# MIT-SPARK/Khronos

Measured on NVIDIA B200. Metric: rgbd_frames_per_sec_integrated, higher is better.
Workload: dtype f32

## Files before the change

khronos_b200/build.py:

```python
from __future__ import annotations

import os
import subprocess
import sys

HERE = os.path.dirname(os.path.abspath(__file__))
ROOT = os.path.dirname(HERE)
CSRC = os.path.join(HERE, "csrc")
SOURCES = ["kb_kernels.cu", "kb_motion_device.cu", "kb_objects_device.cu", "kb_tracks_device.cu", "kb_rays.cu", "kb_peer.cu", "kb_mesh.cu", "kb_api.cu", "kb_motion_host.cpp"]
HEADERS = ["kb_device.cuh", "kb_kernels.cuh", "kb_motion_device.cuh", "kb_objects_device.cuh", "kb_tracks_device.cuh", "kb_unionfind.cuh", "kb_mesh.cuh", "kb_mc_tables.h", "kb_motion_host.h", os.path.join(ROOT, "include", "khronos_b200.h")]
LIB = os.path.join(CSRC, "libkhronos_b200.so")

NVCC_FLAGS = [
    "-gencode", "arch=compute_100a,code=sm_100a", "-O3", "-lineinfo", "-std=c++17",
    "-fmad=false", "-Xcompiler", "-fPIC,-ffp-contract=off,-fno-fast-math", "-shared",
]


def _stale(target, deps):
    if not os.path.exists(target):
        return True
    t = os.path.getmtime(target)
    return any(os.path.getmtime(d) > t for d in deps)


def build_product(force=False, verbose=False):
    srcs = [os.path.join(CSRC, s) for s in SOURCES]
    deps = srcs + [h if os.path.isabs(h) else os.path.join(CSRC, h) for h in HEADERS]
    if not force and not _stale(LIB, deps):
        return LIB
    extra = [f"-DKB_FUSE_MIN_BLOCKS={os.environ['KB_FUSE_MIN_BLOCKS']}"] if os.environ.get("KB_FUSE_MIN_BLOCKS") else []
    cmd = ["nvcc"] + NVCC_FLAGS + extra + (["-Xptxas", "-v"] if verbose else []) + ["-o", LIB] + srcs
    print(" ".join(cmd), file=sys.stderr)
    subprocess.check_call(cmd, cwd=CSRC)
    return LIB


VARIANTS = {"mb12": ["-DKB_FUSE_MIN_BLOCKS=12"], "mb8": ["-DKB_FUSE_MIN_BLOCKS=8"]}


def build_variant(name):
    srcs = [os.path.join(CSRC, s) for s in SOURCES]
    out = os.path.join(CSRC, f"libkhronos_b200_{name}.so")
    cmd = ["nvcc"] + NVCC_FLAGS + VARIANTS[name] + ["-o", out] + srcs
    print(" ".join(cmd), file=sys.stderr)
    subprocess.check_call(cmd, cwd=CSRC)
    return out


def build_oracle():
    subprocess.check_call(["make", "-C", os.path.join(ROOT, "oracle")])
    return os.path.join(ROOT, "oracle", "liboracle.so")


if __name__ == "__main__":
    build_product(force="--force" in sys.argv, verbose="-v" in sys.argv)
    build_oracle()
    for v in VARIANTS:
        if ("--variant=" + v) in sys.argv:
            build_variant(v)
```

khronos_b200/csrc/kb_api.cu:

```cuda
#include <algorithm>
#include <climits>
#include <cmath>
#include <cstdio>
#include <cstdlib>
#include <cstring>
#include <string>
#include <thread>
#include <type_traits>
#include <vector>

#include "../../include/khronos_b200.h"
#include "kb_kernels.cuh"
#include "kb_mesh.cuh"
#include "kb_motion_device.cuh"
#include "kb_objects_device.cuh"
#include "kb_tracks_device.cuh"
#include "kb_motion_host.h"

using namespace kb;

struct kb_handle {
  kb_map_config map{};
  kb_integrator_config integ{};
  kb_tracking_config trk{};
  kb_motion_config mot{};
  kb_camera cam{};
  bool has_trk = false, has_mot = false, has_cam = false;
  int device = 0;
  cudaStream_t stream = nullptr;
  bool own_stream = false;
  int rank = 0, nranks = 1;
  DeviceMap dm{};
  int L = 0;
  float block_size = 0, mle_diag = 0, mle_off = 0, mle_init = 0;
  unsigned long long blocked_mask = 0;
  std::vector<uint64_t> stamps;
  float* stg_depth = nullptr;
  int* stg_label = nullptr;
  int* stg_mask = nullptr;
  int* stg_object = nullptr;
  uint16_t* stg_depth16 = nullptr;
  uint8_t* stg_label8 = nullptr;
  uint8_t* stg_color = nullptr;
  size_t stg_color_pixels = 0;
  uint16_t* mot_depth16 = nullptr;
  float* stg_vertex = nullptr;
  float* mot_depth = nullptr;
  size_t stg_pixels = 0, mot_pixels = 0;
  int stg_set = 0;
  cudaStream_t copy_stream = nullptr;
  cudaEvent_t stg_ready[2] = {nullptr, nullptr}, stg_consumed[2] = {nullptr, nullptr};
  BatchParams batch{};
  float* tile_max = nullptr;
  size_t tile_stride = 0;
  int* work_slots = nullptr;
  uint32_t* work_masks = nullptr;
  uint32_t* work_upd = nullptr;
  uint32_t* item_fmask = nullptr;
  int* item_list = nullptr;
  int item_list_cap = 0;
  bool use_item_list = true;
  bool pipelined = true;
  cudaStream_t pre_stream = nullptr;
  cudaEvent_t pre_done[2] = {nullptr, nullptr}, fuse_done[2] = {nullptr, nullptr}, main_front = nullptr;
  bool main_dirty = true;
  int* work_slots2 = nullptr;
  uint32_t* work_masks2 = nullptr;
  uint32_t* work_upd2 = nullptr;
  uint32_t* item_fmask2 = nullptr;
  bool narrow_labels = false;
  int narrow_threads = 8;
  uint8_t* pin_label8 = nullptr;
  size_t pin_label8_pixels = 0;
  int fuse_coop = 0;
  int mlp_group = 0;
  int cull_grid = 0;
  int parity = 0;
  TrackEval pass{};
  float trk_cfg_thr = 0.f;
  uint64_t last_pass_stamp = 0;
  int* pending = nullptr;
  int everfree_grid = 0;
  bool cull = true;
  bool cull_forced = false;
  int fuse_grid = 0;
  bool hwm_dirty = true;
  size_t tombstones_ub = 0;
  size_t rehash_threshold = 0;
  int hwm_cached = 0;
  int* h_ctr = nullptr;
  int prev_ctr[kNumCounters] = {0};
  bool ctr_dirty = false;
  int3* d_pixel_gidx = nullptr;
  uint8_t* d_pixel_seed = nullptr;
  std::vector<int32_t> h_pixel_gidx;
  std::vector<uint8_t> h_pixel_seed;
  std::vector<float> h_depth;
  MotionResult motion;
  MotionTable mt{};
  int32_t* d_dynamic = nullptr;
  int* h_mscal = nullptr;
  bool motion_stale = false;
  MotionHostParams motion_hp{};
  bool motion_have_image = false;
  bool everfree_v2 = true;
  bool motion_sparse = true;
  bool mt_dirty = false;
  int3* d_removed = nullptr;
  int max_removed = 0;
  float* obj_depth = nullptr;
  int* obj_label = nullptr;
  int32_t* d_object = nullptr;
  int* h_oscal = nullptr;
  size_t obj_pixels = 0;
  std::vector<int32_t> obj_image_host, obj_label_host;
  bool obj_have = false;
  int32_t* trk_ids = nullptr;
  unsigned long long* trk_export = nullptr;
  size_t trk_pixels = 0;
  int* trk_counts = nullptr;
  unsigned long long* trk_sums = nullptr;
  int* trk_present = nullptr;
  int* trk_idlist = nullptr;
  unsigned long long* trk_keys = nullptr;
  int* trk_of = nullptr;
  size_t trk_voxel_cap = 0;
  int* trk_inter = nullptr;
  size_t trk_inter_cap = 0;
  std::vector<int32_t> trk_counts_host;
  bool trk_have = false;
  ShardExchange xch{};
  int cap_pending = 1024, cap_halo = 2048;
  uint8_t* d_flags_local = nullptr;
  size_t flags_local_pixels = 0;
  TrackingParams open_pass{};
  uint64_t open_pass_stamp = 0;
  int open_pass_state = 0;
  std::vector<uint8_t> shard_table_host;
  uint8_t* shard_table_dev = nullptr;
  int* inst_counts = nullptr;
  unsigned int* inst_bbox = nullptr;
  uint8_t* inst_background = nullptr;
  uint8_t* inst_keep = nullptr;
  int* inst_bad = nullptr;
  size_t inst_pixels = 0;
  struct InstCluster { int id, count; float bbox[6]; };
  std::vector<InstCluster> inst_clusters;
  std::vector<uint8_t> inst_keep_host;
  bool inst_have = false;
  int* mesh_slots = nullptr;
  unsigned char* mesh_cases = nullptr;
  int* mesh_tri_count = nullptr;
  long long* mesh_tri_base = nullptr;
  size_t mesh_block_cap = 0;
  float* mesh_points = nullptr;
  unsigned char* mesh_colors = nullptr;
  unsigned int* mesh_labels = nullptr;
  size_t mesh_tri_cap = 0;
// ... 264 lines not shown
    return KB_ERR_INVALID;
  if (integ->semantic_mode == KB_SEMANTICS_MLE && (integ->num_labels < 2 || integ->num_labels > KB_MAX_LABELS))
    return KB_ERR_INVALID;
  if (trk && (trk->neighbor_connectivity != 6 && trk->neighbor_connectivity != 18 && trk->neighbor_connectivity != 26))
    return KB_ERR_INVALID;
  if (trk && (!(trk->temporal_buffer > 0.f) || !(trk->temporal_window > 0.f) || trk->tsdf_occupancy_threshold == 0.f))
    return KB_ERR_INVALID;
  if (mot && (mot->neighbor_connectivity != 6 && mot->neighbor_connectivity != 18 && mot->neighbor_connectivity != 26))
    return KB_ERR_INVALID;
  if (mot && (mot->max_cluster_size < mot->min_cluster_size || !(mot->max_range > 0.f)))
    return KB_ERR_INVALID;

  auto* h = new kb_handle();
  h->map = *map;
  h->integ = *integ;
  if (trk) { h->trk = *trk; h->has_trk = true; }
  {
    const float cfg = trk ? trk->tsdf_occupancy_threshold : -1.5f;
    h->trk_cfg_thr = cfg < 0 ? cfg * -map->voxel_size : cfg;
  }
  if (mot) { h->mot = *mot; h->has_mot = true; }
  h->device = device;
  h->stamps.push_back(0);
  h->block_size = map->voxel_size * static_cast<float>(map->voxels_per_side);
  h->L = !map->with_semantics ? 0
         : integ->semantic_mode == KB_SEMANTICS_MLE ? integ->num_labels
         : integ->semantic_mode == KB_SEMANTICS_BINARY ? 2 : 0;
  if (integ->semantic_mode == KB_SEMANTICS_MLE) {
    const double c = static_cast<double>(integ->label_confidence), N = static_cast<double>(integ->num_labels);
    h->mle_diag = static_cast<float>(std::log(c));
    h->mle_off = static_cast<float>(std::log((1.0 - c) / (N - 1.0)));
    h->mle_init = static_cast<float>(std::log(1.0 / N));
    for (int i = 0; i < KB_MAX_LABELS; ++i)
      if (integ->label_blocked[i]) h->blocked_mask |= 1ull << i;
  }

  DeviceMap& m = h->dm;
  m.vps = map->voxels_per_side;
  m.V = m.vps * m.vps * m.vps;
  m.max_blocks = map->max_blocks;
  m.max_sem = h->L > 0 ? (map->max_semantic_blocks > 0 ? map->max_semantic_blocks : map->max_blocks) : 0;
  m.Lp = h->L == 0 ? 0 : (integ->semantic_mode == KB_SEMANTICS_BINARY ? 2 : ((h->L + 3) / 4) * 4);
  uint32_t cap = 1024;
  while (cap < static_cast<uint32_t>(m.max_blocks) * 2u) cap <<= 1;
  m.hash_mask = cap - 1;

  int st = KB_OK;
  auto run = [&]() -> int {
    KB_CUDA(h, cudaSetDevice(device));
    KB_CUDA(h, cudaStreamCreateWithFlags(&h->stream, cudaStreamNonBlocking));
    h->own_stream = true;
    const size_t S = m.max_blocks, V = m.V;
    KB_CUDA(h, devAlloc(&m.hash_keys, cap, 0xFF));
    KB_CUDA(h, devAlloc(&m.hash_vals, cap, 0xFF));
    KB_CUDA(h, devAlloc(&m.counters, kCounterInts, 0));
    KB_CUDA(h, devAlloc(&m.free_list, S, 0));
    KB_CUDA(h, devAlloc(&m.block_index, S, 0));
    KB_CUDA(h, devAlloc(&m.block_flags, S, 0));
    KB_CUDA(h, devAlloc(&m.block_sem, S, 0xFF));
    KB_CUDA(h, devAlloc(&m.tsdf, S * V, 0));
    if (map->with_tracking) {
      KB_CUDA(h, devAlloc(&m.last_obs, S * V, 0));
      KB_CUDA(h, devAlloc(&m.last_occ, S * V, 0));
      KB_CUDA(h, devAlloc(&m.vflags, S * V, 0));
      KB_CUDA(h, devAlloc(&m.born_frame, S, 0));
      m.frame_capacity = 1 << 20;
      KB_CUDA(h, devAlloc(&m.next_pass, static_cast<size_t>(m.frame_capacity), 0));
      KB_CUDA(h, devAlloc(&m.act_min, static_cast<size_t>(m.frame_capacity), 0));
      KB_CUDA(h, devAlloc(&h->pending, S, 0));
    }
    if (h->L > 0) {
      const size_t Q = m.max_sem;
      KB_CUDA(h, devAlloc(&m.sem_free_list, Q, 0));
      KB_CUDA(h, devAlloc(&m.sem_label, Q * V, 0xFF));
      KB_CUDA(h, devAlloc(&m.sem_lik, Q * V * m.Lp, 0));
    }
    KB_CUDA(h, cudaMallocHost(reinterpret_cast<void**>(&h->h_ctr), sizeof(int) * kCounterInts));
    std::memset(h->h_ctr, 0, sizeof(int) * kCounterInts);
    KB_CUDA(h, cudaStreamCreateWithFlags(&h->copy_stream, cudaStreamNonBlocking));
    for (int i = 0; i < 2; ++i) {
      KB_CUDA(h, cudaEventCreateWithFlags(&h->stg_ready[i], cudaEventDisableTiming));
      KB_CUDA(h, cudaEventCreateWithFlags(&h->stg_consumed[i], cudaEventDisableTiming));
    }
    KB_CUDA(h, devAlloc(&h->work_slots, S, 0));
    KB_CUDA(h, devAlloc(&h->work_masks, S, 0));
    KB_CUDA(h, devAlloc(&h->work_upd, S, 0));
    h->batch.items_per_block = m.V / 128;
    KB_CUDA(h, devAlloc(&h->item_fmask, S * h->batch.items_per_block, 0));
    if (const char* e = std::getenv("KB_FUSE_ITEM_LIST")) h->use_item_list = e[0] == '1';
    h->rehash_threshold = (static_cast<size_t>(cap)) / 4;
    if (const char* e = std::getenv("KB_REHASH_TOMBSTONES")) h->rehash_threshold = static_cast<size_t>(std::max(1, std::atoi(e)));
    if (const char* e = std::getenv("KB_EVERFREE_V2")) h->everfree_v2 = e[0] == '1';
    if (const char* e = std::getenv("KB_MOTION_SPARSE")) h->motion_sparse = e[0] == '1';
    if (const char* e = std::getenv("KB_H2D_NARROW_LABELS")) h->narrow_labels = e[0] == '1';
    if (const char* e = std::getenv("KB_H2D_THREADS")) h->narrow_threads = std::max(1, std::atoi(e));
    if (const char* e = std::getenv("KB_PIPELINE")) h->pipelined = e[0] == '1';
    if (h->pipelined) {
      KB_CUDA(h, cudaStreamCreateWithFlags(&h->pre_stream, cudaStreamNonBlocking));
      for (int i = 0; i < 2; ++i) {
        KB_CUDA(h, cudaEventCreateWithFlags(&h->pre_done[i], cudaEventDisableTiming));
        KB_CUDA(h, cudaEventCreateWithFlags(&h->fuse_done[i], cudaEventDisableTiming));
      }
      KB_CUDA(h, cudaEventCreateWithFlags(&h->main_front, cudaEventDisableTiming));
      KB_CUDA(h, devAlloc(&h->work_slots2, S, 0));
      KB_CUDA(h, devAlloc(&h->work_masks2, S, 0));
      KB_CUDA(h, devAlloc(&h->work_upd2, S, 0));
      KB_CUDA(h, devAlloc(&h->item_fmask2, S * h->batch.items_per_block, 0));
    }
    if (const char* e = std::getenv("KB_FUSE_COOP")) h->fuse_coop = e[0] == '1' ? 1 : 0;
    if (const char* e = std::getenv("KB_FUSE_MLP")) h->mlp_group = e[0] == '2' ? 2 : (e[0] == '4' ? 4 : 0);
    if (h->use_item_list) {
      h->item_list_cap = static_cast<int>(std::min<size_t>(S * h->batch.items_per_block, size_t(1) << 28));
      KB_CUDA(h, devAlloc(&h->item_list, static_cast<size_t>(2 * kItemClasses) * h->item_list_cap, 0));
    }
    {
      cudaDeviceProp prop{};
      KB_CUDA(h, cudaGetDeviceProperties(&prop, device));
      h->everfree_grid = prop.multiProcessorCount * 4;
      h->cull_grid = prop.multiProcessorCount * 8;
      h->fuse_grid = prop.multiProcessorCount * fuseBlocksPerSm(m.vps, m.Lp);
      if (const char* e = std::getenv("KB_FUSE_CTAS_PER_SM")) {
        const int n = std::atoi(e);
        if (n > 0) h->fuse_grid = prop.multiProcessorCount * n;
      }
    }
    h->max_removed = m.max_blocks;
    KB_CUDA(h, devAlloc(&h->d_removed, static_cast<size_t>(h->max_removed), 0));
    KB_CUDA(h, cudaDeviceSynchronize());
    return KB_OK;
  };
  st = run();
  if (st != KB_OK) {
    std::fprintf(stderr, "kb_create: %s\n", h->err.c_str());
    kb_destroy(h);
    return st;
  }
  *out = h;
  return KB_OK;
}

int kb_destroy(kb_handle* h) {
  if (!h) return KB_OK;
  cudaSetDevice(h->device);
  if (h->stream) cudaStreamSynchronize(h->stream);
  DeviceMap& m = h->dm;
  cudaFree(m.hash_keys); cudaFree(m.hash_vals); cudaFree(m.counters); cudaFree(m.free_list);
  cudaFree(m.sem_free_list); cudaFree(m.block_index); cudaFree(m.block_flags); cudaFree(m.block_sem);
  cudaFree(m.tsdf); cudaFree(m.last_obs); cudaFree(m.last_occ); cudaFree(m.vflags);
  cudaFree(m.born_frame); cudaFree(m.next_pass); cudaFree(m.act_min); cudaFree(h->pending);
  cudaFree(m.sem_label); cudaFree(m.sem_lik); cudaFree(m.color); cudaFree(h->stg_color);
  cudaFree(h->xch.halo_mark); cudaFree(h->xch.publish); cudaFree(h->xch.ghost_keys); cudaFree(h->xch.ghost_vals);
  cudaFree(h->obj_depth); cudaFree(h->obj_label); cudaFree(h->d_object); cudaFree(h->d_flags_local);
  if (h->h_oscal) cudaFreeHost(h->h_oscal);
  cudaFree(h->trk_ids); cudaFree(h->trk_export); cudaFree(h->trk_counts); cudaFree(h->trk_sums); cudaFree(h->trk_present); cudaFree(h->trk_idlist);
  cudaFree(h->trk_keys); cudaFree(h->trk_of); cudaFree(h->trk_inter);
  cudaFree(h->stg_depth); cudaFree(h->stg_label); cudaFree(h->stg_mask); cudaFree(h->stg_object);
  cudaFree(h->stg_vertex); cudaFree(h->d_pixel_gidx); cudaFree(h->d_pixel_seed); cudaFree(h->d_removed);
  cudaFree(h->d_dynamic);
  { MotionTable& t = h->mt; cudaFree(t.keys); cudaFree(t.count); cudaFree(t.flags); cudaFree(t.deg); cudaFree(t.parent);
    cudaFree(t.pix_total); cudaFree(t.min_seed); cudaFree(t.cluster_id); cudaFree(t.roots); cudaFree(t.scalars); cudaFree(t.pix_slot); cudaFree(t.occupied); }
  if (h->h_mscal) cudaFreeHost(h->h_mscal);
  cudaFree(h->stg_depth16); cudaFree(h->stg_label8); cudaFree(h->mot_depth16);
  cudaFree(h->mot_depth); cudaFree(h->tile_max); cudaFree(h->work_slots); cudaFree(h->work_masks); cudaFree(h->work_upd); cudaFree(h->item_fmask); cudaFree(h->item_list);
  for (int i = 0; i < 2; ++i) {
    if (h->stg_ready[i]) cudaEventDestroy(h->stg_ready[i]);
    if (h->stg_consumed[i]) cudaEventDestroy(h->stg_consumed[i]);
  }
  if (h->copy_stream) { cudaStreamSynchronize(h->copy_stream); cudaStreamDestroy(h->copy_stream); }
  if (h->pin_label8) cudaFreeHost(h->pin_label8);
  if (h->pre_stream) { cudaStreamSynchronize(h->pre_stream); cudaStreamDestroy(h->pre_stream); }
  for (int i = 0; i < 2; ++i) {
    if (h->pre_done[i]) cudaEventDestroy(h->pre_done[i]);
    if (h->fuse_done[i]) cudaEventDestroy(h->fuse_done[i]);
  }
  if (h->main_front) cudaEventDestroy(h->main_front);
  cudaFree(h->work_slots2); cudaFree(h->work_masks2); cudaFree(h->work_upd2); cudaFree(h->item_fmask2);
  cudaFree(h->shard_table_dev);
  cudaFree(h->inst_counts); cudaFree(h->inst_bbox); cudaFree(h->inst_background); cudaFree(h->inst_keep); cudaFree(h->inst_bad);
  cudaFree(h->mesh_slots); cudaFree(h->mesh_cases); cudaFree(h->mesh_tri_count); cudaFree(h->mesh_tri_base);
  cudaFree(h->mesh_points); cudaFree(h->mesh_colors); cudaFree(h->mesh_labels);
  if (h->h_ctr) cudaFreeHost(h->h_ctr);
  if (h->own_stream && h->stream) cudaStreamDestroy(h->stream);
  delete h;
  return KB_OK;
}

int kb_set_stream(kb_handle* h, void* cuda_stream) {
  if (h) h->main_dirty = true;
  if (!h) return KB_ERR_INVALID;
  KB_CUDA(h, cudaSetDevice(h->device));
  KB_CUDA(h, cudaStreamSynchronize(h->stream));
  if (h->own_stream) cudaStreamDestroy(h->stream);
  h->stream = static_cast<cudaStream_t>(cuda_stream);
  h->own_stream = false;
  return KB_OK;
}

int kb_synchronize(kb_handle* h) {
  if (!h) return KB_ERR_INVALID;
  KB_CUDA(h, cudaStreamSynchronize(h->copy_stream));
  KB_CUDA(h, cudaStreamSynchronize(h->stream));
  return KB_OK;
}

int kb_set_camera(kb_handle* h, const kb_camera* cam) {
  if (!h || !cam || cam->width <= 1 || cam->height <= 1 || !(cam->fx > 0.f) || !(cam->fy > 0.f))
    return fail(h, KB_ERR_INVALID, "invalid camera");
  KB_CUDA(h, cudaSetDevice(h->device));
  const bool same = h->has_cam && std::memcmp(&h->cam, cam, sizeof(kb_camera)) == 0;
  h->cam = *cam;
  h->has_cam = true;
  if (same) return KB_OK;
  const kb_camera& c = h->cam;
  BatchParams& p = h->batch;
  p.W = c.width; p.H = c.height;
  p.fx = c.fx; p.fy = c.fy; p.cx = c.cx; p.cy = c.cy;
  p.min_range = c.min_range; p.max_range = c.max_range;
  {
    const float xl = (0.f - c.cx) / c.fx, xr = (static_cast<float>(c.width - 1) - c.cx) / c.fx;
    const float yt = (0.f - c.cy) / c.fy, yb = (static_cast<float>(c.height - 1) - c.cy) / c.fy;
    const float il = 1.f / std::sqrt(1.f + xl * xl), ir = 1.f / std::sqrt(1.f + xr * xr);
    const float it = 1.f / std::sqrt(1.f + yt * yt), ib = 1.f / std::sqrt(1.f + yb * yb);
    p.pl[0][0] = il;  p.pl[0][1] = -xl * il;
    p.pl[1][0] = -ir; p.pl[1][1] = xr * ir;
    p.pl[2][0] = it;  p.pl[2][1] = -yt * it;
    p.pl[3][0] = -ib; p.pl[3][1] = yb * ib;
  }
  p.voxel_size = h->map.voxel_size;
  p.block_size = h->block_size;
  p.trunc = h->map.truncation_distance;
  p.infl = h->block_size * 0.8660254f;
  p.use_dropoff = h->integ.use_weight_dropoff;
  p.dropoff_eps = h->integ.weight_dropoff_epsilon > 0.f ? h->integ.weight_dropoff_epsilon
                                                       : h->integ.weight_dropoff_epsilon * -h->map.voxel_size;
  p.constant_weight = h->integ.use_constant_weight;
  p.max_weight = h->integ.max_weight;
  p.interp = h->integ.interpolation_method;
  p.adaptive_thr = h->integ.adaptive_max_depth_difference;
  p.sem_mode = h->L > 0 ? h->integ.semantic_mode : KB_SEMANTICS_NONE;
  p.L = h->L;
  p.mle_diag = h->mle_diag; p.mle_off = h->mle_off; p.mle_init = h->mle_init;
  p.blocked_mask = h->blocked_mask;
  p.with_tracking = h->map.with_tracking;
  p.occ_thr = h->trk_cfg_thr;
  h->tile_stride = 0;
  for (int l = 0; l < kTileLevels; ++l) {
    p.lvl_tx[l] = l == 0 ? (c.width + 7) / 8 : (p.lvl_tx[l - 1] + 1) / 2;
    p.lvl_ty[l] = l == 0 ? (c.height + 7) / 8 : (p.lvl_ty[l - 1] + 1) / 2;
    p.lvl_off[l] = static_cast<int>(h->tile_stride);
    h->tile_stride += static_cast<size_t>(p.lvl_tx[l]) * p.lvl_ty[l];
  }
  p.work_slots = h->work_slots;
  p.work_masks = h->work_masks;
  p.work_upd = h->work_upd;
  p.item_fmask = h->item_fmask;
  p.max_work = h->dm.max_blocks;
  cudaFree(h->tile_max);
  h->tile_max = nullptr;
  KB_CUDA(h, devAlloc(&h->tile_max, h->tile_stride * kMaxBatch * 2, 0));
  return ensureMotionBuffers(h, static_cast<size_t>(c.width) * c.height);
}

int kb_get_debug_counters(kb_handle* h, int32_t* out, int32_t n) {
  if (!h || !out) return KB_ERR_INVALID;
  KB_CUDA(h, cudaSetDevice(h->device));
  int st = readCounters(h);
  if (st != KB_OK) return st;
  for (int i = 0; i < std::min<int>(n, kNumCounters); ++i) out[i] = h->h_ctr[i];
  return KB_OK;
}

int kb_set_culling(kb_handle* h, int enabled) {
  if (!h) return KB_ERR_INVALID;
  h->cull = enabled != 0;
  h->cull_forced = enabled == 2;
  return KB_OK;
}

int kb_set_shard(kb_handle* h, int rank, int nranks) {
  if (h) h->main_dirty = true;
  if (!h || nranks < 1 || rank < 0 || rank >= nranks) return fail(h, KB_ERR_INVALID, "invalid shard");
  h->rank = rank;
  h->nranks = nranks;
  h->dm.shard_cell = 0;
  h->dm.shard_gx = h->dm.shard_gy = 1;
  h->dm.shard_table = nullptr;
  h->shard_table_host.clear();
  return KB_OK;
}

int kb_set_shard_cells(kb_handle* h, int rank, int nranks, int cell_blocks, int grid_x, int grid_y) {
  if (h) h->main_dirty = true;
  if (!h || nranks < 1 || rank < 0 || rank >= nranks || cell_blocks < 0 || (cell_blocks > 0 && (grid_x < 1 || grid_y < 1)))
    return fail(h, KB_ERR_INVALID, "invalid cell shard layout");
  h->rank = rank;
  h->nranks = nranks;
  h->dm.shard_cell = cell_blocks;
  h->dm.shard_gx = cell_blocks > 0 ? grid_x : 1;
  h->dm.shard_gy = cell_blocks > 0 ? grid_y : 1;
  h->dm.shard_table = nullptr;
  h->shard_table_host.clear();
  return KB_OK;
}

int kb_set_shard_table(kb_handle* h, int rank, int nranks, int cell_blocks, int32_t origin_cx, int32_t origin_cy, int32_t width,
                       int32_t height, const uint8_t* owners) {
  if (h) h->main_dirty = true;
  if (!h || nranks < 1 || nranks > 255 || rank < 0 || rank >= nranks || cell_blocks < 1 || width < 1 || height < 1 || !owners ||
      static_cast<long long>(width) * height > (1 << 24))
    return fail(h, KB_ERR_INVALID, "invalid cell table");
  KB_CUDA(h, cudaSetDevice(h->device));
  const size_t n = static_cast<size_t>(width) * height;
  for (size_t i = 0; i < n; ++i)
    if (owners[i] >= nranks) return fail(h, KB_ERR_INVALID, "cell table entry >= nranks");
  KB_CUDA(h, cudaStreamSynchronize(h->stream));
  cudaFree(h->shard_table_dev);
  h->shard_table_dev = nullptr;
  KB_CUDA(h, cudaMalloc(reinterpret_cast<void**>(&h->shard_table_dev), n));
  KB_CUDA(h, cudaMemcpy(h->shard_table_dev, owners, n, cudaMemcpyHostToDevice));
  h->shard_table_host.assign(owners, owners + n);
  h->rank = rank;
  h->nranks = nranks;
  h->dm.shard_cell = cell_blocks;
  int gy = static_cast<int>(std::floor(std::sqrt(static_cast<double>(nranks))));
  while (nranks % gy) --gy;
  h->dm.shard_gx = nranks / gy;
  h->dm.shard_gy = gy;
  h->dm.shard_table = h->shard_table_dev;
  h->dm.tab_ox = origin_cx; h->dm.tab_oy = origin_cy; h->dm.tab_w = width; h->dm.tab_h = height;
  return KB_OK;
}

int kb_cell_owner(int32_t bx, int32_t by, int cell_blocks, int grid_x, int grid_y, int nranks) {
  if (nranks <= 1 || cell_blocks < 1 || grid_x < 1 || grid_y < 1) return 0;
  return cellOwner(bx, by, cell_blocks, grid_x, grid_y, nranks);
}

namespace {
struct HostFrustum { float pl[4][2]; float infl, min_range, max_range, block_size; };
struct HostLayout { int nranks, cell, gx, gy; const uint8_t* table; int ox, oy, w, h; };

void hostFrustum(const kb_camera& c, float block_size, HostFrustum* f) {
// ... 67 lines not shown
      for (int by = lo[1]; by <= hi[1] && mask != all; ++by)
        for (int bx = lo[0]; bx <= hi[0]; ++bx) {
          const int owner = layoutOwner(L, bx, by, bz);
          if ((mask >> owner) & 1u) continue;
          if (!candidateSelected(f, infl, R, t, bx, by, bz)) continue;
          mask |= 1u << owner;
          if (mask == all) break;
        }
    owner_mask[i] = mask;
  }
  return KB_OK;
}

int frameCellsImpl(const HostFrustum& f, const kb_frame* frames, int32_t n_frames, int cell_blocks, int32_t origin_cx, int32_t origin_cy,
                   int32_t width, int32_t height, uint8_t* touched) {
  const float infl = f.infl + 1e-3f;
  const size_t cells = static_cast<size_t>(width) * height;
  std::memset(touched, 0, cells * static_cast<size_t>(n_frames));
  for (int i = 0; i < n_frames; ++i) {
    float R[9], t[3];
    int lo[3], hi[3];
    if (!frameBox(f, infl, frames[i], R, t, lo, hi)) return KB_ERR_INVALID;
    uint8_t* row = touched + cells * static_cast<size_t>(i);
    for (int by = lo[1]; by <= hi[1]; ++by) {
      const int cy = floorDiv(by, cell_blocks) - origin_cy;
      if (cy < 0 || cy >= height) continue;
      for (int bx = lo[0]; bx <= hi[0]; ++bx) {
        const int cx = floorDiv(bx, cell_blocks) - origin_cx;
        if (cx < 0 || cx >= width || row[cy * width + cx]) continue;
        for (int bz = lo[2]; bz <= hi[2]; ++bz)
          if (candidateSelected(f, infl, R, t, bx, by, bz)) { row[cy * width + cx] = 1; break; }
      }
    }
  }
  return KB_OK;
}

HostLayout handleLayout(const kb_handle* h) {
  const DeviceMap& m = h->dm;
  return HostLayout{h->nranks, m.shard_cell, m.shard_gx, m.shard_gy, h->shard_table_host.empty() ? nullptr : h->shard_table_host.data(),
                    m.tab_ox, m.tab_oy, m.tab_w, m.tab_h};
}
}

int kb_frame_owners(kb_handle* h, const kb_frame* frames, int32_t n_frames, uint32_t* owner_mask) {
  if (!h || !frames || !owner_mask || n_frames < 0) return fail(h, KB_ERR_INVALID, "null argument");
  if (!h->has_cam) return fail(h, KB_ERR_STATE, "kb_set_camera must be called first");
  if (h->nranks > 32) return fail(h, KB_ERR_INVALID, "kb_frame_owners supports at most 32 ranks");
  HostFrustum f;
  handleFrustum(h, &f);
  const int st = frameOwnersImpl(f, handleLayout(h), frames, n_frames, owner_mask);
  return st == KB_OK ? KB_OK : fail(h, st, "non-finite sensor pose");
}

int kb_frame_cells(kb_handle* h, const kb_frame* frames, int32_t n_frames, int cell_blocks, int32_t origin_cx, int32_t origin_cy,
                   int32_t width, int32_t height, uint8_t* touched) {
  if (!h || !frames || !touched || n_frames < 0 || cell_blocks < 1 || width < 1 || height < 1) return fail(h, KB_ERR_INVALID, "invalid argument");
  if (!h->has_cam) return fail(h, KB_ERR_STATE, "kb_set_camera must be called first");
  HostFrustum f;
  handleFrustum(h, &f);
  const int st = frameCellsImpl(f, frames, n_frames, cell_blocks, origin_cx, origin_cy, width, height, touched);
  return st == KB_OK ? KB_OK : fail(h, st, "non-finite sensor pose");
}

int kb_frame_owners_host(const kb_camera* camera, float voxel_size, int32_t voxels_per_side, const kb_shard_layout* layout,
                         const kb_frame* frames, int32_t n_frames, uint32_t* owner_mask) {
  if (!camera || !layout || !frames || !owner_mask || n_frames < 0 || !(voxel_size > 0.f) || voxels_per_side < 1 || layout->nranks < 1 ||
      layout->nranks > 32 || layout->cell_blocks < 0 || (layout->cell_blocks > 0 && (layout->grid_x < 1 || layout->grid_y < 1)))
    return KB_ERR_INVALID;
  HostFrustum f;
  hostFrustum(*camera, voxel_size * static_cast<float>(voxels_per_side), &f);
  const HostLayout L{layout->nranks, layout->cell_blocks, layout->grid_x, layout->grid_y, layout->table, layout->table_origin_cx,
                     layout->table_origin_cy, layout->table_width, layout->table_height};
  return frameOwnersImpl(f, L, frames, n_frames, owner_mask);
}

int kb_frame_cells_host(const kb_camera* camera, float voxel_size, int32_t voxels_per_side, const kb_frame* frames, int32_t n_frames,
                        int cell_blocks, int32_t origin_cx, int32_t origin_cy, int32_t width, int32_t height, uint8_t* touched) {
  if (!camera || !frames || !touched || n_frames < 0 || !(voxel_size > 0.f) || voxels_per_side < 1 || cell_blocks < 1 || width < 1 || height < 1)
    return KB_ERR_INVALID;
  HostFrustum f;
  hostFrustum(*camera, voxel_size * static_cast<float>(voxels_per_side), &f);
  return frameCellsImpl(f, frames, n_frames, cell_blocks, origin_cx, origin_cy, width, height, touched);
}

static int integrateBatch(kb_handle* h, const kb_frame* frames, int n, int allocate_blocks) {
  const kb_camera& c = h->cam;
  const size_t px = static_cast<size_t>(c.width) * c.height;
  BatchParams& p = h->batch;
  if (allocate_blocks && n > 1) {
    const double reach = static_cast<double>(c.max_range) + static_cast<double>(h->block_size) * 0.8660254;
    const double inv = 1.0 / static_cast<double>(h->block_size);
    double lo[3] = {1e300, 1e300, 1e300}, hi[3] = {-1e300, -1e300, -1e300};
    for (int b = 0; b < n; ++b)
      for (int a = 0; a < 3; ++a) {
        const double t = frames[b].world_T_sensor[a * 4 + 3];
        lo[a] = std::min(lo[a], std::floor((t - reach) * inv));
        hi[a] = std::max(hi[a], std::floor((t + reach) * inv));
      }
    const double single = std::pow(2.0 * reach * inv + 2.0, 3.0);
    const double cells = (hi[0] - lo[0] + 1.0) * (hi[1] - lo[1] + 1.0) * (hi[2] - lo[2] + 1.0);
    if (!(cells <= 8.0 * single)) {
      int st = integrateBatch(h, frames, n / 2, allocate_blocks);
      if (st != KB_OK) return st;
      return integrateBatch(h, frames + n / 2, n - n / 2, allocate_blocks);
    }
  }
  p.n_frames = n;
  p.allocate = allocate_blocks ? 1 : 0;
  p.rank = h->rank;
  p.nranks = h->nranks;
  p.parity = h->parity;
  h->parity ^= 1;
  const int par = p.parity;
  const bool pipe = h->pipelined && n >= 4;
  if (!pipe) h->main_dirty = true;
  p.pipelined = pipe ? 1 : 0;
  p.fetch_ctr = (pipe && par) ? kCtrFetchB : kCtrFetch;
  p.items_ctr = (pipe && par) ? kCtrItemsB0 : kCtrItems0;
  p.work_slots = (pipe && par) ? h->work_slots2 : h->work_slots;
  p.work_masks = (pipe && par) ? h->work_masks2 : h->work_masks;
  p.work_upd = (pipe && par) ? h->work_upd2 : h->work_upd;
  p.item_fmask = (pipe && par) ? h->item_fmask2 : h->item_fmask;
  const size_t tile_set = (pipe && par) ? h->tile_stride * kMaxBatch : 0;
  p.cull = (h->cull && (n >= 4 || h->cull_forced)) ? 1 : 0;
  p.layers_per_item = n >= 8 ? 1 : 4;
  p.trk = h->pass;

  bool any_host = false, any_compact = false, any_color = false, any_host_color = false;
  for (int b = 0; b < n; ++b) {
    any_host |= frames[b].memory != KB_MEM_DEVICE;
    any_compact |= frames[b].depth_u16 != nullptr || frames[b].label_u8 != nullptr;
    any_color |= frames[b].color != nullptr;
    any_host_color |= frames[b].color != nullptr && frames[b].memory != KB_MEM_DEVICE;
  }
  p.has_color = any_color ? 1 : 0;
  p.item_list = (h->use_item_list && p.cull && n >= 8 && !any_color)
                    ? h->item_list + ((pipe && par) ? static_cast<size_t>(kItemClasses) * h->item_list_cap : 0) : nullptr;
  p.item_list_cap = h->item_list_cap;
  p.mlp_group = h->mlp_group;
  p.coop = h->fuse_coop;
  if (any_color) {
    int st = ensureColorLayer(h);
    if (st == KB_OK && any_host_color) st = ensureColorStaging(h, px);
    if (st != KB_OK) return st;
  }
  const int set = h->stg_set;
  const bool use_staging = any_host || any_compact;
  if (use_staging) {
    int st = ensureStaging(h, px);
    if (st != KB_OK) return st;
    h->stg_set ^= 1;
    KB_CUDA(h, cudaStreamWaitEvent(h->copy_stream, h->stg_consumed[set], 0));
  }
  bool narrowed[kMaxBatch] = {false};
  bool any_narrowed = false;
  if (h->narrow_labels && any_host) {
    int cand[kMaxBatch], nc = 0;
    for (int b = 0; b < n; ++b)
      if (frames[b].memory != KB_MEM_DEVICE && frames[b].label && !frames[b].label_u8) cand[nc++] = b;
    if (nc > 0) {
      if (h->pin_label8_pixels < px) {
        KB_CUDA(h, cudaStreamSynchronize(h->copy_stream));
        if (h->pin_label8) cudaFreeHost(h->pin_label8);
        h->pin_label8 = nullptr;
        KB_CUDA(h, cudaMallocHost(reinterpret_cast<void**>(&h->pin_label8), px * kMaxBatch * 2));
        h->pin_label8_pixels = px;
      }
      KB_CUDA(h, cudaEventSynchronize(h->stg_ready[set]));
      uint8_t* base8 = h->pin_label8 + static_cast<size_t>(set) * kMaxBatch * px;
      auto work = [&](int t, int T) {
        for (int k = t; k < nc; k += T) {
          const int b = cand[k];
          const int32_t* __restrict__ src = frames[b].label;
          uint8_t* __restrict__ dst = base8 + static_cast<size_t>(b) * px;
          int32_t acc = 0;
          for (size_t i = 0; i < px; ++i) { acc |= src[i]; dst[i] = static_cast<uint8_t>(src[i]); }
          narrowed[b] = (acc & ~0xFF) == 0;
        }
      };
      const int T = std::max(1, std::min(h->narrow_threads, nc));
      if (T == 1) {
        work(0, 1);
      } else {
        std::vector<std::thread> pool;
        for (int t = 0; t < T; ++t) pool.emplace_back(work, t, T);
        for (auto& th : pool) th.join();
      }
      for (int b = 0; b < n; ++b) any_narrowed |= narrowed[b];
    }
  }
  int lo[3] = {INT32_MAX, INT32_MAX, INT32_MAX}, hi[3] = {INT32_MIN, INT32_MIN, INT32_MIN};
  for (int b = 0; b < n; ++b) {
    const kb_frame& f = frames[b];
    FrameView& v = p.f[b];
    float Rw[9], tw[3];
    poseToFloat(f.world_T_sensor, v.R, v.t, Rw, tw);
    if (h->map.with_tracking && f.stamp_ns <= h->last_pass_stamp)
      return fail(h, KB_ERR_STATE, "frames must be newer than the last kb_update_tracking stamp");
    uint32_t fidx = 0;
    int st = frameIndex(h, f.stamp_ns, &fidx);
    if (st != KB_OK) return st;
    v.frame_idx = fidx;
    v.target_id = f.object_target_id;
    const size_t off = (static_cast<size_t>(set) * kMaxBatch + b) * px;
    if (f.memory == KB_MEM_DEVICE) {
      v.depth = f.depth; v.label = f.label; v.mask = f.mask; v.object_image = f.object_image;
      v.depth16 = f.depth_u16; v.label8 = f.label_u8;
      v.color = f.color;
    } else {
      v.color = f.color ? h->stg_color + off * 3 : nullptr;
      v.depth = f.depth ? h->stg_depth + off : nullptr;
      v.label = f.label ? h->stg_label + off : nullptr;
      v.mask = f.mask ? h->stg_mask + off : nullptr;
      v.object_image = f.object_image ? h->stg_object + off : nullptr;
      v.depth16 = f.depth_u16 ? h->stg_depth16 + off : nullptr;
      v.label8 = (f.label_u8 || narrowed[b]) ? h->stg_label8 + off : nullptr;
    }
    v.depth_scale = f.depth_u16_scale;
    if (v.depth16) v.depth = h->stg_depth + off;
    if (v.label8) v.label = h->stg_label + off;
    if (!v.depth) return fail(h, KB_ERR_INVALID, "frame without depth image");
    if (f.mask == KB_MASK_LAST_DETECTION)
      v.mask = h->motion_have_image ? h->d_dynamic : nullptr;
    v.tiles = h->tile_max + tile_set + static_cast<size_t>(b) * h->tile_stride;
    if (allocate_blocks) {
      const float reach = c.max_range + p.infl;
      const float inv = 1.f / h->block_size;
      for (int a = 0; a < 3; ++a) {
        lo[a] = std::min(lo[a], static_cast<int>(std::floor((tw[a] - reach) * inv)));
        hi[a] = std::max(hi[a], static_cast<int>(std::floor((tw[a] + reach) * inv)));
      }
    }
  }
  if (any_host) {
    auto copyKind = [&](auto member, auto* staging, size_t per = 1) -> int {
      using T = std::remove_pointer_t<decltype(staging)>;
      const size_t img = px * per;
      int b = 0;
      while (b < n) {
        const T* src = (frames[b].memory == KB_MEM_DEVICE) ? nullptr : static_cast<const T*>(frames[b].*member);
        if (!src || static_cast<const void*>(src) == static_cast<const void*>(KB_MASK_LAST_DETECTION)) { ++b; continue; }
        int e = b + 1;
        while (e < n && frames[e].memory != KB_MEM_DEVICE && static_cast<const T*>(frames[e].*member) == src + static_cast<size_t>(e - b) * img) ++e;
        T* dst = staging + (static_cast<size_t>(set) * kMaxBatch + b) * img;
        KB_CUDA(h, cudaMemcpyAsync(dst, src, static_cast<size_t>(e - b) * img * sizeof(T), cudaMemcpyHostToDevice, h->copy_stream));
        b = e;
      }
      return KB_OK;
    };
    int cst;
    if ((cst = copyKind(&kb_frame::depth, h->stg_depth)) != KB_OK) return cst;
    if (!any_narrowed) {
      if ((cst = copyKind(&kb_frame::label, h->stg_label)) != KB_OK) return cst;
    } else {
      for (int b = 0; b < n;) {
        if (narrowed[b]) {
          int e = b + 1;
          while (e < n && narrowed[e]) ++e;
          const size_t o = (static_cast<size_t>(set) * kMaxBatch + b) * px;
          KB_CUDA(h, cudaMemcpyAsync(h->stg_label8 + o, h->pin_label8 + o, static_cast<size_t>(e - b) * px, cudaMemcpyHostToDevice, h->copy_stream));
          b = e;
        } else {
          if (frames[b].memory != KB_MEM_DEVICE && frames[b].label) {
            const size_t o = (static_cast<size_t>(set) * kMaxBatch + b) * px;
            KB_CUDA(h, cudaMemcpyAsync(h->stg_label + o, frames[b].label, px * sizeof(int32_t), cudaMemcpyHostToDevice, h->copy_stream));
          }
          ++b;
        }
      }
    }
    if ((cst = copyKind(&kb_frame::mask, h->stg_mask)) != KB_OK) return cst;
    if ((cst = copyKind(&kb_frame::object_image, h->stg_object)) != KB_OK) return cst;
    if ((cst = copyKind(&kb_frame::depth_u16, h->stg_depth16)) != KB_OK) return cst;
    if ((cst = copyKind(&kb_frame::label_u8, h->stg_label8)) != KB_OK) return cst;
    if (any_host_color && (cst = copyKind(&kb_frame::color, h->stg_color, 3)) != KB_OK) return cst;
    KB_CUDA(h, cudaEventRecord(h->stg_ready[set], h->copy_stream));
    KB_CUDA(h, cudaStreamWaitEvent(h->stream, h->stg_ready[set], 0));
  }
  if (allocate_blocks) {
    for (int a = 0; a < 3; ++a) { p.lo[a] = lo[a]; p.dims[a] = hi[a] - lo[a] + 1; }
    h->hwm_dirty = true;
  } else {
    if (h->hwm_dirty) {
      int st, nslots = 0;
      if ((st = slotHwm(h, &nslots)) != KB_OK) return st;
      h->hwm_cached = nslots;
      h->hwm_dirty = false;
    }
    p.n_slots = h->hwm_cached;
  }
  any_compact = any_compact || any_narrowed;
  bool all_compact = any_compact;
  for (int b = 0; b < n; ++b) all_compact = all_compact && frames[b].depth_u16 != nullptr && frames[b].label == nullptr;
  p.compact_taps = all_compact ? 1 : 0;
  cudaStream_t ps = h->stream;
  if (pipe) {
    ps = h->pre_stream;
    if (any_host) KB_CUDA(h, cudaStreamWaitEvent(ps, h->stg_ready[set], 0));
    KB_CUDA(h, cudaStreamWaitEvent(ps, h->fuse_done[par], 0));
    if (h->main_dirty) {
      KB_CUDA(h, cudaEventRecord(h->main_front, h->stream));
      KB_CUDA(h, cudaStreamWaitEvent(ps, h->main_front, 0));
      h->main_dirty = false;
    }
    KB_CUDA(h, cudaMemsetAsync(h->dm.counters + kCtrWork0 + par, 0, sizeof(int), ps));
    KB_CUDA(h, cudaMemsetAsync(h->dm.counters + p.fetch_ctr, 0, sizeof(int), ps));
  }
  if (!pipe && h->pipelined) {
    KB_CUDA(h, cudaMemsetAsync(h->dm.counters + kCtrWork0 + par, 0, sizeof(int), ps));
  }
  if (any_compact && !all_compact) launchExpandFrames(p, ps);
  if (p.cull) launchTileMax(p, ps);
  launchSelectBlocks(h->dm, p, h->cull_grid, ps);
  if (pipe) {
    KB_CUDA(h, cudaEventRecord(h->pre_done[par], ps));
    KB_CUDA(h, cudaStreamWaitEvent(h->stream, h->pre_done[par], 0));
  }
  launchFuse(h->dm, p, h->fuse_grid, h->stream);
  if (pipe) KB_CUDA(h, cudaEventRecord(h->fuse_done[par], h->stream));
  KB_CUDA(h, cudaGetLastError());
  if (use_staging) KB_CUDA(h, cudaEventRecord(h->stg_consumed[set], h->stream));
  if (any_host) {
    bool must_wait = false;
    for (int b = 0; b < n; ++b) must_wait |= frames[b].memory == KB_MEM_HOST;
    if (must_wait) KB_CUDA(h, cudaStreamSynchronize(h->copy_stream));
  }
  h->ctr_dirty = true;
  return KB_OK;
}

int kb_integrate_frames(kb_handle* h, const kb_frame* frames, int32_t n_frames, int allocate_blocks,
                        kb_frame_stats* stats) {
  if (!h || !frames || n_frames < 0) return fail(h, KB_ERR_INVALID, "null frames");
  if (!h->has_cam) return fail(h, KB_ERR_STATE, "kb_set_camera must be called first");
  for (int i = 0; i < n_frames; ++i) {
    if (!frames[i].depth && !frames[i].depth_u16) return fail(h, KB_ERR_INVALID, "frame without depth image");
    for (int k = 0; k < 16; ++k)
      if (!std::isfinite(frames[i].world_T_sensor[k])) return fail(h, KB_ERR_INVALID, "non-finite sensor pose");
  }
  KB_CUDA(h, cudaSetDevice(h->device));
  int st;
  if (stats && h->ctr_dirty) {
    if ((st = readCounters(h)) != KB_OK) return st;
    std::memcpy(h->prev_ctr, h->h_ctr, sizeof(h->prev_ctr));
    h->ctr_dirty = false;
  }
  if (!h->own_stream) h->main_dirty = true;
  for (int i = 0; i < n_frames; i += kMaxBatch) {
    if ((st = integrateBatch(h, frames + i, std::min(kMaxBatch, n_frames - i), allocate_blocks)) != KB_OK) return st;
  }
  if (stats) {
    if ((st = readCounters(h)) != KB_OK) return st;
    const int* c1 = h->h_ctr;
    const int* c0 = h->prev_ctr;
    auto d = [&](int k) { return static_cast<int32_t>(static_cast<uint32_t>(c1[k]) - static_cast<uint32_t>(c0[k])); };
    stats->blocks_in_frustum = d(kCtrFrustum);
    stats->blocks_allocated = d(kCtrAllocated);
    stats->blocks_updated = d(kCtrBlocksUpdated);
    stats->voxels_updated = d(kCtrVoxelsUpdated);
    stats->voxels_in_band = d(kCtrVoxelsBand);
    stats->voxels_semantic = d(kCtrVoxelsSemantic);
    stats->total_blocks = c1[kCtrLiveBlocks];
    stats->capacity_exceeded = c1[kCtrCapacityExceeded];
    std::memcpy(h->prev_ctr, h->h_ctr, sizeof(h->prev_ctr));
    h->ctr_dirty = false;
    if (c1[kCtrCapacityExceeded]) return fail(h, KB_ERR_CAPACITY, "block / semantic pool exhausted");
  }
  return KB_OK;
}

int kb_integrate_frame(kb_handle* h, const kb_frame* f, int allocate_blocks, kb_frame_stats* stats) {
  return kb_integrate_frames(h, f, f ? 1 : 0, allocate_blocks, stats);
}

int kb_get_totals(kb_handle* h, kb_frame_stats* t) {
  if (!h || !t) return KB_ERR_INVALID;
  KB_CUDA(h, cudaSetDevice(h->device));
  int st = readCounters(h);
  if (st != KB_OK) return st;
  const int* c = h->h_ctr;
  t->blocks_in_frustum = c[kCtrFrustum];
  t->blocks_allocated = c[kCtrAllocated];
  t->blocks_updated = c[kCtrBlocksUpdated];
  t->voxels_updated = c[kCtrVoxelsUpdated];
  t->voxels_in_band = c[kCtrVoxelsBand];
  t->voxels_semantic = c[kCtrVoxelsSemantic];
  t->total_blocks = c[kCtrLiveBlocks];
  t->capacity_exceeded = c[kCtrCapacityExceeded];
  return KB_OK;
}

int kb_get_totals64(kb_handle* h, kb_totals64* t) {
  if (!h || !t) return KB_ERR_INVALID;
  KB_CUDA(h, cudaSetDevice(h->device));
  int st = readCounters(h);
  if (st != KB_OK) return st;
  const unsigned long long* c = totals64(h->h_ctr);
  t->blocks_in_frustum = c[kTotFrustum];
  t->blocks_allocated = c[kTotAllocated];
  t->blocks_updated = c[kTotBlocksUpdated];
  t->voxels_updated = c[kTotVoxelsUpdated];
  t->voxels_in_band = c[kTotVoxelsBand];
  t->voxels_semantic = c[kTotVoxelsSemantic];
  t->block_frame_pairs = c[kTotPairs];
  t->total_blocks = static_cast<uint64_t>(std::max(h->h_ctr[kCtrLiveBlocks], 0));
  t->capacity_exceeded = static_cast<uint64_t>(h->h_ctr[kCtrCapacityExceeded]);
  t->frames = static_cast<uint64_t>(h->stamps.size() - 1);
  return KB_OK;
}

int kb_map_checksum(kb_handle* h, uint64_t out[4]) {
  if (!h || !out) return KB_ERR_INVALID;
  KB_CUDA(h, cudaSetDevice(h->device));
  int st, n = 0;
  if ((st = slotHwm(h, &n)) != KB_OK) return st;
  unsigned long long *d_stamps = nullptr, *d_out = nullptr;
  auto body = [&]() -> int {
    KB_CUDA(h, cudaMalloc(&d_stamps, sizeof(uint64_t) * h->stamps.size()));
    KB_CUDA(h, cudaMalloc(&d_out, sizeof(uint64_t) * 4));
    KB_CUDA(h, cudaMemcpyAsync(d_stamps, h->stamps.data(), sizeof(uint64_t) * h->stamps.size(), cudaMemcpyHostToDevice, h->stream));
    KB_CUDA(h, cudaMemsetAsync(d_out, 0, sizeof(uint64_t) * 4, h->stream));
    launchChecksum(h->dm, n, d_stamps, d_out, h->stream);
    KB_CUDA(h, cudaGetLastError());
    KB_CUDA(h, cudaMemcpyAsync(out, d_out, sizeof(uint64_t) * 4, cudaMemcpyDeviceToHost, h->stream));
    KB_CUDA(h, cudaStreamSynchronize(h->stream));
    return KB_OK;
  };
  st = body();
  cudaFree(d_stamps);
  cudaFree(d_out);
  h->main_dirty = true;
  return st;
}
// ... 1144 lines not shown
```

khronos_b200/csrc/kb_device.cuh:

```cuda
#pragma once

#include <cuda_runtime.h>
#include <stdint.h>

namespace kb {

constexpr unsigned long long kEmptyKey = ~0ull;
constexpr unsigned long long kTombKey = ~0ull - 1ull;
constexpr uint32_t kFlagAllocated = 1u << 8;
constexpr uint32_t kFlagEverFreePending = 1u << 9;
constexpr uint32_t kPublicFlagMask = 0x1Fu;
constexpr uint16_t kSemEmpty = 0xFFFFu;
constexpr uint8_t kVoxEverFree = 1, kVoxActive = 2, kVoxToRemove = 4;
constexpr uint8_t kVoxNotOccupied = 8;
constexpr uint32_t kFlagInactiveOverride = 1u << 10;

struct DeviceMap {
  unsigned long long* hash_keys;
  int* hash_vals;
  uint32_t hash_mask;
  int max_blocks, max_sem;
  int vps, V, Lp;
  int* counters;
  int* free_list;
  int* sem_free_list;
  int3* block_index;
  uint32_t* block_flags;
  int* block_sem;
  float2* tsdf;
  uint32_t* last_obs;
  uint32_t* last_occ;
  uint8_t* vflags;
  uint32_t* born_frame;
  uint32_t* next_pass;
  uint32_t* act_min;
  int frame_capacity;
  uint16_t* sem_label;
  float* sem_lik;
  uchar4* color;
  int shard_cell, shard_gx, shard_gy;
  const uint8_t* shard_table;
  int tab_ox, tab_oy, tab_w, tab_h;
};

enum Counter {
  kCtrPoolHwm = 0,
  kCtrFreeCount = 1,
  kCtrSemHwm = 2,
  kCtrSemFreeCount = 3,
  kCtrLiveBlocks = 4,
  kCtrCapacityExceeded = 5,
  kCtrFrustum = 6,
  kCtrAllocated = 7,
  kCtrBlocksUpdated = 8,
  kCtrVoxelsUpdated = 9,
  kCtrVoxelsBand = 10,
  kCtrVoxelsSemantic = 11,
  kCtrSeeds = 12,
  kCtrRemoved = 13,
  kCtrErased = 14,
  kCtrWork0 = 15,
  kCtrWork1 = 16,
  kCtrPairs = 17,
  kCtrPending = 18,
  kCtrFetch = 19,
  kCtrHalo = 20,
  kCtrFetchB = 24,
  kCtrRehash = 28,
  kCtrItems0 = 32,
  kCtrItemsB0 = 40,
  kNumCounters = 48
};
constexpr int kItemClasses = 8;

enum Total64 {
  kTotVoxelsUpdated = 0,
  kTotVoxelsBand = 1,
  kTotVoxelsSemantic = 2,
  kTotFrustum = 3,
  kTotPairs = 4,
  kTotBlocksUpdated = 5,
  kTotAllocated = 6,
  kNumTotals = 8
};
constexpr int kCounterInts = kNumCounters + 2 * kNumTotals;
__host__ __device__ inline unsigned long long* totals64(int* counters) {
  return reinterpret_cast<unsigned long long*>(counters + kNumCounters);
}

__host__ __device__ inline unsigned long long packKey(int x, int y, int z) {
  const unsigned long long o = 1ull << 20, m = (1ull << 21) - 1ull;
  return ((static_cast<unsigned long long>(x + static_cast<long long>(o)) & m)) |
         ((static_cast<unsigned long long>(y + static_cast<long long>(o)) & m) << 21) |
         ((static_cast<unsigned long long>(z + static_cast<long long>(o)) & m) << 42);
}

__host__ __device__ inline unsigned long long mix64(unsigned long long k) {
  k ^= k >> 33;
  k *= 0xff51afd7ed558ccdull;
  k ^= k >> 33;
  k *= 0xc4ceb9fe1a85ec53ull;
  k ^= k >> 33;
  return k;
}

__host__ __device__ inline int blockOwner(int x, int y, int z, int nranks) {
  return static_cast<int>((mix64(packKey(x, y, z)) >> 40) % static_cast<unsigned long long>(nranks));
}

__host__ __device__ inline int cellOwner(int x, int y, int cell, int gx, int gy, int nranks) {
  const int cx = (x >= 0 ? x : x - cell + 1) / cell, cy = (y >= 0 ? y : y - cell + 1) / cell;
  const int mx = ((cx % gx) + gx) % gx, my = ((cy % gy) + gy) % gy;
  return (mx + gx * my) % nranks;
}
__host__ __device__ inline int floorDiv(int a, int b) { return (a >= 0 ? a : a - b + 1) / b; }
__host__ __device__ inline int tableOwner(const uint8_t* table, int ox, int oy, int w, int h, int cell, int gx, int gy, int x, int y,
                                          int nranks) {
  const int cx = floorDiv(x, cell) - ox, cy = floorDiv(y, cell) - oy;
  if (cx >= 0 && cx < w && cy >= 0 && cy < h) return table[cy * w + cx] % nranks;
  return cellOwner(x, y, cell, gx, gy, nranks);
}
__device__ inline int mapOwner(const DeviceMap& m, int x, int y, int z, int nranks) {
  if (m.shard_cell <= 0) return blockOwner(x, y, z, nranks);
  if (m.shard_table) return tableOwner(m.shard_table, m.tab_ox, m.tab_oy, m.tab_w, m.tab_h, m.shard_cell, m.shard_gx, m.shard_gy, x, y, nranks);
  return cellOwner(x, y, m.shard_cell, m.shard_gx, m.shard_gy, nranks);
}

#ifdef __CUDACC__
__device__ inline int hashLookup(const DeviceMap& m, int x, int y, int z) {
  const unsigned long long key = packKey(x, y, z);
  uint32_t h = static_cast<uint32_t>(mix64(key)) & m.hash_mask;
  for (uint32_t probe = 0; probe <= m.hash_mask; ++probe) {
    const unsigned long long k = m.hash_keys[h];
    if (k == key) return m.hash_vals[h];
    if (k == kEmptyKey) return -1;
    h = (h + 1) & m.hash_mask;
  }
  return -1;
}

__device__ inline int allocSlot(int* counters, int ctr_hwm, int ctr_free, const int* free_list, int cap) {
  int nfree = atomicSub(&counters[ctr_free], 1);
  if (nfree > 0) return free_list[nfree - 1];
  atomicAdd(&counters[ctr_free], 1);
  const int s = atomicAdd(&counters[ctr_hwm], 1);
  if (s >= cap) {
    atomicSub(&counters[ctr_hwm], 1);
    atomicExch(&counters[kCtrCapacityExceeded], 1);
    return -1;
  }
  return s;
}

__device__ inline int hashFindOrInsert(const DeviceMap& m, int x, int y, int z, uint32_t born, int* created) {
  const unsigned long long key = packKey(x, y, z);
  uint32_t h = static_cast<uint32_t>(mix64(key)) & m.hash_mask;
// ... 76 lines not shown
```

khronos_b200/csrc/kb_kernels.cu:

```cuda
#include <limits.h>

#include <algorithm>

#include "../../include/khronos_b200.h"
#include "kb_kernels.cuh"

namespace kb {

namespace {

constexpr int kThreads = 256;
constexpr int kFuseThreads = 128;
#ifndef KB_FUSE_MIN_BLOCKS
#define KB_FUSE_MIN_BLOCKS 10
#endif
#ifndef KB_FUSE_COLOR_MIN_BLOCKS
#define KB_FUSE_COLOR_MIN_BLOCKS 8
#endif

__device__ __forceinline__ void xform(const float* R, const float* t, float x, float y, float z,
                                      float& ox, float& oy, float& oz) {
  ox = ((R[0] * x + R[1] * y) + R[2] * z) + t[0];
  oy = ((R[3] * x + R[4] * y) + R[5] * z) + t[1];
  oz = ((R[6] * x + R[7] * y) + R[8] * z) + t[2];
}

__device__ __forceinline__ bool inFrustum(const BatchParams& p, float x, float y, float z) {
  const float infl = p.infl;
  if (z < -infl) return false;
  const float r = sqrtf((x * x + y * y) + z * z);
  if (r < p.min_range - infl || r > p.max_range + infl) return false;
  if (p.pl[0][0] * x + p.pl[0][1] * z < -infl) return false;
  if (p.pl[1][0] * x + p.pl[1][1] * z < -infl) return false;
  if (p.pl[2][0] * y + p.pl[2][1] * z < -infl) return false;
  if (p.pl[3][0] * y + p.pl[3][1] * z < -infl) return false;
  return true;
}

template <bool COMPACT>
__device__ __forceinline__ float depthAt(const FrameView& f, int i) {
  if (COMPACT) return static_cast<float>(__ldg(&f.depth16[i])) * f.depth_scale;
  return __ldg(&f.depth[i]);
}
template <bool COMPACT>
__device__ __forceinline__ int labelAt(const FrameView& f, int i) {
  if (COMPACT) return static_cast<int>(__ldg(&f.label8[i]));
  return __ldg(&f.label[i]);
}

struct Taps {
  bool valid, bilinear;
  int u, v;
  float w0, w1, w2, w3;
};

template <bool COMPACT>
__device__ __forceinline__ Taps nearestTaps(const BatchParams& p, const FrameView& f, float u, float v) {
  Taps t;
  t.bilinear = false;
  t.u = static_cast<int>(roundf(u));
  t.v = static_cast<int>(roundf(v));
  t.w0 = t.w1 = t.w2 = t.w3 = 0.f;
  t.valid = t.u >= 0 && t.u < p.W && t.v >= 0 && t.v < p.H && depthAt<COMPACT>(f, t.v * p.W + t.u) > 0.f;
  return t;
}

template <bool COMPACT>
__device__ __forceinline__ Taps computeTaps(const BatchParams& p, const FrameView& f, float u, float v, float& range) {
  Taps t;
  t.valid = false;
  if (p.interp == KB_INTERP_NEAREST) {
    t = nearestTaps<COMPACT>(p, f, u, v);
    if (t.valid) range = depthAt<COMPACT>(f, t.v * p.W + t.u);
    return t;
  }
  const int u0 = static_cast<int>(floorf(u)), v0 = static_cast<int>(floorf(v));
  const bool inside = u0 >= 0 && v0 >= 0 && u0 + 1 < p.W && v0 + 1 < p.H;
  bool use_nearest = !inside;
  float r0 = 0.f, r1 = 0.f, r2 = 0.f, r3 = 0.f;
  if (inside) {
    const int i0 = v0 * p.W + u0;
    r0 = depthAt<COMPACT>(f, i0);
    r2 = depthAt<COMPACT>(f, i0 + 1);
    r1 = depthAt<COMPACT>(f, i0 + p.W);
    r3 = depthAt<COMPACT>(f, i0 + p.W + 1);
    const bool all_valid = r0 > 0.f && r1 > 0.f && r2 > 0.f && r3 > 0.f;
    if (p.interp == KB_INTERP_ADAPTIVE) {
      const float mx = fmaxf(fmaxf(r0, r1), fmaxf(r2, r3));
      const float mn = fminf(fminf(r0, r1), fminf(r2, r3));
      use_nearest = !all_valid || !(mx - mn < p.adaptive_thr);
    } else if (!all_valid) {
      return t;
    }
  } else if (p.interp != KB_INTERP_ADAPTIVE) {
    return t;
  }
  if (use_nearest) {
    t = nearestTaps<COMPACT>(p, f, u, v);
    if (t.valid) range = depthAt<COMPACT>(f, t.v * p.W + t.u);
    return t;
  }
  const float du = u - static_cast<float>(u0), dv = v - static_cast<float>(v0);
  t.valid = true;
  t.bilinear = true;
  t.u = u0;
  t.v = v0;
  t.w0 = (1.f - du) * (1.f - dv);
  t.w1 = (1.f - du) * dv;
  t.w2 = du * (1.f - dv);
  t.w3 = du * dv;
  range = ((t.w0 * r0 + t.w1 * r1) + t.w2 * r2) + t.w3 * r3;
  return t;
}

__device__ __forceinline__ int tapIndex(const BatchParams& p, const Taps& t) {
  int du = 0, dv = 0;
  if (t.bilinear) {
    int best = 0;
    float bw = t.w0;
    if (t.w1 > bw) { best = 1; bw = t.w1; }
    if (t.w2 > bw) { best = 2; bw = t.w2; }
    if (t.w3 > bw) { best = 3; }
    du = best >> 1;
    dv = best & 1;
  }
  return (t.v + dv) * p.W + t.u + du;
}

__device__ __forceinline__ float measurementWeight(const BatchParams& p, float depth, float sdf) {
  float w = (p.fx * p.fy) * (p.voxel_size * p.voxel_size) / (depth * depth);
  if (!p.constant_weight) w = w / (depth * depth);
  if (p.use_dropoff && sdf < -p.dropoff_eps) {
    w = w * ((p.trunc + sdf) / (p.trunc - p.dropoff_eps));
    w = fmaxf(w, 0.f);
  }
  return w;
}

__device__ __forceinline__ uchar3 measuredColor(const BatchParams& p, const FrameView& f, const Taps& t) {
  const uint8_t* __restrict__ p0 = f.color + (static_cast<size_t>(t.v) * p.W + t.u) * 3;
  if (!t.bilinear) return make_uchar3(__ldg(p0), __ldg(p0 + 1), __ldg(p0 + 2));
  const uint8_t* __restrict__ p1 = p0 + static_cast<size_t>(p.W) * 3;
  uint8_t o[3];
#pragma unroll
  for (int ch = 0; ch < 3; ++ch) {
    const float s = ((t.w0 * static_cast<float>(__ldg(p0 + ch)) + t.w1 * static_cast<float>(__ldg(p1 + ch))) +
                     t.w2 * static_cast<float>(__ldg(p0 + 3 + ch))) + t.w3 * static_cast<float>(__ldg(p1 + 3 + ch));
    o[ch] = static_cast<uint8_t>(static_cast<int>(s));
  }
  return make_uchar3(o[0], o[1], o[2]);
}

__device__ __forceinline__ uint8_t mergeChannel(uint8_t c, uint8_t cm, float ratio) {
  return static_cast<uint8_t>(static_cast<int>(static_cast<float>(c) * (1.f - ratio) + static_cast<float>(cm) * ratio));
}

__device__ __forceinline__ int warpSum(int v) {
#pragma unroll
  for (int o = 16; o > 0; o >>= 1) v += __shfl_xor_sync(0xffffffffu, v, o);
  return v;
}

__global__ void __launch_bounds__(256) expandFramesKernel(const __grid_constant__ BatchParams p) {
  const FrameView& f = p.f[blockIdx.y];
  const int n = p.W * p.H;
  for (int i = blockIdx.x * blockDim.x + threadIdx.x; i < n; i += gridDim.x * blockDim.x) {
    if (f.depth16) const_cast<float*>(f.depth)[i] = static_cast<float>(__ldg(&f.depth16[i])) * f.depth_scale;
    if (f.label8) const_cast<int*>(f.label)[i] = static_cast<int>(__ldg(&f.label8[i]));
  }
}

__global__ void expandDepthKernel(const uint16_t* __restrict__ src, float scale, float* __restrict__ dst, int n) {
  const int i = blockIdx.x * blockDim.x + threadIdx.x;
  if (i < n) dst[i] = static_cast<float>(src[i]) * scale;
}

__global__ void __launch_bounds__(256) tileMaxKernel(const __grid_constant__ BatchParams p) {
  const int b = blockIdx.y;
  const int warps_x = (p.W + 31) / 32;
  const int warp = blockIdx.x * 8 + (threadIdx.x >> 5);
  const int lane = threadIdx.x & 31;
  if (warp >= warps_x * p.lvl_ty[1]) return;
  const int ty16 = warp / warps_x, wx = warp % warps_x;
  const int u = wx * 32 + lane;
  const FrameView& f = p.f[b];
  float d[2] = {0.f, 0.f};
#pragma unroll
  for (int r = 0; r < 16; ++r) {
    const int v = ty16 * 16 + r;
    if (u < p.W && v < p.H)
      d[r >> 3] = fmaxf(d[r >> 3], p.compact_taps ? depthAt<true>(f, v * p.W + u) : depthAt<false>(f, v * p.W + u));
  }
#pragma unroll
  for (int h = 0; h < 2; ++h) {
    d[h] = fmaxf(d[h], __shfl_xor_sync(0xffffffffu, d[h], 1));
    d[h] = fmaxf(d[h], __shfl_xor_sync(0xffffffffu, d[h], 2));
    d[h] = fmaxf(d[h], __shfl_xor_sync(0xffffffffu, d[h], 4));
    const int tx = wx * 4 + (lane >> 3), ty = ty16 * 2 + h;
    if ((lane & 7) == 0 && tx < p.lvl_tx[0] && ty < p.lvl_ty[0]) p.f[b].tiles[p.lvl_off[0] + ty * p.lvl_tx[0] + tx] = d[h];
  }
  float m16 = fmaxf(d[0], d[1]);
  m16 = fmaxf(m16, __shfl_xor_sync(0xffffffffu, m16, 8));
  const int tx16 = wx * 2 + (lane >> 4);
  if ((lane & 15) == 0 && tx16 < p.lvl_tx[1]) p.f[b].tiles[p.lvl_off[1] + ty16 * p.lvl_tx[1] + tx16] = m16;
}

__global__ void __launch_bounds__(256) tileMaxVec4Kernel(const __grid_constant__ BatchParams p) {
  const int b = blockIdx.y;
  const int strips_x = (p.W + 127) / 128;
  const int warp = blockIdx.x * 8 + (threadIdx.x >> 5);
  const int lane = threadIdx.x & 31;
  if (warp >= strips_x * p.lvl_ty[1]) return;
  const int ty16 = warp / strips_x, sx = warp % strips_x;
  const int u = sx * 128 + lane * 4;
  const FrameView& f = p.f[b];
  float d[2] = {0.f, 0.f};
  if (u < p.W) {
    const float4* __restrict__ base = reinterpret_cast<const float4*>(f.depth + u);
    const int w4 = p.W >> 2;
    float4 v[16];
#pragma unroll
    for (int r = 0; r < 16; ++r) {
// ... 79 lines not shown
__device__ __forceinline__ bool boxCulledLane(const BatchParams& p, const FrameView& f, float lox, float loy, float loz,
                                              float hix, float hiy, float hiz) {
  return boxCulledPose(p, f.R, f.t, f.tiles, lox, loy, loz, hix, hiy, hiz);
}

template <bool PIPE>
__global__ void __launch_bounds__(128) selectBlocksKernel(const DeviceMap m, const __grid_constant__ BatchParams p) {
  const int c0 = (blockIdx.x * blockDim.x + threadIdx.x) >> 5;
  const int lane = threadIdx.x & 31;
  __shared__ float s_pose[12][kMaxBatch];
  __shared__ const float* s_tiles[kMaxBatch];
  for (int i = threadIdx.x; i < 12 * kMaxBatch; i += blockDim.x) {
    const int b = i % kMaxBatch, k = i / kMaxBatch;
    s_pose[k][b] = b < p.n_frames ? (k < 9 ? p.f[b].R[k] : p.f[b].t[k - 9]) : 0.f;
  }
  if (threadIdx.x < kMaxBatch) s_tiles[threadIdx.x] = threadIdx.x < p.n_frames ? p.f[threadIdx.x].tiles : nullptr;
  __syncthreads();
  float Rl[9], tl[3];
#pragma unroll
  for (int k = 0; k < 9; ++k) Rl[k] = s_pose[k][lane];
#pragma unroll
  for (int k = 0; k < 3; ++k) tl[k] = s_pose[9 + k][lane];
  if (!PIPE && c0 == 0 && lane == 0) {
    m.counters[kCtrWork0 + (p.parity ^ 1)] = 0;
    m.counters[kCtrFetch] = 0;
  }
  int slot = -1, bx = 0, by = 0, bz = 0;
  uint32_t mask = 0;
  int created = 0;
  if (p.allocate) {
    if (c0 >= p.dims[0] * p.dims[1] * p.dims[2]) return;
    int c = c0;
    bx = p.lo[0] + c % p.dims[0];
    c /= p.dims[0];
    by = p.lo[1] + c % p.dims[1];
    bz = p.lo[2] + c / p.dims[1];
    const float cx = (static_cast<float>(bx) + 0.5f) * p.block_size;
    const float cy = (static_cast<float>(by) + 0.5f) * p.block_size;
    const float cz = (static_cast<float>(bz) + 0.5f) * p.block_size;
    if (p.nranks > 1 && mapOwner(m, bx, by, bz, p.nranks) != p.rank) return;
    bool in = false;
    if (lane < p.n_frames) {
      float x, y, z;
      xform(Rl, tl, cx, cy, cz, x, y, z);
      in = inFrustum(p, x, y, z);
    }
    mask = __ballot_sync(0xffffffffu, in);
    if (!mask) return;
    if (lane == 0) slot = hashFindOrInsert(m, bx, by, bz, p.f[__ffs(mask) - 1].frame_idx, &created);
    slot = __shfl_sync(0xffffffffu, slot, 0);
    if (slot < 0) return;
  } else {
    if (c0 >= p.n_slots || !(m.block_flags[c0] & kFlagAllocated)) return;
    slot = c0;
    const int3 bi = m.block_index[slot];
    bx = bi.x; by = bi.y; bz = bi.z;
    mask = p.n_frames >= 32 ? 0xffffffffu : ((1u << p.n_frames) - 1u);
  }
  if (lane == 0) {
    atomicAdd(&m.counters[kCtrFrustum], __popc(mask));
    atomicAdd(&totals64(m.counters)[kTotFrustum], static_cast<unsigned long long>(__popc(mask)));
    if (created) {
      atomicAdd(&m.counters[kCtrAllocated], 1);
      atomicAdd(&totals64(m.counters)[kTotAllocated], 1ull);
    }
  }
  if (p.cull) {
    const float ox = static_cast<float>(bx) * p.block_size, oy = static_cast<float>(by) * p.block_size,
                oz = static_cast<float>(bz) * p.block_size;
    const float lo = 0.5f * p.voxel_size, hi = p.block_size - 0.5f * p.voxel_size;
    bool keep = false;
    if ((mask >> lane) & 1u)
      keep = !boxCulledPose(p, Rl, tl, s_tiles[lane], ox + lo, oy + lo, oz + lo, ox + hi, oy + hi, oz + hi);
    mask = __ballot_sync(0xffffffffu, keep);
    if (!mask) return;
  }
  int i = 0;
  if (lane == 0) {
    if (p.L > 0 && m.block_sem[slot] < 0) {
      m.block_sem[slot] = allocSlot(m.counters, kCtrSemHwm, kCtrSemFreeCount, m.sem_free_list, m.max_sem);
    }
    atomicAdd(&m.counters[kCtrPairs], __popc(mask));
    atomicAdd(&totals64(m.counters)[kTotPairs], static_cast<unsigned long long>(__popc(mask)));
    i = atomicAdd(&m.counters[kCtrWork0 + p.parity], 1);
    if (i < p.max_work) {
      p.work_slots[i] = slot;
      p.work_masks[i] = mask;
      p.work_upd[i] = 0;
    } else {
      atomicExch(&m.counters[kCtrCapacityExceeded], 1);
    }
  }
  i = __shfl_sync(0xffffffffu, i, 0);
  if (i < p.max_work && lane < p.items_per_block) p.item_fmask[static_cast<size_t>(i) * p.items_per_block + lane] = p.cull ? 0u : mask;
}

constexpr int kCullChunk = 1;
template <int VPS>
__global__ void __launch_bounds__(128) itemCullKernel(const DeviceMap m, const __grid_constant__ BatchParams p) {
  constexpr int ITEMS = (VPS / 4) * (VPS / 8) * (VPS / 4);
  const int lane = threadIdx.x & 31;
  const int warp = (blockIdx.x * blockDim.x + threadIdx.x) >> 5;
  const int n_warps = (gridDim.x * blockDim.x) >> 5;
  const int chunks = (p.n_frames + kCullChunk - 1) / kCullChunk;
  const int n = min(m.counters[kCtrWork0 + p.parity], p.max_work) * chunks;
  for (int w = warp; w < n; w += n_warps) {
    const int wi = w / chunks, ch = w % chunks;
    const uint32_t bmask = p.work_masks[wi] & (((kCullChunk >= 32 ? 0u : (1u << kCullChunk)) - 1u) << (ch * kCullChunk));
    if (!bmask || lane >= ITEMS) continue;
    const int3 bi = m.block_index[p.work_slots[wi]];
    int x0, y0, z0;
    itemOrigin<VPS>(lane, x0, y0, z0);
    const float ox = static_cast<float>(bi.x) * p.block_size, oy = static_cast<float>(bi.y) * p.block_size,
                oz = static_cast<float>(bi.z) * p.block_size;
    const float lx = ox + (static_cast<float>(x0) + 0.5f) * p.voxel_size, hx = ox + (static_cast<float>(x0 + 3) + 0.5f) * p.voxel_size;
    const float ly = oy + (static_cast<float>(y0) + 0.5f) * p.voxel_size, hy = oy + (static_cast<float>(y0 + 7) + 0.5f) * p.voxel_size;
    const float lz = oz + (static_cast<float>(z0) + 0.5f) * p.voxel_size, hz = oz + (static_cast<float>(z0 + 3) + 0.5f) * p.voxel_size;
    uint32_t keep = 0, rem = bmask;
    while (rem) {
      const int b = __ffs(rem) - 1;
      rem &= rem - 1;
      if (!boxCulledLane(p, p.f[b], lx, ly, lz, hx, hy, hz)) keep |= 1u << b;
    }
    if (keep) atomicOr(&p.item_fmask[static_cast<size_t>(wi) * ITEMS + lane], keep);
  }
}

template <int VPS, bool PB>
__global__ void __launch_bounds__(256) itemCompactKernel(const DeviceMap m, const __grid_constant__ BatchParams p) {
  constexpr int kItems = PB ? kCtrItemsB0 : kCtrItems0;
  constexpr int BOXES = (VPS / 4) * (VPS / 8) * (VPS / 4);
  const int n = min(m.counters[kCtrWork0 + p.parity], p.max_work) * BOXES;
  const int lane = threadIdx.x & 31;
  for (int base = (blockIdx.x * blockDim.x + threadIdx.x) - lane; base < n; base += gridDim.x * blockDim.x) {
    const int i = base + lane;
    const uint32_t fm = i < n ? p.item_fmask[i] : 0u;
    const int cls = fm ? (32 - __popc(fm)) >> 2 : -1;
    const unsigned peers = __match_any_sync(0xffffffffu, cls);
    if (cls < 0) continue;
    const int leader = __ffs(peers) - 1;
    int start = 0;
    if (lane == leader) start = atomicAdd(&m.counters[kItems + cls], __popc(peers));
    start = __shfl_sync(peers, start, leader);
    const int idx = start + __popc(peers & ((1u << lane) - 1u));
    if (idx < p.item_list_cap) p.item_list[static_cast<size_t>(cls) * p.item_list_cap + idx] = i;
  }
}

template <bool PB>
__device__ __forceinline__ int listedBox(const BatchParams& p, const int (&n_cls)[kItemClasses], int j) {
  int k = 0;
#pragma unroll
  for (int c = 0; c < kItemClasses - 1; ++c) {
    if (k == c && j >= n_cls[c]) { j -= n_cls[c]; k = c + 1; }
  }
  return p.item_list[static_cast<size_t>(k) * p.item_list_cap + j];
}

__device__ __noinline__ uint32_t trackingFold(const DeviceMap m, const TrackEval t, uint32_t born, size_t gi) {
  const uint8_t fl = m.vflags[gi];
  const uint32_t c_stored = m.last_occ[gi];
  uint32_t c_true;
  bool act, rem;
  evalTracking(m, t, born, m.last_obs[gi], c_stored, fl, &c_true, &act, &rem);
  if (c_true != c_stored) m.last_occ[gi] = c_true;
  return (fl & kVoxEverFree) | (act ? kVoxActive : 0) | (rem ? kVoxToRemove : 0);
}

template <int VPS, int LPI, bool COMPACT, bool COLOR, bool LIST = false, bool PB = false>
__global__ void __launch_bounds__(kFuseThreads, COLOR ? KB_FUSE_COLOR_MIN_BLOCKS : KB_FUSE_MIN_BLOCKS) fuseKernel(const DeviceMap m, const __grid_constant__ BatchParams p) {
  constexpr int kFetch = PB ? kCtrFetchB : kCtrFetch;
  [[maybe_unused]] constexpr int kItems = PB ? kCtrItemsB0 : kCtrItems0;
  constexpr int V = VPS * VPS * VPS;
  constexpr int NK = 4;
  constexpr int BOXES = (VPS / 4) * (VPS / 8) * (VPS / NK);
  extern __shared__ float s_rows[];
  const int lane = threadIdx.x & 31;
  constexpr int lpi = LPI, ipb = NK / LPI;
  int n_cls[kItemClasses] = {0};
  int n_items;
  if constexpr (LIST) {
    n_items = 0;
#pragma unroll
    for (int c = 0; c < kItemClasses; ++c) {
      n_cls[c] = min(m.counters[kItems + c], p.item_list_cap);
      n_items += n_cls[c];
    }
    n_items *= ipb;
  } else {
    n_items = min(m.counters[kCtrWork0 + p.parity], p.max_work) * BOXES * ipb;
  }
  const bool binary = p.sem_mode == KB_SEMANTICS_BINARY;
  const int L = p.L;
  int n_valid = 0, n_band = 0, n_sem = 0;

  int pending = 0;
  if (lane == 0) pending = atomicAdd(&m.counters[kFetch], 1);
  for (;;) {
    const int w = __shfl_sync(0xffffffffu, pending, 0);
    if (w >= n_items) break;
    if (lane == 0) pending = atomicAdd(&m.counters[kFetch], 1);
    int box = w / ipb;
    if constexpr (LIST) {
      box = listedBox<PB>(p, n_cls, box);
    }
    const uint32_t fmask = p.item_fmask[box];
    if (!fmask) continue;
    const int wi = box / BOXES, it = box % BOXES;
    const int slot = p.work_slots[wi];
    const int3 bi = m.block_index[slot];
    const int sem = L > 0 ? m.block_sem[slot] : -1;
    int x0, y0, z0;
    itemOrigin<VPS>(it, x0, y0, z0);
    uint32_t upd_all = 0;
    bool any_have = false;
#pragma unroll 1
    for (int k = (w % ipb) * lpi; k < (w % ipb) * lpi + lpi; ++k) {
    const int vx = x0 + (lane & 3), vy = y0 + (lane >> 2), vz = z0 + k;
    const int lin = vx + VPS * (vy + VPS * vz);
    const size_t gi = static_cast<size_t>(slot) * V + lin;
    const float wx = static_cast<float>(bi.x) * p.block_size + (static_cast<float>(vx) + 0.5f) * p.voxel_size;
    const float wy = static_cast<float>(bi.y) * p.block_size + (static_cast<float>(vy) + 0.5f) * p.voxel_size;
    const float wz = static_cast<float>(bi.z) * p.block_size + (static_cast<float>(vz) + 0.5f) * p.voxel_size;
    float2 st = make_float2(0.f, 0.f);
    uint32_t lobs = 0, vfl = 0, upd_frames = 0;
    bool have = false, row_resident = false;
    int best_label = 0;
    uchar4 col = make_uchar4(0, 0, 0, 0);
    bool col_dirty = false;

    uint32_t rem = fmask;
    while (rem) {
      const int b = __ffs(rem) - 1;
      rem &= rem - 1;
      const FrameView& f = p.f[b];
      const bool has_label_img = L > 0 && (binary ? f.object_image != nullptr : (COMPACT ? f.label8 != nullptr : f.label != nullptr));
      float x, y, z;
      xform(f.R, f.t, wx, wy, wz, x, y, z);
      if (z <= 0.f) continue;
      const float u = p.fx * x / z + p.cx;
      const float v = p.fy * y / z + p.cy;
      if (u < 0.f || u > static_cast<float>(p.W - 1) || v < 0.f || v > static_cast<float>(p.H - 1)) continue;
      float range = 0.f;
      const Taps taps = computeTaps<COMPACT>(p, f, u, v, range);
      if (!taps.valid) continue;
      const float sdf = range - z;
      if (sdf < -p.trunc) continue;
      const bool in_band = fabsf(sdf) < p.trunc;
      uint32_t label = 0;
      if (in_band) {
        const int ti = tapIndex(p, taps);
        if (f.mask != nullptr && __ldg(&f.mask[ti]) != 0) continue;
        if (has_label_img) {
          if (binary) {
            label = __ldg(&f.object_image[ti]) == f.target_id ? 1u : 0u;
          } else {
            label = static_cast<uint32_t>(labelAt<COMPACT>(f, ti));
            if (label < static_cast<uint32_t>(KB_MAX_LABELS) && ((p.blocked_mask >> label) & 1ull)) continue;
          }
        }
      }
      const float wm = measurementWeight(p, z, sdf);
      if (!have) {
        st = m.tsdf[gi];
        have = true;
        if (p.with_tracking) vfl = trackingFold(m, p.trk, m.born_frame[slot], gi);
        if constexpr (COLOR) col = m.color[gi];
      }
      const float sdf_c = fminf(fmaxf(sdf, -p.trunc), p.trunc);
      const float2 old = st;
      st.x = (old.x * old.y + sdf_c * wm) / (old.y + wm);
      st.y = fminf(old.y + wm, p.max_weight);
      lobs = f.frame_idx;
      upd_frames |= 1u << b;
      ++n_valid;
      if (!in_band) continue;
      ++n_band;
      if constexpr (COLOR) {
        if (f.color != nullptr) {
          const uchar3 cm = measuredColor(p, f, taps);
          const float tot = old.y + wm;
          const float ratio = tot > 0.f ? wm / tot : 0.f;
          col.x = mergeChannel(col.x, cm.x, ratio);
          col.y = mergeChannel(col.y, cm.y, ratio);
          col.z = mergeChannel(col.z, cm.z, ratio);
          col_dirty = true;
        }
      }
      if (sem >= 0 && has_label_img && label < static_cast<uint32_t>(L)) {
        const size_t si = static_cast<size_t>(sem) * V + lin;
        if (!row_resident) {
          row_resident = true;
          const bool empty = m.sem_label[si] == kSemEmpty;
          if (binary) {
            const float2 c = empty ? make_float2(0.f, 0.f) : *reinterpret_cast<const float2*>(m.sem_lik + si * 2);
            s_rows[threadIdx.x] = c.x;
            s_rows[kFuseThreads + threadIdx.x] = c.y;
          } else {
            const float4* __restrict__ lk = reinterpret_cast<const float4*>(m.sem_lik + si * m.Lp);
            for (int k4 = 0; k4 < m.Lp; k4 += 4) {
              const float4 c = empty ? make_float4(p.mle_init, p.mle_init, p.mle_init, p.mle_init) : lk[k4 >> 2];
              s_rows[(k4 + 0) * kFuseThreads + threadIdx.x] = c.x;
              s_rows[(k4 + 1) * kFuseThreads + threadIdx.x] = c.y;
              s_rows[(k4 + 2) * kFuseThreads + threadIdx.x] = c.z;
              s_rows[(k4 + 3) * kFuseThreads + threadIdx.x] = c.w;
            }
          }
        }
        if (binary) {
          const float c = s_rows[label * kFuseThreads + threadIdx.x] + 1.f;
          s_rows[label * kFuseThreads + threadIdx.x] = c;
          best_label = s_rows[kFuseThreads + threadIdx.x] > s_rows[threadIdx.x] ? 1 : 0;
        } else {
          for (int k2 = 0; k2 < m.Lp; k2 += 2) {
            float c0 = s_rows[(k2 + 0) * kFuseThreads + threadIdx.x], c1 = s_rows[(k2 + 1) * kFuseThreads + threadIdx.x];
            c0 += static_cast<uint32_t>(k2 + 0) == label ? p.mle_diag : p.mle_off;
            c1 += static_cast<uint32_t>(k2 + 1) == label ? p.mle_diag : p.mle_off;
            s_rows[(k2 + 0) * kFuseThreads + threadIdx.x] = c0;
            s_rows[(k2 + 1) * kFuseThreads + threadIdx.x] = c1;
          }
        }
        ++n_sem;
      }
    }

    if (have) {
      m.tsdf[gi] = st;
      if constexpr (COLOR) {
        if (col_dirty) m.color[gi] = col;
      }
      if (p.with_tracking) {
        m.last_obs[gi] = lobs;
        m.vflags[gi] = static_cast<uint8_t>(vfl | (st.x < p.occ_thr ? 0 : kVoxNotOccupied));
      }
      if (row_resident) {
        const size_t si = static_cast<size_t>(sem) * V + lin;
        if (binary) {
          *reinterpret_cast<float2*>(m.sem_lik + si * 2) = make_float2(s_rows[threadIdx.x], s_rows[kFuseThreads + threadIdx.x]);
        } else {
          float4* __restrict__ lk = reinterpret_cast<float4*>(m.sem_lik + si * m.Lp);
          for (int k4 = 0; k4 < m.Lp; k4 += 4)
            lk[k4 >> 2] = make_float4(s_rows[(k4 + 0) * kFuseThreads + threadIdx.x], s_rows[(k4 + 1) * kFuseThreads + threadIdx.x],
                                      s_rows[(k4 + 2) * kFuseThreads + threadIdx.x], s_rows[(k4 + 3) * kFuseThreads + threadIdx.x]);
        }
        if (!binary) {
          float bestv = s_rows[threadIdx.x];
          best_label = 0;
          for (int kk = 1; kk < L; ++kk) {
            const float c = s_rows[kk * kFuseThreads + threadIdx.x];
            if (c > bestv) { bestv = c; best_label = kk; }
          }
        }
        m.sem_label[si] = static_cast<uint16_t>(best_label);
      }
    }
    upd_all |= upd_frames;
    any_have |= have;
    }
    if (__any_sync(0xffffffffu, any_have)) {
      uint32_t upd_frames = upd_all;
#pragma unroll
      for (int o = 16; o > 0; o >>= 1) upd_frames |= __shfl_xor_sync(0xffffffffu, upd_frames, o);
      if (lane == 0) {
        const uint32_t all = KB_FLAG_UPDATED | KB_FLAG_MESH_UPDATED | KB_FLAG_ESDF_UPDATED | KB_FLAG_TRACKING_UPDATED;
        if ((m.block_flags[slot] & all) != all) atomicOr(&m.block_flags[slot], all);
        if ((p.work_upd[wi] & upd_frames) != upd_frames) {
          const uint32_t prev = atomicOr(&p.work_upd[wi], upd_frames);
          const int fresh = __popc(upd_frames & ~prev);
          if (fresh) {
            atomicAdd(&m.counters[kCtrBlocksUpdated], fresh);
            atomicAdd(&totals64(m.counters)[kTotBlocksUpdated], static_cast<unsigned long long>(fresh));
          }
        }
      }
    }
  }
  n_valid = warpSum(n_valid);
  if (n_valid) {
    n_band = warpSum(n_band);
    n_sem = warpSum(n_sem);
    if (lane == 0) {
      unsigned long long* t64 = totals64(m.counters);
      atomicAdd(&m.counters[kCtrVoxelsUpdated], n_valid);
      atomicAdd(&t64[kTotVoxelsUpdated], static_cast<unsigned long long>(n_valid));
      if (n_band) {
        atomicAdd(&m.counters[kCtrVoxelsBand], n_band);
        atomicAdd(&t64[kTotVoxelsBand], static_cast<unsigned long long>(n_band));
      }
      if (n_sem) {
        atomicAdd(&m.counters[kCtrVoxelsSemantic], n_sem);
        atomicAdd(&t64[kTotVoxelsSemantic], static_cast<unsigned long long>(n_sem));
      }
    }
  }
}

template <int VPS, bool COMPACT, bool PB>
__global__ void __launch_bounds__(kFuseThreads, KB_FUSE_MIN_BLOCKS) fuseKernelCoop(const DeviceMap m, const __grid_constant__ BatchParams p) {
  constexpr int kFetch = PB ? kCtrFetchB : kCtrFetch;
  constexpr int kItems = PB ? kCtrItemsB0 : kCtrItems0;
  constexpr int V = VPS * VPS * VPS;
  constexpr int NK = 4;
  constexpr int BOXES = (VPS / 4) * (VPS / 8) * (VPS / NK);
  constexpr uint8_t kInvalid = 0xFE, kNoSem = 0xFF;
  extern __shared__ float s_dyn[];
  const int rows_floats = max(m.Lp, 2) * 32;
  float* __restrict__ s_rows = s_dyn;
  float* __restrict__ s_w = s_dyn + rows_floats;
  float* __restrict__ s_s = s_w + 32 * 32;
  uint8_t* __restrict__ s_l = reinterpret_cast<uint8_t*>(s_s + 32 * 32);
  __shared__ int s_item;
  const int warp = threadIdx.x >> 5, lane = threadIdx.x & 31;
  int n_cls[kItemClasses];
  int n_items = 0;
#pragma unroll
  for (int c = 0; c < kItemClasses; ++c) {
    n_cls[c] = min(m.counters[kItems + c], p.item_list_cap);
    n_items += n_cls[c];
  }
  n_items *= NK;
  const bool binary = p.sem_mode == KB_SEMANTICS_BINARY;
  const int L = p.L;
  int n_valid = 0, n_band = 0, n_sem = 0;
  int pending = 0;
  if (threadIdx.x == 0) pending = atomicAdd(&m.counters[kFetch], 1);
  for (;;) {
    if (threadIdx.x == 0) s_item = pending;
    __syncthreads();
    const int w = s_item;
    if (w >= n_items) break;
    if (threadIdx.x == 0) pending = atomicAdd(&m.counters[kFetch], 1);
    const int box = listedBox<PB>(p, n_cls, w / NK);
    const uint32_t fmask = p.item_fmask[box];
    const int wi = box / BOXES, it = box % BOXES;
    const int slot = p.work_slots[wi];
    const int3 bi = m.block_index[slot];
    const int sem = L > 0 ? m.block_sem[slot] : -1;
    int x0, y0, z0;
    itemOrigin<VPS>(it, x0, y0, z0);
    const int vx = x0 + (lane & 3), vy = y0 + (lane >> 2), vz = z0 + (w % NK);
    const int lin = vx + VPS * (vy + VPS * vz);
    const size_t gi = static_cast<size_t>(slot) * V + lin;
    const float wx = static_cast<float>(bi.x) * p.block_size + (static_cast<float>(vx) + 0.5f) * p.voxel_size;
    const float wy = static_cast<float>(bi.y) * p.block_size + (static_cast<float>(vy) + 0.5f) * p.voxel_size;
    const float wz = static_cast<float>(bi.z) * p.block_size + (static_cast<float>(vz) + 0.5f) * p.voxel_size;
    const int nf = __popc(fmask);
    for (int r = warp; r < nf; r += 4) {
      const int b = __fns(fmask, 0, r + 1);
      const FrameView& f = p.f[b];
      const bool has_label_img = L > 0 && (binary ? f.object_image != nullptr : (COMPACT ? f.label8 != nullptr : f.label != nullptr));
      uint8_t tag = kInvalid;
      float sdf = 0.f, wm = 0.f;
      float x, y, z;
      xform(f.R, f.t, wx, wy, wz, x, y, z);
      if (z > 0.f) {
        const float u = p.fx * x / z + p.cx;
        const float v = p.fy * y / z + p.cy;
        if (!(u < 0.f || u > static_cast<float>(p.W - 1) || v < 0.f || v > static_cast<float>(p.H - 1))) {
          float range = 0.f;
          const Taps taps = computeTaps<COMPACT>(p, f, u, v, range);
          if (taps.valid) {
            sdf = range - z;
            if (!(sdf < -p.trunc)) {
              bool ok = true;
              uint32_t label = 0;
              const bool in_band = fabsf(sdf) < p.trunc;
              if (in_band) {
                const int ti = tapIndex(p, taps);
                if (f.mask != nullptr && __ldg(&f.mask[ti]) != 0) ok = false;
                if (ok && has_label_img) {
                  if (binary) {
                    label = __ldg(&f.object_image[ti]) == f.target_id ? 1u : 0u;
                  } else {
                    label = static_cast<uint32_t>(labelAt<COMPACT>(f, ti));
                    if (label < static_cast<uint32_t>(KB_MAX_LABELS) && ((p.blocked_mask >> label) & 1ull)) ok = false;
                  }
                }
              }
              if (ok) {
                wm = measurementWeight(p, z, sdf);
                tag = (in_band && sem >= 0 && has_label_img && label < static_cast<uint32_t>(L)) ? static_cast<uint8_t>(label) : kNoSem;
              }
            }
          }
        }
      }
      s_w[r * 32 + lane] = wm;
      s_s[r * 32 + lane] = sdf;
      s_l[r * 32 + lane] = tag;
    }
    __syncthreads();
    if (warp == 0) {
      float2 st = make_float2(0.f, 0.f);
      uint32_t lobs = 0, vfl = 0, upd_frames = 0;
      bool have = false, row_resident = false;
      int best_label = 0;
      uint32_t rem = fmask;
      int r = 0;
      while (rem) {
        const int b = __ffs(rem) - 1;
        rem &= rem - 1;
        const uint8_t tag = s_l[r * 32 + lane];
        const float wm = s_w[r * 32 + lane], sdf = s_s[r * 32 + lane];
        ++r;
        if (tag == kInvalid) continue;
        if (!have) {
          st = m.tsdf[gi];
          have = true;
          if (p.with_tracking) vfl = trackingFold(m, p.trk, m.born_frame[slot], gi);
        }
        const float sdf_c = fminf(fmaxf(sdf, -p.trunc), p.trunc);
        const float2 old = st;
        st.x = (old.x * old.y + sdf_c * wm) / (old.y + wm);
        st.y = fminf(old.y + wm, p.max_weight);
        lobs = p.f[b].frame_idx;
        upd_frames |= 1u << b;
        ++n_valid;
        if (!(fabsf(sdf) < p.trunc)) continue;
        ++n_band;
        if (tag == kNoSem) continue;
        const uint32_t label = tag;
        const size_t si = static_cast<size_t>(sem) * V + lin;
        if (!row_resident) {
          row_resident = true;
          const bool empty = m.sem_label[si] == kSemEmpty;
          if (binary) {
            const float2 c = empty ? make_float2(0.f, 0.f) : *reinterpret_cast<const float2*>(m.sem_lik + si * 2);
            s_rows[lane] = c.x;
            s_rows[32 + lane] = c.y;
          } else {
            const float4* __restrict__ lk = reinterpret_cast<const float4*>(m.sem_lik + si * m.Lp);
            for (int k4 = 0; k4 < m.Lp; k4 += 4) {
              const float4 c = empty ? make_float4(p.mle_init, p.mle_init, p.mle_init, p.mle_init) : lk[k4 >> 2];
              s_rows[(k4 + 0) * 32 + lane] = c.x;
              s_rows[(k4 + 1) * 32 + lane] = c.y;
              s_rows[(k4 + 2) * 32 + lane] = c.z;
              s_rows[(k4 + 3) * 32 + lane] = c.w;
            }
          }
        }
        if (binary) {
          s_rows[label * 32 + lane] = s_rows[label * 32 + lane] + 1.f;
          best_label = s_rows[32 + lane] > s_rows[lane] ? 1 : 0;
        } else {
          for (int k2 = 0; k2 < m.Lp; k2 += 2) {
            float c0 = s_rows[(k2 + 0) * 32 + lane], c1 = s_rows[(k2 + 1) * 32 + lane];
            c0 += static_cast<uint32_t>(k2 + 0) == label ? p.mle_diag : p.mle_off;
            c1 += static_cast<uint32_t>(k2 + 1) == label ? p.mle_diag : p.mle_off;
            s_rows[(k2 + 0) * 32 + lane] = c0;
            s_rows[(k2 + 1) * 32 + lane] = c1;
          }
        }
        ++n_sem;
      }
      if (have) {
        m.tsdf[gi] = st;
        if (p.with_tracking) {
          m.last_obs[gi] = lobs;
          m.vflags[gi] = static_cast<uint8_t>(vfl | (st.x < p.occ_thr ? 0 : kVoxNotOccupied));
        }
        if (row_resident) {
          const size_t si = static_cast<size_t>(sem) * V + lin;
          if (binary) {
            *reinterpret_cast<float2*>(m.sem_lik + si * 2) = make_float2(s_rows[lane], s_rows[32 + lane]);
          } else {
            float4* __restrict__ lk = reinterpret_cast<float4*>(m.sem_lik + si * m.Lp);
            for (int k4 = 0; k4 < m.Lp; k4 += 4)
              lk[k4 >> 2] = make_float4(s_rows[(k4 + 0) * 32 + lane], s_rows[(k4 + 1) * 32 + lane], s_rows[(k4 + 2) * 32 + lane],
                                        s_rows[(k4 + 3) * 32 + lane]);
            float bestv = s_rows[lane];
            best_label = 0;
            for (int kk = 1; kk < L; ++kk) {
              const float c = s_rows[kk * 32 + lane];
              if (c > bestv) { bestv = c; best_label = kk; }
            }
          }
          m.sem_label[si] = static_cast<uint16_t>(best_label);
        }
      }
      if (__any_sync(0xffffffffu, have)) {
#pragma unroll
        for (int o = 16; o > 0; o >>= 1) upd_frames |= __shfl_xor_sync(0xffffffffu, upd_frames, o);
        if (lane == 0) {
          const uint32_t all = KB_FLAG_UPDATED | KB_FLAG_MESH_UPDATED | KB_FLAG_ESDF_UPDATED | KB_FLAG_TRACKING_UPDATED;
          if ((m.block_flags[slot] & all) != all) atomicOr(&m.block_flags[slot], all);
          if ((p.work_upd[wi] & upd_frames) != upd_frames) {
            const uint32_t prev = atomicOr(&p.work_upd[wi], upd_frames);
            const int fresh = __popc(upd_frames & ~prev);
            if (fresh) {
              atomicAdd(&m.counters[kCtrBlocksUpdated], fresh);
              atomicAdd(&totals64(m.counters)[kTotBlocksUpdated], static_cast<unsigned long long>(fresh));
            }
          }
        }
      }
    }
  }
  if (warp == 0) {
    n_valid = warpSum(n_valid);
    if (n_valid) {
      n_band = warpSum(n_band);
      n_sem = warpSum(n_sem);
      if (lane == 0) {
        unsigned long long* t64 = totals64(m.counters);
        atomicAdd(&m.counters[kCtrVoxelsUpdated], n_valid);
        atomicAdd(&t64[kTotVoxelsUpdated], static_cast<unsigned long long>(n_valid));
        if (n_band) {
          atomicAdd(&m.counters[kCtrVoxelsBand], n_band);
          atomicAdd(&t64[kTotVoxelsBand], static_cast<unsigned long long>(n_band));
        }
        if (n_sem) {
          atomicAdd(&m.counters[kCtrVoxelsSemantic], n_sem);
          atomicAdd(&t64[kTotVoxelsSemantic], static_cast<unsigned long long>(n_sem));
        }
      }
    }
  }
}

#ifndef KB_FUSE_MLP_MIN_BLOCKS
#define KB_FUSE_MLP_MIN_BLOCKS 5
#endif
template <int VPS, int LPI, bool COMPACT, int G, bool LIST, bool PB = false>
__global__ void __launch_bounds__(kFuseThreads, KB_FUSE_MLP_MIN_BLOCKS) fuseKernelMlp(const DeviceMap m, const __grid_constant__ BatchParams p) {
  constexpr int kFetch = PB ? kCtrFetchB : kCtrFetch;
  [[maybe_unused]] constexpr int kItems = PB ? kCtrItemsB0 : kCtrItems0;
  constexpr int V = VPS * VPS * VPS;
  constexpr int NK = 4;
  constexpr int BOXES = (VPS / 4) * (VPS / 8) * (VPS / NK);
  extern __shared__ float s_rows[];
  const int lane = threadIdx.x & 31;
  constexpr int lpi = LPI, ipb = NK / LPI;
  int n_cls[kItemClasses] = {0};
  int n_items;
  if constexpr (LIST) {
    n_items = 0;
#pragma unroll
    for (int c = 0; c < kItemClasses; ++c) {
      n_cls[c] = min(m.counters[kItems + c], p.item_list_cap);
      n_items += n_cls[c];
    }
    n_items *= ipb;
  } else {
    n_items = min(m.counters[kCtrWork0 + p.parity], p.max_work) * BOXES * ipb;
  }
  const bool binary = p.sem_mode == KB_SEMANTICS_BINARY;
  const int L = p.L;
  const int W = p.W, H = p.H;
  int n_valid = 0, n_band = 0, n_sem = 0;

  int pending = 0;
  if (lane == 0) pending = atomicAdd(&m.counters[kFetch], 1);
  for (;;) {
    const int w = __shfl_sync(0xffffffffu, pending, 0);
    if (w >= n_items) break;
    if (lane == 0) pending = atomicAdd(&m.counters[kFetch], 1);
    int box = w / ipb;
    if constexpr (LIST) {
      box = listedBox<PB>(p, n_cls, box);
    }
    const uint32_t fmask = p.item_fmask[box];
    if (!fmask) continue;
    const int wi = box / BOXES, it = box % BOXES;
    const int slot = p.work_slots[wi];
    const int3 bi = m.block_index[slot];
    const int sem = L > 0 ? m.block_sem[slot] : -1;
    int x0, y0, z0;
    itemOrigin<VPS>(it, x0, y0, z0);
    uint32_t upd_all = 0;
    bool any_have = false;
#pragma unroll 1
    for (int k = (w % ipb) * lpi; k < (w % ipb) * lpi + lpi; ++k) {
      const int vx = x0 + (lane & 3), vy = y0 + (lane >> 2), vz = z0 + k;
      const int lin = vx + VPS * (vy + VPS * vz);
      const size_t gi = static_cast<size_t>(slot) * V + lin;
      const float wx = static_cast<float>(bi.x) * p.block_size + (static_cast<float>(vx) + 0.5f) * p.voxel_size;
      const float wy = static_cast<float>(bi.y) * p.block_size + (static_cast<float>(vy) + 0.5f) * p.voxel_size;
      const float wz = static_cast<float>(bi.z) * p.block_size + (static_cast<float>(vz) + 0.5f) * p.voxel_size;
      float2 st = make_float2(0.f, 0.f);
      uint32_t lobs = 0, vfl = 0, upd_frames = 0;
      bool have = false, row_resident = false;
      int best_label = 0;

      uint32_t rem = fmask;
#pragma unroll 1
      while (rem) {
        int fb[G];
        bool ok[G], inside[G];
        int u0[G], v0[G];
        float fz[G], du[G], dv[G], r0[G], r1[G], r2[G], r3[G];
#pragma unroll
        for (int g = 0; g < G; ++g) {
          ok[g] = false;
          fb[g] = 0;
          if (rem) {
            const int b = __ffs(rem) - 1;
            rem &= rem - 1;
            fb[g] = b;
            const FrameView& f = p.f[b];
            float x, y, z;
            xform(f.R, f.t, wx, wy, wz, x, y, z);
            const float zs = z > 0.f ? z : 1.f;
            const float u = p.fx * x / zs + p.cx;
            const float v = p.fy * y / zs + p.cy;
            const bool o = z > 0.f && !(u < 0.f || u > static_cast<float>(W - 1) || v < 0.f || v > static_cast<float>(H - 1));
            const int iu = o ? static_cast<int>(floorf(u)) : 0, iv = o ? static_cast<int>(floorf(v)) : 0;
            ok[g] = o;
            fz[g] = z;
            u0[g] = iu;
            v0[g] = iv;
            du[g] = u - static_cast<float>(iu);
            dv[g] = v - static_cast<float>(iv);
            inside[g] = iu + 1 < W && iv + 1 < H;
            const int iu1 = min(iu + 1, W - 1), iv1 = min(iv + 1, H - 1);
            r0[g] = depthAt<COMPACT>(f, iv * W + iu);
            r2[g] = depthAt<COMPACT>(f, iv * W + iu1);
            r1[g] = depthAt<COMPACT>(f, iv1 * W + iu);
            r3[g] = depthAt<COMPACT>(f, iv1 * W + iu1);
          }
        }
        bool valid[G], band[G];
        float sdfc[G], wm[G];
        uint32_t lab[G];
        int maskv[G];
#pragma unroll
        for (int g = 0; g < G; ++g) {
          valid[g] = false;
          band[g] = false;
          sdfc[g] = 0.f;
          wm[g] = 0.f;
          lab[g] = 0;
          maskv[g] = 0;
          if (!ok[g]) continue;
          const FrameView& f = p.f[fb[g]];
          const bool ru = du[g] >= 0.5f, rv = dv[g] >= 0.5f;
          const float rn = ru ? (rv ? r3[g] : r2[g]) : (rv ? r1[g] : r0[g]);
          bool tv = false, bil = false;
          float range = 0.f, w0 = 0.f, w1 = 0.f, w2 = 0.f, w3 = 0.f;
          if (p.interp == KB_INTERP_NEAREST) {
            tv = rn > 0.f;
            range = rn;
          } else {
            bool use_nearest = !inside[g], reject = false;
            if (inside[g]) {
              const bool all_valid = r0[g] > 0.f && r1[g] > 0.f && r2[g] > 0.f && r3[g] > 0.f;
              if (p.interp == KB_INTERP_ADAPTIVE) {
                const float mx = fmaxf(fmaxf(r0[g], r1[g]), fmaxf(r2[g], r3[g]));
                const float mn = fminf(fminf(r0[g], r1[g]), fminf(r2[g], r3[g]));
                use_nearest = !all_valid || !(mx - mn < p.adaptive_thr);
              } else if (!all_valid) {
                reject = true;
              }
            } else if (p.interp != KB_INTERP_ADAPTIVE) {
              reject = true;
            }
            if (!reject) {
              if (use_nearest) {
                tv = rn > 0.f;
                range = rn;
              } else {
                tv = true;
                bil = true;
                w0 = (1.f - du[g]) * (1.f - dv[g]);
                w1 = (1.f - du[g]) * dv[g];
                w2 = du[g] * (1.f - dv[g]);
                w3 = du[g] * dv[g];
                range = ((w0 * r0[g] + w1 * r1[g]) + w2 * r2[g]) + w3 * r3[g];
              }
            }
          }
          if (!tv) continue;
          const float sdf = range - fz[g];
          if (sdf < -p.trunc) continue;
          valid[g] = true;
          band[g] = fabsf(sdf) < p.trunc;
          sdfc[g] = fminf(fmaxf(sdf, -p.trunc), p.trunc);
          wm[g] = measurementWeight(p, fz[g], sdf);
          if (band[g]) {
            int tu = u0[g] + (ru ? 1 : 0), tvv = v0[g] + (rv ? 1 : 0);
            if (bil) {
              int best = 0;
              float bw = w0;
              if (w1 > bw) { best = 1; bw = w1; }
              if (w2 > bw) { best = 2; bw = w2; }
              if (w3 > bw) { best = 3; }
              tu = u0[g] + (best >> 1);
              tvv = v0[g] + (best & 1);
            }
            const int ti = tvv * W + tu;
            if (f.mask != nullptr) maskv[g] = __ldg(&f.mask[ti]);
            const bool has_label_img = L > 0 && (binary ? f.object_image != nullptr : (COMPACT ? f.label8 != nullptr : f.label != nullptr));
            if (has_label_img) {
              if (binary) lab[g] = __ldg(&f.object_image[ti]) == f.target_id ? 1u : 0u;
              else lab[g] = static_cast<uint32_t>(labelAt<COMPACT>(f, ti));
            }
          }
        }
#pragma unroll
        for (int g = 0; g < G; ++g) {
          if (!valid[g]) continue;
          const int b = fb[g];
          const FrameView& f = p.f[b];
          const bool has_label_img = L > 0 && (binary ? f.object_image != nullptr : (COMPACT ? f.label8 != nullptr : f.label != nullptr));
          const uint32_t label = lab[g];
          if (band[g]) {
            if (maskv[g] != 0) continue;
            if (has_label_img && !binary && label < static_cast<uint32_t>(KB_MAX_LABELS) && ((p.blocked_mask >> label) & 1ull)) continue;
          }
          if (!have) {
            st = m.tsdf[gi];
            have = true;
            if (p.with_tracking) vfl = trackingFold(m, p.trk, m.born_frame[slot], gi);
          }
          const float2 old = st;
          st.x = (old.x * old.y + sdfc[g] * wm[g]) / (old.y + wm[g]);
          st.y = fminf(old.y + wm[g], p.max_weight);
          lobs = f.frame_idx;
          upd_frames |= 1u << b;
          ++n_valid;
          if (!band[g]) continue;
          ++n_band;
          if (sem >= 0 && has_label_img && label < static_cast<uint32_t>(L)) {
            const size_t si = static_cast<size_t>(sem) * V + lin;
            if (!row_resident) {
              row_resident = true;
              const bool empty = m.sem_label[si] == kSemEmpty;
              if (binary) {
                const float2 c = empty ? make_float2(0.f, 0.f) : *reinterpret_cast<const float2*>(m.sem_lik + si * 2);
                s_rows[threadIdx.x] = c.x;
                s_rows[kFuseThreads + threadIdx.x] = c.y;
              } else {
                const float4* __restrict__ lk = reinterpret_cast<const float4*>(m.sem_lik + si * m.Lp);
                for (int k4 = 0; k4 < m.Lp; k4 += 4) {
                  const float4 c = empty ? make_float4(p.mle_init, p.mle_init, p.mle_init, p.mle_init) : lk[k4 >> 2];
                  s_rows[(k4 + 0) * kFuseThreads + threadIdx.x] = c.x;
                  s_rows[(k4 + 1) * kFuseThreads + threadIdx.x] = c.y;
                  s_rows[(k4 + 2) * kFuseThreads + threadIdx.x] = c.z;
                  s_rows[(k4 + 3) * kFuseThreads + threadIdx.x] = c.w;
                }
              }
            }
            if (binary) {
              const float c = s_rows[label * kFuseThreads + threadIdx.x] + 1.f;
              s_rows[label * kFuseThreads + threadIdx.x] = c;
              best_label = s_rows[kFuseThreads + threadIdx.x] > s_rows[threadIdx.x] ? 1 : 0;
            } else {
              for (int k2 = 0; k2 < m.Lp; k2 += 2) {
                float c0 = s_rows[(k2 + 0) * kFuseThreads + threadIdx.x], c1 = s_rows[(k2 + 1) * kFuseThreads + threadIdx.x];
                c0 += static_cast<uint32_t>(k2 + 0) == label ? p.mle_diag : p.mle_off;
                c1 += static_cast<uint32_t>(k2 + 1) == label ? p.mle_diag : p.mle_off;
                s_rows[(k2 + 0) * kFuseThreads + threadIdx.x] = c0;
                s_rows[(k2 + 1) * kFuseThreads + threadIdx.x] = c1;
              }
            }
            ++n_sem;
          }
        }
      }

      if (have) {
        m.tsdf[gi] = st;
        if (p.with_tracking) {
          m.last_obs[gi] = lobs;
          m.vflags[gi] = static_cast<uint8_t>(vfl | (st.x < p.occ_thr ? 0 : kVoxNotOccupied));
        }
        if (row_resident) {
          const size_t si = static_cast<size_t>(sem) * V + lin;
          if (binary) {
            *reinterpret_cast<float2*>(m.sem_lik + si * 2) = make_float2(s_rows[threadIdx.x], s_rows[kFuseThreads + threadIdx.x]);
          } else {
            float4* __restrict__ lk = reinterpret_cast<float4*>(m.sem_lik + si * m.Lp);
            for (int k4 = 0; k4 < m.Lp; k4 += 4)
              lk[k4 >> 2] = make_float4(s_rows[(k4 + 0) * kFuseThreads + threadIdx.x], s_rows[(k4 + 1) * kFuseThreads + threadIdx.x],
                                        s_rows[(k4 + 2) * kFuseThreads + threadIdx.x], s_rows[(k4 + 3) * kFuseThreads + threadIdx.x]);
          }
          if (!binary) {
            float bestv = s_rows[threadIdx.x];
            best_label = 0;
            for (int kk = 1; kk < L; ++kk) {
              const float c = s_rows[kk * kFuseThreads + threadIdx.x];
              if (c > bestv) { bestv = c; best_label = kk; }
            }
          }
          m.sem_label[si] = static_cast<uint16_t>(best_label);
        }
      }
      upd_all |= upd_frames;
      any_have |= have;
    }
    if (__any_sync(0xffffffffu, any_have)) {
      uint32_t upd_frames = upd_all;
#pragma unroll
      for (int o = 16; o > 0; o >>= 1) upd_frames |= __shfl_xor_sync(0xffffffffu, upd_frames, o);
      if (lane == 0) {
        const uint32_t all = KB_FLAG_UPDATED | KB_FLAG_MESH_UPDATED | KB_FLAG_ESDF_UPDATED | KB_FLAG_TRACKING_UPDATED;
        if ((m.block_flags[slot] & all) != all) atomicOr(&m.block_flags[slot], all);
        if ((p.work_upd[wi] & upd_frames) != upd_frames) {
          const uint32_t prev = atomicOr(&p.work_upd[wi], upd_frames);
          const int fresh = __popc(upd_frames & ~prev);
          if (fresh) {
            atomicAdd(&m.counters[kCtrBlocksUpdated], fresh);
            atomicAdd(&totals64(m.counters)[kTotBlocksUpdated], static_cast<unsigned long long>(fresh));
          }
        }
      }
    }
  }
  n_valid = warpSum(n_valid);
  if (n_valid) {
    n_band = warpSum(n_band);
    n_sem = warpSum(n_sem);
    if (lane == 0) {
      unsigned long long* t64 = totals64(m.counters);
      atomicAdd(&m.counters[kCtrVoxelsUpdated], n_valid);
      atomicAdd(&t64[kTotVoxelsUpdated], static_cast<unsigned long long>(n_valid));
      if (n_band) {
        atomicAdd(&m.counters[kCtrVoxelsBand], n_band);
        atomicAdd(&t64[kTotVoxelsBand], static_cast<unsigned long long>(n_band));
      }
      if (n_sem) {
        atomicAdd(&m.counters[kCtrVoxelsSemantic], n_sem);
        atomicAdd(&t64[kTotVoxelsSemantic], static_cast<unsigned long long>(n_sem));
      }
    }
  }
}

__global__ void trackingPassKernel(const DeviceMap m, const TrackingParams p) {
  const int slot = blockIdx.x * blockDim.x + threadIdx.x;
  if (slot == 0) {
    for (uint32_t i = p.prev_pass + 1; i <= p.ev.k_last; ++i) m.next_pass[i] = p.ev.k_last;
    m.act_min[p.ev.k_last] = p.ev.act_min;
  }
  if (slot >= p.n_slots) return;
  const uint32_t flags = m.block_flags[slot];
  if (!(flags & kFlagAllocated)) return;
  uint32_t f = flags & ~(static_cast<uint32_t>(KB_FLAG_TRACKING_UPDATED) | kFlagInactiveOverride);
  if (flags & KB_FLAG_TRACKING_UPDATED) p.pending[atomicAdd(&m.counters[kCtrPending], 1)] = slot;
  if (f != flags) m.block_flags[slot] = f;
}

__device__ __forceinline__ bool voxelFreeNow(const DeviceMap& m, const TrackEval& t, size_t idx, uint8_t f) {
  if (f & kVoxEverFree) return true;
  if (!(f & kVoxNotOccupied)) return false;
  const uint32_t oc = m.last_occ[idx];
  return oc == 0 ? (t.zero_free != 0) : (oc < t.free_max);
}

__device__ __forceinline__ int ghostLookup(const TrackingParams& p, int x, int y, int z) {
  const unsigned long long key = packKey(x, y, z);
  uint32_t h = static_cast<uint32_t>(mix64(key)) & p.ghost_mask;
  for (uint32_t probe = 0; probe <= p.ghost_mask; ++probe) {
    const unsigned long long k = p.ghost_keys[h];
    if (k == key) return p.ghost_vals[h];
    if (k == kEmptyKey) return -1;
    h = (h + 1) & p.ghost_mask;
  }
  return -1;
}

template <bool SHARD>
__global__ void __launch_bounds__(kThreads) everFreeKernel(const DeviceMap m, const TrackingParams p) {
  __shared__ int s_nbr[27];
  __shared__ uint8_t s_free[18 * 18 * 18];
  const int n = m.counters[kCtrPending];
  const int vps = m.vps, V = m.V, hs = vps + 2;
  for (int w = blockIdx.x; w < n; w += gridDim.x) {
    const int slot = p.pending[w];
    __syncthreads();
    if (threadIdx.x < 27) {
      const int3 bi = m.block_index[slot];
      const int dx = threadIdx.x % 3 - 1, dy = (threadIdx.x / 3) % 3 - 1, dz = threadIdx.x / 9 - 1;
      int ns = (dx == 0 && dy == 0 && dz == 0) ? slot : hashLookup(m, bi.x + dx, bi.y + dy, bi.z + dz);
      if (SHARD && ns < 0 && mapOwner(m, bi.x + dx, bi.y + dy, bi.z + dz, p.nranks) != p.rank) {
        const int off = ghostLookup(p, bi.x + dx, bi.y + dy, bi.z + dz);
        if (off >= 0) ns = -(2 + off);
      }
      s_nbr[threadIdx.x] = ns;
    }
    __syncthreads();
    for (int i = threadIdx.x; i < hs * hs * hs; i += kThreads) {
      int x = i % hs - 1, y = (i / hs) % hs - 1, z = i / (hs * hs) - 1;
      int bx = 1, by = 1, bz = 1;
      if (x < 0) { x += vps; bx = 0; } else if (x >= vps) { x -= vps; bx = 2; }
      if (y < 0) { y += vps; by = 0; } else if (y >= vps) { y -= vps; by = 2; }
      if (z < 0) { z += vps; bz = 0; } else if (z >= vps) { z -= vps; bz = 2; }
      const int ns = s_nbr[bx + 3 * by + 9 * bz];
      uint8_t v = 0;
      if (ns >= 0) {
        const size_t idx = static_cast<size_t>(ns) * V + (x + vps * (y + vps * z));
        const uint8_t f = m.vflags[idx];
        v = (voxelFreeNow(m, p.ev, idx, f) ? 1 : 0) | ((f & kVoxEverFree) ? 2 : 0);
      } else if (SHARD && ns <= -2) {
        const int lin = x + vps * (y + vps * z);
        v = (static_cast<uint32_t>(__ldg(&p.ghost_bits[(-ns - 2) + (lin >> 5)])) >> (lin & 31)) & 1u;
      }
      s_free[i] = v;
    }
    __syncthreads();
    const size_t base = static_cast<size_t>(slot) * V;
    for (int lin = threadIdx.x; lin < V; lin += kThreads) {
      const int vx = lin % vps, vy = (lin / vps) % vps, vz = lin / (vps * vps);
      const int c = (vx + 1) + hs * ((vy + 1) + hs * (vz + 1));
      if (s_free[c] != 1) continue;
      bool blocked = false;
      for (int dz = -1; dz <= 1 && !blocked; ++dz)
        for (int dy = -1; dy <= 1 && !blocked; ++dy)
          for (int dx = -1; dx <= 1; ++dx) {
// ... 435 lines not shown
                                     const unsigned long long* stamps, unsigned long long* last_obs,
                                     unsigned long long* last_occ, uint8_t* ever_free, uint8_t* active,
                                     uint8_t* to_remove, uint8_t* block_active) {
  const int V = m.V, slot = slots[blockIdx.x];
  const uint32_t born = m.born_frame[slot];
  int any_active = 0;
  for (int lin = threadIdx.x; lin < V; lin += blockDim.x) {
    const size_t src = static_cast<size_t>(slot) * V + lin, dst = static_cast<size_t>(blockIdx.x) * V + lin;
    const uint8_t f = m.vflags[src];
    const uint32_t o = m.last_obs[src];
    uint32_t c;
    bool act, rem;
    evalTracking(m, ev, born, o, m.last_occ[src], f, &c, &act, &rem);
    last_obs[dst] = stamps[o];
    last_occ[dst] = stamps[c];
    ever_free[dst] = (f & kVoxEverFree) ? 1 : 0;
    active[dst] = act ? 1 : 0;
    to_remove[dst] = rem ? 1 : 0;
    any_active |= act ? 1 : 0;
  }
  any_active = __syncthreads_or(any_active);
  if (threadIdx.x == 0) {
    const bool seen = ev.k_last != 0 && ev.k_last >= born;
    block_active[blockIdx.x] = (seen && any_active && !(m.block_flags[slot] & kFlagInactiveOverride)) ? 1 : 0;
  }
}

__global__ void gatherColorKernel(const DeviceMap m, const int* slots, uint8_t* rgb) {
  const int V = m.V, slot = slots[blockIdx.x];
  for (int lin = threadIdx.x; lin < V; lin += blockDim.x) {
    const uchar4 c = m.color[static_cast<size_t>(slot) * V + lin];
    uint8_t* o = rgb + (static_cast<size_t>(blockIdx.x) * V + lin) * 3;
    o[0] = c.x; o[1] = c.y; o[2] = c.z;
  }
}

__global__ void gatherSemanticKernel(const DeviceMap m, const int* slots, int L, uint32_t* label,
                                     uint8_t* empty, float* lik) {
  const int V = m.V, slot = slots[blockIdx.x];
  const int sem = m.block_sem[slot];
  for (int lin = threadIdx.x; lin < V; lin += blockDim.x) {
    const size_t dst = static_cast<size_t>(blockIdx.x) * V + lin;
    uint16_t lb = kSemEmpty;
    if (sem >= 0) lb = m.sem_label[static_cast<size_t>(sem) * V + lin];
    const bool is_empty = lb == kSemEmpty;
    label[dst] = is_empty ? 0u : lb;
    empty[dst] = is_empty ? 1 : 0;
    if (lik) {
      for (int k = 0; k < L; ++k)
        lik[dst * L + k] = is_empty ? 0.f : m.sem_lik[(static_cast<size_t>(sem) * V + lin) * m.Lp + k];
    }
  }
}

}

void launchExpandFrames(const BatchParams& p, cudaStream_t s) {
  expandFramesKernel<<<dim3(148, p.n_frames), 256, 0, s>>>(p);
}
void launchExpandDepth(const uint16_t* src, float scale, float* dst, int n, cudaStream_t s) {
  expandDepthKernel<<<(n + 255) / 256, 256, 0, s>>>(src, scale, dst, n);
}
void launchTileMax(const BatchParams& p, cudaStream_t s) {
  bool vec4 = !p.compact_taps && (p.W % 4) == 0;
  for (int b = 0; b < p.n_frames && vec4; ++b) vec4 = (reinterpret_cast<uintptr_t>(p.f[b].depth) & 15u) == 0;
  if (vec4) {
    const int warps = ((p.W + 127) / 128) * p.lvl_ty[1];
    tileMaxVec4Kernel<<<dim3((warps + 7) / 8, p.n_frames), 256, 0, s>>>(p);
  } else {
    const int warps = ((p.W + 31) / 32) * p.lvl_ty[1];
    tileMaxKernel<<<dim3((warps + 7) / 8, p.n_frames), 256, 0, s>>>(p);
  }
  tilePyramidKernel<<<p.n_frames, 256, 0, s>>>(p);
}
void launchSelectBlocks(const DeviceMap& m, const BatchParams& p, int cull_grid, cudaStream_t s) {
  const int n = p.allocate ? p.dims[0] * p.dims[1] * p.dims[2] : p.n_slots;
  if (p.pipelined) selectBlocksKernel<true><<<(std::max(n, 1) + 3) / 4, 128, 0, s>>>(m, p);
  else selectBlocksKernel<false><<<(std::max(n, 1) + 3) / 4, 128, 0, s>>>(m, p);
  if (p.cull) {
    if (m.vps == 16) itemCullKernel<16><<<cull_grid, 128, 0, s>>>(m, p);
    else itemCullKernel<8><<<cull_grid, 128, 0, s>>>(m, p);
  }
  if (p.item_list) {
    const bool pb = p.fetch_ctr == kCtrFetchB;
    cudaMemsetAsync(m.counters + (pb ? kCtrItemsB0 : kCtrItems0), 0, kItemClasses * sizeof(int), s);
    if (m.vps == 16) { if (pb) itemCompactKernel<16, true><<<cull_grid, 256, 0, s>>>(m, p); else itemCompactKernel<16, false><<<cull_grid, 256, 0, s>>>(m, p); }
    else { if (pb) itemCompactKernel<8, true><<<cull_grid, 256, 0, s>>>(m, p); else itemCompactKernel<8, false><<<cull_grid, 256, 0, s>>>(m, p); }
  }
}
static size_t fuseSmemBytes(int Lp) { return static_cast<size_t>(std::max(Lp, 2)) * kFuseThreads * sizeof(float); }
int fuseBlocksPerSm(int vps, int Lp) {
  int n = 0;
  if (vps == 16) cudaOccupancyMaxActiveBlocksPerMultiprocessor(&n, fuseKernel<16, 1, false, false>, kFuseThreads, fuseSmemBytes(Lp));
  else cudaOccupancyMaxActiveBlocksPerMultiprocessor(&n, fuseKernel<8, 1, false, false>, kFuseThreads, fuseSmemBytes(Lp));
  return n > 0 ? n : 4;
}
void launchFuse(const DeviceMap& m, const BatchParams& p, int grid, cudaStream_t s) {
  if (grid <= 0) return;
  const size_t smem = fuseSmemBytes(m.Lp);
  const bool one = p.layers_per_item == 1, c = p.compact_taps != 0, col = p.has_color != 0 && m.color != nullptr;
  const bool pb = p.fetch_ctr == kCtrFetchB;
#define KB_FUSE(V, LP, C)                                                                        \
  do {                                                                                           \
    if (pb) {                                                                                    \
      if (col) fuseKernel<V, LP, C, true, false, true><<<grid, kFuseThreads, smem, s>>>(m, p);   \
      else if (p.item_list) fuseKernel<V, LP, C, false, true, true><<<grid, kFuseThreads, smem, s>>>(m, p); \
      else fuseKernel<V, LP, C, false, false, true><<<grid, kFuseThreads, smem, s>>>(m, p);      \
    } else {                                                                                     \
      if (col) fuseKernel<V, LP, C, true><<<grid, kFuseThreads, smem, s>>>(m, p);                \
      else if (p.item_list) fuseKernel<V, LP, C, false, true><<<grid, kFuseThreads, smem, s>>>(m, p); \
      else fuseKernel<V, LP, C, false><<<grid, kFuseThreads, smem, s>>>(m, p);                   \
    }                                                                                            \
  } while (0)
#define KB_FUSE_MLP_G(V, LP, C, GG)                                                                                  \
  do {                                                                                                               \
    if (pb) {                                                                                                        \
      if (p.item_list) fuseKernelMlp<V, LP, C, GG, true, true><<<grid, kFuseThreads, smem, s>>>(m, p);               \
      else fuseKernelMlp<V, LP, C, GG, false, true><<<grid, kFuseThreads, smem, s>>>(m, p);                          \
    } else {                                                                                                         \
      if (p.item_list) fuseKernelMlp<V, LP, C, GG, true><<<grid, kFuseThreads, smem, s>>>(m, p);                     \
      else fuseKernelMlp<V, LP, C, GG, false><<<grid, kFuseThreads, smem, s>>>(m, p);                                \
    }                                                                                                                \
  } while (0)
#define KB_FUSE_MLP(V, LP, C)                                                                                        \
  do {                                                                                                               \
    if (p.mlp_group == 2) KB_FUSE_MLP_G(V, LP, C, 2);                                                                \
    else KB_FUSE_MLP_G(V, LP, C, 4);                                                                                 \
  } while (0)
  if (p.coop && p.item_list && one && !col && p.mlp_group == 0) {
    const size_t csmem = static_cast<size_t>(std::max(m.Lp, 2)) * 32 * sizeof(float) + 2 * 32 * 32 * sizeof(float) + 32 * 32;
#define KB_COOP(V, C)                                                                   \
  do {                                                                                  \
    if (pb) fuseKernelCoop<V, C, true><<<grid, kFuseThreads, csmem, s>>>(m, p);         \
    else fuseKernelCoop<V, C, false><<<grid, kFuseThreads, csmem, s>>>(m, p);           \
  } while (0)
    if (m.vps == 16) { if (c) KB_COOP(16, true); else KB_COOP(16, false); }
    else { if (c) KB_COOP(8, true); else KB_COOP(8, false); }
#undef KB_COOP
    return;
  }
  if (p.mlp_group != 0 && !col) {
    if (m.vps == 16) {
      if (one) { if (c) KB_FUSE_MLP(16, 1, true); else KB_FUSE_MLP(16, 1, false); }
      else { if (c) KB_FUSE_MLP(16, 4, true); else KB_FUSE_MLP(16, 4, false); }
    } else {
      if (one) { if (c) KB_FUSE_MLP(8, 1, true); else KB_FUSE_MLP(8, 1, false); }
      else { if (c) KB_FUSE_MLP(8, 4, true); else KB_FUSE_MLP(8, 4, false); }
    }
    return;
  }
  if (m.vps == 16) {
    if (one) { if (c) KB_FUSE(16, 1, true); else KB_FUSE(16, 1, false); }
    else { if (c) KB_FUSE(16, 4, true); else KB_FUSE(16, 4, false); }
  } else {
    if (one) { if (c) KB_FUSE(8, 1, true); else KB_FUSE(8, 1, false); }
    else { if (c) KB_FUSE(8, 4, true); else KB_FUSE(8, 4, false); }
  }
#undef KB_FUSE
#undef KB_FUSE_MLP
#undef KB_FUSE_MLP_G
}
void launchTrackingPass(const DeviceMap& m, const TrackingParams& p, int everfree_grid, cudaStream_t s) {
  trackingPassKernel<<<(std::max(p.n_slots, 1) + 255) / 256, 256, 0, s>>>(m, p);
  if (p.everfree_v2) everFreeKernelV2<false><<<everfree_grid, kThreads, 0, s>>>(m, p);
  else everFreeKernel<false><<<everfree_grid, kThreads, 0, s>>>(m, p);
  resetPendingKernel<<<1, 1, 0, s>>>(m);
}
void launchTrackingBegin(const DeviceMap& m, const TrackingParams& p, const ShardExchange& x, int32_t* pending_out, cudaStream_t s) {
  trackingPassKernel<<<(std::max(p.n_slots, 1) + 255) / 256, 256, 0, s>>>(m, p);
  exportPendingKernel<<<(x.cap_pending + 255) / 256, 256, 0, s>>>(m, p.pending, pending_out, x.cap_pending);
}
void launchHaloPack(const DeviceMap& m, const TrackingParams& p, const ShardExchange& x, const int32_t* all_pending,
                    int32_t* halo_out, cudaStream_t s) {
  const int n = x.nranks * x.cap_pending * 27;
  haloMarkKernel<<<(n + 255) / 256, 256, 0, s>>>(m, x, all_pending);
  haloPackKernel<<<148 * 4, kThreads, 0, s>>>(m, p, x, halo_out);
  haloUnmarkKernel<<<(m.max_blocks + 255) / 256, 256, 0, s>>>(m, x, m.max_blocks);
}
void launchTrackingBeginPeers(const DeviceMap& m, const TrackingParams& p, const ShardExchange& x, const PeerBuffers& peers, cudaStream_t s) {
  trackingPassKernel<<<(std::max(p.n_slots, 1) + 255) / 256, 256, 0, s>>>(m, p);
  exportPendingPeersKernel<<<(x.cap_pending + 255) / 256, 256, 0, s>>>(m, p.pending, peers, x.rank, x.pending_stride(), x.cap_pending);
}
void launchHaloPackPeers(const DeviceMap& m, const TrackingParams& p, const ShardExchange& x, const int32_t* all_pending,
                         const PeerBuffers& peers, cudaStream_t s) {
  const int n = x.nranks * x.cap_pending * 27;
  haloMarkKernel<<<(n + 255) / 256, 256, 0, s>>>(m, x, all_pending);
  haloPackPeersKernel<<<148 * 4, kThreads, 0, s>>>(m, p, x, peers);
  haloUnmarkKernel<<<(m.max_blocks + 255) / 256, 256, 0, s>>>(m, x, m.max_blocks);
}
void launchMulticastCopy(void* mc_dst, const void* src, size_t bytes, cudaStream_t s) {
  const size_t n16 = bytes / 16;
  if (n16 == 0) return;
  const int grid = static_cast<int>(std::min<size_t>((n16 + 255) / 256, 148 * 8));
  multicastCopyKernel<<<grid, 256, 0, s>>>(static_cast<float4*>(mc_dst), static_cast<const float4*>(src), n16);
}
void launchFlagScatter(const uint8_t* local_flags, const PeerBuffers& peers, int n, cudaStream_t s) {
  flagScatterKernel<<<(n + 255) / 256, 256, 0, s>>>(local_flags, peers, n);
}
void launchTrackingFinish(const DeviceMap& m, const TrackingParams& p, const ShardExchange& x, const int32_t* all_pending,
                          const int32_t* all_halo, int everfree_grid, cudaStream_t s) {
  cudaMemsetAsync(x.ghost_keys, 0xFF, (static_cast<size_t>(x.ghost_mask) + 1) * sizeof(unsigned long long), s);
  const int n = x.nranks * x.cap_halo;
  ghostBuildKernel<<<(n + 255) / 256, 256, 0, s>>>(m, x, all_pending, all_halo);
  if (p.everfree_v2) everFreeKernelV2<true><<<everfree_grid, kThreads, 0, s>>>(m, p);
  else everFreeKernel<true><<<everfree_grid, kThreads, 0, s>>>(m, p);
  resetPendingKernel<<<1, 1, 0, s>>>(m);
}
void launchResetInactive(const DeviceMap& m, const TrackEval& ev, int n, int3* removed, int max_removed, cudaStream_t s) {
  if (n > 0) resetInactiveKernel<<<n, kThreads, 0, s>>>(m, ev, removed, max_removed);
}
void launchRehash(const DeviceMap& m, int n, cudaStream_t s) {
  cudaMemsetAsync(m.hash_keys, 0xFF, (static_cast<size_t>(m.hash_mask) + 1) * sizeof(unsigned long long), s);
  rehashKernel<<<(std::max(n, 1) + 255) / 256, 256, 0, s>>>(m, n);
}
void launchMarkAllInactive(const DeviceMap& m, int n, cudaStream_t s) {
  if (n > 0) markAllInactiveKernel<<<(n + 255) / 256, 256, 0, s>>>(m, n);
}
void launchClearUpdated(const DeviceMap& m, int n, cudaStream_t s) {
  if (n > 0) clearUpdatedKernel<<<(n + 255) / 256, 256, 0, s>>>(m, n);
}
void launchMotionLookup(const DeviceMap& m, const MotionParams& p, cudaStream_t s) {
  const int n = p.W * p.H;
  motionLookupKernel<false><<<(n + 255) / 256, 256, 0, s>>>(m, p);
}
void launchMotionLookupLocal(const DeviceMap& m, const MotionParams& p, cudaStream_t s) {
  const int n = p.W * p.H;
  motionLookupKernel<true><<<(n + 255) / 256, 256, 0, s>>>(m, p);
}
void launchMotionFinalize(const DeviceMap& m, const uint8_t* flags, int3* gidx, uint8_t* seed, int n, cudaStream_t s) {
  motionFinalizeKernel<<<(n + 255) / 256, 256, 0, s>>>(m, flags, gidx, seed, n);
}
void launchAllocateBox(const DeviceMap& m, int3 lo, int3 dims, int rank, int nranks, uint32_t born, cudaStream_t s) {
  const int n = dims.x * dims.y * dims.z;
  if (n > 0) allocateBoxKernel<<<(n + 127) / 128, 128, 0, s>>>(m, lo, dims, rank, nranks, born);
}
void launchScanConfidence(const DeviceMap& m, float min_conf, float min_obs, float trunc, int n, cudaStream_t s) {
  if (n > 0) scanConfidenceKernel<<<n, kThreads, 0, s>>>(m, min_conf, min_obs, trunc);
}
void launchGatherTsdf(const DeviceMap& m, const int* slots, int n, float* dist, float* weight, cudaStream_t s) {
  if (n > 0) gatherTsdfKernel<<<n, 256, 0, s>>>(m, slots, dist, weight);
}
void launchGatherTracking(const DeviceMap& m, const TrackEval& ev, const int* slots, int n,
                          const unsigned long long* stamps, unsigned long long* last_obs,
                          unsigned long long* last_occ, uint8_t* ever_free, uint8_t* active, uint8_t* to_remove,
                          uint8_t* block_active, cudaStream_t s) {
  if (n > 0) gatherTrackingKernel<<<n, 256, 0, s>>>(m, ev, slots, stamps, last_obs, last_occ, ever_free, active, to_remove, block_active);
}
void launchGatherColor(const DeviceMap& m, const int* slots, int n, uint8_t* rgb, cudaStream_t s) {
  if (n > 0) gatherColorKernel<<<n, 256, 0, s>>>(m, slots, rgb);
}
void launchGatherSemantic(const DeviceMap& m, const int* slots, int n, int L, uint32_t* label, uint8_t* empty,
                          float* lik, cudaStream_t s) {
  if (n > 0) gatherSemanticKernel<<<n, 256, 0, s>>>(m, slots, L, label, empty, lik);
}

namespace {
__global__ void __launch_bounds__(256) checksumKernel(const DeviceMap m, int n_slots, const unsigned long long* __restrict__ stamps,
                                                      unsigned long long* __restrict__ out) {
  const int slot = blockIdx.x;
  if (slot >= n_slots || !(m.block_flags[slot] & kFlagAllocated)) return;
  const int3 bi = m.block_index[slot];
  const unsigned long long key = packKey(bi.x, bi.y, bi.z);
  const int sem = m.block_sem[slot];
  unsigned long long sum = 0, xr = 0, seen = 0;
  for (int lin = threadIdx.x; lin < m.V; lin += blockDim.x) {
    const size_t gi = static_cast<size_t>(slot) * m.V + lin;
    const float2 st = m.tsdf[gi];
    uint32_t label = 0xFFFFFFFFu;
    if (sem >= 0 && m.sem_label) {
      const uint16_t lb = m.sem_label[static_cast<size_t>(sem) * m.V + lin];
      if (lb != kSemEmpty) label = lb;
    }
    const unsigned long long stamp = m.last_obs ? stamps[m.last_obs[gi]] : 0ull;
    unsigned long long v = mix64(key ^ mix64(static_cast<unsigned long long>(lin) + 1ull));
    v = mix64(v ^ (static_cast<unsigned long long>(__float_as_uint(st.x)) | (static_cast<unsigned long long>(__float_as_uint(st.y)) << 32)));
    v = mix64(v ^ static_cast<unsigned long long>(label));
    v = mix64(v ^ stamp);
    sum += v;
    xr ^= v;
    seen += (stamp != 0ull || st.y > 0.f) ? 1ull : 0ull;
  }
#pragma unroll
  for (int o = 16; o > 0; o >>= 1) {
    sum += __shfl_xor_sync(0xffffffffu, sum, o);
    xr ^= __shfl_xor_sync(0xffffffffu, xr, o);
    seen += __shfl_xor_sync(0xffffffffu, seen, o);
  }
  if ((threadIdx.x & 31) == 0) {
    atomicAdd(&out[0], sum);
    atomicXor(&out[1], xr);
    atomicAdd(&out[3], seen);
  }
  if (threadIdx.x == 0) atomicAdd(&out[2], 1ull);
}
}

void launchChecksum(const DeviceMap& m, int n_slots, const unsigned long long* stamps, unsigned long long* out, cudaStream_t s) {
  if (n_slots > 0) checksumKernel<<<n_slots, 256, 0, s>>>(m, n_slots, stamps, out);
}


}
```

khronos_b200/csrc/kb_kernels.cuh:

```cuda
#pragma once

#include "kb_device.cuh"

namespace kb {

constexpr int kTileLevels = 4;
constexpr int kMaxBatch = 32;

struct FrameView {
  float R[9], t[3];
  const float* depth;
  const int* label;
  const int* mask;
  const int* object_image;
  const uint8_t* color;
  float* tiles;
  const uint16_t* depth16;
  const uint8_t* label8;
  float depth_scale;
  uint32_t frame_idx;
  int target_id;
};

struct BatchParams {
  int W, H;
  float fx, fy, cx, cy, min_range, max_range;
  float pl[4][2];
  float voxel_size, block_size, trunc, infl;
  int use_dropoff;
  float dropoff_eps;
  int constant_weight;
  float max_weight;
  int interp;
  float adaptive_thr;
  int sem_mode, L;
  float mle_diag, mle_off, mle_init;
  unsigned long long blocked_mask;
  int lo[3], dims[3];
  int allocate;
  int n_slots;
  int rank, nranks;
  int with_tracking;
  TrackEval trk;
  float occ_thr;
  int n_frames;
  int parity;
  int compact_taps;
  int cull;
  int has_color;
  int lvl_tx[kTileLevels], lvl_ty[kTileLevels], lvl_off[kTileLevels];
  int* work_slots;
  uint32_t* work_masks;
  uint32_t* work_upd;
  uint32_t* item_fmask;
  int pipelined;
  int fetch_ctr;
  int items_ctr;
  int coop;
  int mlp_group;
  int* item_list;
  int item_list_cap;
  int items_per_block;
  int layers_per_item;
  int max_work;
  FrameView f[kMaxBatch];
};

struct TrackingParams {
  TrackEval ev;
  uint32_t prev_pass;
  int connectivity;
  int n_slots;
  int* pending;
  int everfree_v2;
  int rank, nranks;
  const int32_t* ghost_bits;
  const unsigned long long* ghost_keys;
  const int* ghost_vals;
  uint32_t ghost_mask;
};

constexpr int kMaxPeers = 16;
struct PeerBuffers {
  void* p[kMaxPeers];
  int n;
};

struct ShardExchange {
  int rank, nranks;
  int cap_pending, cap_halo;
  int mask_words;
  int* halo_mark;
  int* publish;
  unsigned long long* ghost_keys;
  int* ghost_vals;
  uint32_t ghost_mask;
  __host__ __device__ int pending_stride() const { return 4 + 3 * cap_pending; }
  __host__ __device__ int halo_entry() const { return 4 + mask_words; }
  __host__ __device__ int halo_stride() const { return 4 + cap_halo * halo_entry(); }
};

struct MotionParams {
  float Rw[9], tw[3];
  int W, H;
  float fx, fy, cx, cy;
  float max_range, min_z_world;
  float block_size, block_size_inv, voxel_size_inv;
  const float* depth;
  const float* vertex;
  int3* pixel_gidx;
  uint8_t* pixel_seed;
  uint8_t* pixel_flags;
};

void launchTileMax(const BatchParams& p, cudaStream_t s);
void launchExpandFrames(const BatchParams& p, cudaStream_t s);
void launchExpandDepth(const uint16_t* src, float scale, float* dst, int n, cudaStream_t s);
void launchSelectBlocks(const DeviceMap& m, const BatchParams& p, int cull_grid, cudaStream_t s);
void launchFuse(const DeviceMap& m, const BatchParams& p, int grid, cudaStream_t s);
int fuseBlocksPerSm(int vps, int Lp);
void launchTrackingPass(const DeviceMap& m, const TrackingParams& p, int everfree_grid, cudaStream_t s);
void launchResetInactive(const DeviceMap& m, const TrackEval& ev, int n_slots, int3* removed, int max_removed, cudaStream_t s);
void launchRehash(const DeviceMap& m, int n_slots, cudaStream_t s);
void launchMarkAllInactive(const DeviceMap& m, int n_slots, cudaStream_t s);
void launchClearUpdated(const DeviceMap& m, int n_slots, cudaStream_t s);
void launchMotionLookup(const DeviceMap& m, const MotionParams& p, cudaStream_t s);
void launchMotionLookupLocal(const DeviceMap& m, const MotionParams& p, cudaStream_t s);
void launchMotionFinalize(const DeviceMap& m, const uint8_t* flags, int3* gidx, uint8_t* seed, int n, cudaStream_t s);
void launchTrackingBegin(const DeviceMap& m, const TrackingParams& p, const ShardExchange& x, int32_t* pending_out, cudaStream_t s);
void launchHaloPack(const DeviceMap& m, const TrackingParams& p, const ShardExchange& x, const int32_t* all_pending,
                    int32_t* halo_out, cudaStream_t s);
void launchTrackingBeginPeers(const DeviceMap& m, const TrackingParams& p, const ShardExchange& x, const PeerBuffers& peers, cudaStream_t s);
void launchHaloPackPeers(const DeviceMap& m, const TrackingParams& p, const ShardExchange& x, const int32_t* all_pending,
                         const PeerBuffers& peers, cudaStream_t s);
void launchFlagScatter(const uint8_t* local_flags, const PeerBuffers& peers, int n, cudaStream_t s);
void launchMulticastCopy(void* mc_dst, const void* src, size_t bytes, cudaStream_t s);
void launchTrackingFinish(const DeviceMap& m, const TrackingParams& p, const ShardExchange& x, const int32_t* all_pending,
                          const int32_t* all_halo, int everfree_grid, cudaStream_t s);
void launchAllocateBox(const DeviceMap& m, int3 lo, int3 dims, int rank, int nranks, uint32_t born, cudaStream_t s);
void launchScanConfidence(const DeviceMap& m, float min_conf, float min_obs, float trunc, int n_slots,
                          cudaStream_t s);

void launchGatherTsdf(const DeviceMap& m, const int* slots, int n, float* dist, float* weight, cudaStream_t s);
void launchGatherTracking(const DeviceMap& m, const TrackEval& ev, const int* slots, int n,
                          const unsigned long long* stamps, unsigned long long* last_obs,
                          unsigned long long* last_occ, uint8_t* ever_free, uint8_t* active, uint8_t* to_remove,
                          uint8_t* block_active, cudaStream_t s);
void launchGatherColor(const DeviceMap& m, const int* slots, int n, uint8_t* rgb, cudaStream_t s);
void launchGatherSemantic(const DeviceMap& m, const int* slots, int n, int L, uint32_t* label,
                          uint8_t* empty, float* lik, cudaStream_t s);

void launchChecksum(const DeviceMap& m, int n_slots, const unsigned long long* stamps, unsigned long long* out, cudaStream_t s);

}
```

Baseline: 180,300.

## Fuse multiple batches into one windowed fuse kernel with per-batch buffers

Adds a window mode that accumulates up to several pipelined item-listed batches, each with its own work buffers, counters and item lists, and launches a single fuse kernel over the whole window. Cross-batch ordering on shared voxels is handled through per-item sequence numbers (last_listed, item_prev, done). The goal is fewer fuse launches and less per-batch sync and tail idle time. It removes the unused coop and MLP fuse variants and adds an optional trace build, at the cost of more memory, added device-side dependency tracking, and possible stalls between dependent batches.

```diff
diff --git a/khronos_b200/build.py b/khronos_b200/build.py
--- a/khronos_b200/build.py
+++ b/khronos_b200/build.py
@@ -36,7 +36,8 @@
     return LIB
 
 
-VARIANTS = {"mb12": ["-DKB_FUSE_MIN_BLOCKS=12"], "mb8": ["-DKB_FUSE_MIN_BLOCKS=8"]}
+VARIANTS = {"mb12": ["-DKB_FUSE_MIN_BLOCKS=12"], "mb8": ["-DKB_FUSE_MIN_BLOCKS=8"],
+            "trace": ["-DKB_FUSE_TRACE"]}
 
 
 def build_variant(name):
diff --git a/khronos_b200/csrc/kb_api.cu b/khronos_b200/csrc/kb_api.cu
--- a/khronos_b200/csrc/kb_api.cu
+++ b/khronos_b200/csrc/kb_api.cu
@@ -53,27 +53,33 @@
   BatchParams batch{};
   float* tile_max = nullptr;
   size_t tile_stride = 0;
-  int* work_slots = nullptr;
-  uint32_t* work_masks = nullptr;
-  uint32_t* work_upd = nullptr;
-  uint32_t* item_fmask = nullptr;
-  int* item_list = nullptr;
+  struct BatchBufs {
+    int* work_slots = nullptr;
+    uint32_t* work_masks = nullptr;
+    uint32_t* work_upd = nullptr;
+    uint32_t* item_fmask = nullptr;
+    int* item_list = nullptr;
+    int* item_prev = nullptr;
+  };
+  std::vector<BatchBufs> bufs;
+  int* batch_ctr = nullptr;
   int item_list_cap = 0;
+  int win_g = 4;
+  int wpar = 0;
+  int win_n = 0;
+  WindowParams win{};
+  uint32_t seq = 0;
+  uint32_t* last_listed = nullptr;
+  uint32_t* done = nullptr;
   bool use_item_list = true;
   bool pipelined = true;
   cudaStream_t pre_stream = nullptr;
   cudaEvent_t pre_done[2] = {nullptr, nullptr}, fuse_done[2] = {nullptr, nullptr}, main_front = nullptr;
   bool main_dirty = true;
-  int* work_slots2 = nullptr;
-  uint32_t* work_masks2 = nullptr;
-  uint32_t* work_upd2 = nullptr;
-  uint32_t* item_fmask2 = nullptr;
   bool narrow_labels = false;
   int narrow_threads = 8;
   uint8_t* pin_label8 = nullptr;
   size_t pin_label8_pixels = 0;
-  int fuse_coop = 0;
-  int mlp_group = 0;
   int cull_grid = 0;
   int parity = 0;
   TrackEval pass{};
@@ -504,11 +510,7 @@
       KB_CUDA(h, cudaEventCreateWithFlags(&h->stg_ready[i], cudaEventDisableTiming));
       KB_CUDA(h, cudaEventCreateWithFlags(&h->stg_consumed[i], cudaEventDisableTiming));
     }
-    KB_CUDA(h, devAlloc(&h->work_slots, S, 0));
-    KB_CUDA(h, devAlloc(&h->work_masks, S, 0));
-    KB_CUDA(h, devAlloc(&h->work_upd, S, 0));
     h->batch.items_per_block = m.V / 128;
-    KB_CUDA(h, devAlloc(&h->item_fmask, S * h->batch.items_per_block, 0));
     if (const char* e = std::getenv("KB_FUSE_ITEM_LIST")) h->use_item_list = e[0] == '1';
     h->rehash_threshold = (static_cast<size_t>(cap)) / 4;
     if (const char* e = std::getenv("KB_REHASH_TOMBSTONES")) h->rehash_threshold = static_cast<size_t>(std::max(1, std::atoi(e)));
@@ -524,16 +526,23 @@
         KB_CUDA(h, cudaEventCreateWithFlags(&h->fuse_done[i], cudaEventDisableTiming));
       }
       KB_CUDA(h, cudaEventCreateWithFlags(&h->main_front, cudaEventDisableTiming));
-      KB_CUDA(h, devAlloc(&h->work_slots2, S, 0));
-      KB_CUDA(h, devAlloc(&h->work_masks2, S, 0));
-      KB_CUDA(h, devAlloc(&h->work_upd2, S, 0));
-      KB_CUDA(h, devAlloc(&h->item_fmask2, S * h->batch.items_per_block, 0));
-    }
-    if (const char* e = std::getenv("KB_FUSE_COOP")) h->fuse_coop = e[0] == '1' ? 1 : 0;
-    if (const char* e = std::getenv("KB_FUSE_MLP")) h->mlp_group = e[0] == '2' ? 2 : (e[0] == '4' ? 4 : 0);
-    if (h->use_item_list) {
-      h->item_list_cap = static_cast<int>(std::min<size_t>(S * h->batch.items_per_block, size_t(1) << 28));
-      KB_CUDA(h, devAlloc(&h->item_list, static_cast<size_t>(2 * kItemClasses) * h->item_list_cap, 0));
+    }
+    if (const char* e = std::getenv("KB_FUSE_WINDOW")) h->win_g = std::min(std::max(std::atoi(e), 1), kMaxWindow);
+    h->item_list_cap = static_cast<int>(std::min<size_t>(S * h->batch.items_per_block, size_t(1) << 28));
+    h->batch.item_list_cap = h->item_list_cap;
+    h->bufs.resize(h->pipelined ? 2 * h->win_g : 1);
+    for (auto& b : h->bufs) {
+      KB_CUDA(h, devAlloc(&b.work_slots, S, 0));
+      KB_CUDA(h, devAlloc(&b.work_masks, S, 0));
+      KB_CUDA(h, devAlloc(&b.work_upd, S, 0));
+      KB_CUDA(h, devAlloc(&b.item_fmask, S * h->batch.items_per_block, 0));
+      if (h->use_item_list) KB_CUDA(h, devAlloc(&b.item_list, static_cast<size_t>(h->item_list_cap), 0));
+      if (h->use_item_list && h->pipelined) KB_CUDA(h, devAlloc(&b.item_prev, static_cast<size_t>(h->item_list_cap), 0));
+    }
+    KB_CUDA(h, devAlloc(&h->batch_ctr, h->bufs.size() * kBatchCtrInts + 2, 0));
+    if (h->use_item_list && h->pipelined) {
+      KB_CUDA(h, devAlloc(&h->last_listed, S * h->batch.items_per_block, 0));
+      KB_CUDA(h, devAlloc(&h->done, S * h->batch.items_per_block * 4, 0));
     }
     {
       cudaDeviceProp prop{};
@@ -583,7 +592,9 @@
     cudaFree(t.pix_total); cudaFree(t.min_seed); cudaFree(t.cluster_id); cudaFree(t.roots); cudaFree(t.scalars); cudaFree(t.pix_slot); cudaFree(t.occupied); }
   if (h->h_mscal) cudaFreeHost(h->h_mscal);
   cudaFree(h->stg_depth16); cudaFree(h->stg_label8); cudaFree(h->mot_depth16);
-  cudaFree(h->mot_depth); cudaFree(h->tile_max); cudaFree(h->work_slots); cudaFree(h->work_masks); cudaFree(h->work_upd); cudaFree(h->item_fmask); cudaFree(h->item_list);
+  cudaFree(h->mot_depth); cudaFree(h->tile_max); cudaFree(h->batch_ctr);
+  cudaFree(h->last_listed); cudaFree(h->done);
+  for (auto& b : h->bufs) { cudaFree(b.work_slots); cudaFree(b.work_masks); cudaFree(b.work_upd); cudaFree(b.item_fmask); cudaFree(b.item_list); cudaFree(b.item_prev); }
   for (int i = 0; i < 2; ++i) {
     if (h->stg_ready[i]) cudaEventDestroy(h->stg_ready[i]);
     if (h->stg_consumed[i]) cudaEventDestroy(h->stg_consumed[i]);
@@ -596,7 +607,6 @@
     if (h->fuse_done[i]) cudaEventDestroy(h->fuse_done[i]);
   }
   if (h->main_front) cudaEventDestroy(h->main_front);
-  cudaFree(h->work_slots2); cudaFree(h->work_masks2); cudaFree(h->work_upd2); cudaFree(h->item_fmask2);
   cudaFree(h->shard_table_dev);
   cudaFree(h->inst_counts); cudaFree(h->inst_bbox); cudaFree(h->inst_background); cudaFree(h->inst_keep); cudaFree(h->inst_bad);
   cudaFree(h->mesh_slots); cudaFree(h->mesh_cases); cudaFree(h->mesh_tri_count); cudaFree(h->mesh_tri_base);
@@ -672,14 +682,10 @@
     p.lvl_off[l] = static_cast<int>(h->tile_stride);
     h->tile_stride += static_cast<size_t>(p.lvl_tx[l]) * p.lvl_ty[l];
   }
-  p.work_slots = h->work_slots;
-  p.work_masks = h->work_masks;
-  p.work_upd = h->work_upd;
-  p.item_fmask = h->item_fmask;
   p.max_work = h->dm.max_blocks;
   cudaFree(h->tile_max);
   h->tile_max = nullptr;
-  KB_CUDA(h, devAlloc(&h->tile_max, h->tile_stride * kMaxBatch * 2, 0));
+  KB_CUDA(h, devAlloc(&h->tile_max, h->tile_stride * kMaxBatch * h->bufs.size(), 0));
   return ensureMotionBuffers(h, static_cast<size_t>(c.width) * c.height);
 }
 
@@ -913,6 +919,19 @@
   HostFrustum f;
   hostFrustum(*camera, voxel_size * static_cast<float>(voxels_per_side), &f);
   return frameCellsImpl(f, frames, n_frames, cell_blocks, origin_cx, origin_cy, width, height, touched);
+}
+
+static int flushWindow(kb_handle* h) {
+  if (h->win_n == 0) return KB_OK;
+  const int wp = h->wpar;
+  h->win_n = 0;
+  h->wpar ^= 1;
+  KB_CUDA(h, cudaEventRecord(h->pre_done[wp], h->pre_stream));
+  KB_CUDA(h, cudaStreamWaitEvent(h->stream, h->pre_done[wp], 0));
+  launchFuseWindow(h->dm, h->win, h->fuse_grid, h->stream);
+  KB_CUDA(h, cudaEventRecord(h->fuse_done[wp], h->stream));
+  KB_CUDA(h, cudaGetLastError());
+  return KB_OK;
 }
 
 static int integrateBatch(kb_handle* h, const kb_frame* frames, int n, int allocate_blocks) {
@@ -947,13 +966,6 @@
   const bool pipe = h->pipelined && n >= 4;
   if (!pipe) h->main_dirty = true;
   p.pipelined = pipe ? 1 : 0;
-  p.fetch_ctr = (pipe && par) ? kCtrFetchB : kCtrFetch;
-  p.items_ctr = (pipe && par) ? kCtrItemsB0 : kCtrItems0;
-  p.work_slots = (pipe && par) ? h->work_slots2 : h->work_slots;
-  p.work_masks = (pipe && par) ? h->work_masks2 : h->work_masks;
-  p.work_upd = (pipe && par) ? h->work_upd2 : h->work_upd;
-  p.item_fmask = (pipe && par) ? h->item_fmask2 : h->item_fmask;
-  const size_t tile_set = (pipe && par) ? h->tile_stride * kMaxBatch : 0;
   p.cull = (h->cull && (n >= 4 || h->cull_forced)) ? 1 : 0;
   p.layers_per_item = n >= 8 ? 1 : 4;
   p.trk = h->pass;
@@ -966,18 +978,39 @@
     any_host_color |= frames[b].color != nullptr && frames[b].memory != KB_MEM_DEVICE;
   }
   p.has_color = any_color ? 1 : 0;
-  p.item_list = (h->use_item_list && p.cull && n >= 8 && !any_color)
-                    ? h->item_list + ((pipe && par) ? static_cast<size_t>(kItemClasses) * h->item_list_cap : 0) : nullptr;
-  p.item_list_cap = h->item_list_cap;
-  p.mlp_group = h->mlp_group;
-  p.coop = h->fuse_coop;
+  const bool use_staging = any_host || any_compact;
+  const bool listed = h->use_item_list && p.cull && n >= 8 && !any_color;
+  const bool windowed = pipe && listed && !use_staging;
+  if (!windowed) {
+    int st = flushWindow(h);
+    if (st != KB_OK) return st;
+  }
+  const int bset = pipe ? h->wpar * h->win_g + (windowed ? h->win_n : 0) : 0;
+  const kb_handle::BatchBufs& bb = h->bufs[bset];
+  p.work_slots = bb.work_slots;
+  p.work_masks = bb.work_masks;
+  p.work_upd = bb.work_upd;
+  p.item_fmask = bb.item_fmask;
+  p.item_list = listed ? bb.item_list : nullptr;
+  p.item_prev = windowed ? bb.item_prev : nullptr;
+  p.last_listed = h->last_listed;
+  p.seq = windowed ? ++h->seq : 0;
+  if (pipe) {
+    p.work_ctr = h->batch_ctr + static_cast<size_t>(bset) * kBatchCtrInts + kBatchWork;
+    p.cls_ctr = h->batch_ctr + static_cast<size_t>(bset) * kBatchCtrInts + kBatchCls;
+    p.fetch = h->batch_ctr + h->bufs.size() * kBatchCtrInts + h->wpar;
+  } else {
+    p.work_ctr = h->dm.counters + kCtrWork0 + par;
+    p.cls_ctr = h->dm.counters + kCtrItems0;
+    p.fetch = h->dm.counters + kCtrFetch;
+  }
+  const size_t tile_set = static_cast<size_t>(bset) * h->tile_stride * kMaxBatch;
   if (any_color) {
     int st = ensureColorLayer(h);
     if (st == KB_OK && any_host_color) st = ensureColorStaging(h, px);
     if (st != KB_OK) return st;
   }
   const int set = h->stg_set;
-  const bool use_staging = any_host || any_compact;
   if (use_staging) {
     int st = ensureStaging(h, px);
     if (st != KB_OK) return st;
@@ -1129,14 +1162,14 @@
   if (pipe) {
     ps = h->pre_stream;
     if (any_host) KB_CUDA(h, cudaStreamWaitEvent(ps, h->stg_ready[set], 0));
-    KB_CUDA(h, cudaStreamWaitEvent(ps, h->fuse_done[par], 0));
+    KB_CUDA(h, cudaStreamWaitEvent(ps, h->fuse_done[h->wpar], 0));
     if (h->main_dirty) {
       KB_CUDA(h, cudaEventRecord(h->main_front, h->stream));
       KB_CUDA(h, cudaStreamWaitEvent(ps, h->main_front, 0));
       h->main_dirty = false;
     }
-    KB_CUDA(h, cudaMemsetAsync(h->dm.counters + kCtrWork0 + par, 0, sizeof(int), ps));
-    KB_CUDA(h, cudaMemsetAsync(h->dm.counters + p.fetch_ctr, 0, sizeof(int), ps));
+    KB_CUDA(h, cudaMemsetAsync(p.work_ctr, 0, kBatchCtrInts * sizeof(int), ps));
+    if (!windowed || h->win_n == 0) KB_CUDA(h, cudaMemsetAsync(p.fetch, 0, sizeof(int), ps));
   }
   if (!pipe && h->pipelined) {
     KB_CUDA(h, cudaMemsetAsync(h->dm.counters + kCtrWork0 + par, 0, sizeof(int), ps));
@@ -1144,12 +1177,32 @@
   if (any_compact && !all_compact) launchExpandFrames(p, ps);
   if (p.cull) launchTileMax(p, ps);
   launchSelectBlocks(h->dm, p, h->cull_grid, ps);
-  if (pipe) {
-    KB_CUDA(h, cudaEventRecord(h->pre_done[par], ps));
-    KB_CUDA(h, cudaStreamWaitEvent(h->stream, h->pre_done[par], 0));
-  }
-  launchFuse(h->dm, p, h->fuse_grid, h->stream);
-  if (pipe) KB_CUDA(h, cudaEventRecord(h->fuse_done[par], h->stream));
+  if (windowed) {
+    WindowParams& w = h->win;
+    if (h->win_n == 0) {
+      static_cast<BatchCommon&>(w) = p;
+      w.seq0 = p.seq;
+      w.fetch = p.fetch;
+      w.done = h->done;
+    }
+    w.b[h->win_n] = WindowBatch{p.work_slots, p.work_upd, p.item_fmask, p.cls_ctr, p.item_list, p.item_prev, p.seq};
+    std::memcpy(w.f[h->win_n], p.f, sizeof(p.f));
+    w.n_batches = ++h->win_n;
+    if (h->win_n == h->win_g) {
+      int st = flushWindow(h);
+      if (st != KB_OK) return st;
+    }
+  } else {
+    if (pipe) {
+      KB_CUDA(h, cudaEventRecord(h->pre_done[h->wpar], ps));
+      KB_CUDA(h, cudaStreamWaitEvent(h->stream, h->pre_done[h->wpar], 0));
+    }
+    launchFuse(h->dm, p, h->fuse_grid, h->stream);
+    if (pipe) {
+      KB_CUDA(h, cudaEventRecord(h->fuse_done[h->wpar], h->stream));
+      h->wpar ^= 1;
+    }
+  }
   KB_CUDA(h, cudaGetLastError());
   if (use_staging) KB_CUDA(h, cudaEventRecord(h->stg_consumed[set], h->stream));
   if (any_host) {
@@ -1179,8 +1232,12 @@
   }
   if (!h->own_stream) h->main_dirty = true;
   for (int i = 0; i < n_frames; i += kMaxBatch) {
-    if ((st = integrateBatch(h, frames + i, std::min(kMaxBatch, n_frames - i), allocate_blocks)) != KB_OK) return st;
-  }
+    if ((st = integrateBatch(h, frames + i, std::min(kMaxBatch, n_frames - i), allocate_blocks)) != KB_OK) {
+      flushWindow(h);
+      return st;
+    }
+  }
+  if ((st = flushWindow(h)) != KB_OK) return st;
   if (stats) {
     if ((st = readCounters(h)) != KB_OK) return st;
     const int* c1 = h->h_ctr;
diff --git a/khronos_b200/csrc/kb_device.cuh b/khronos_b200/csrc/kb_device.cuh
--- a/khronos_b200/csrc/kb_device.cuh
+++ b/khronos_b200/csrc/kb_device.cuh
@@ -65,13 +65,14 @@
   kCtrPending = 18,
   kCtrFetch = 19,
   kCtrHalo = 20,
-  kCtrFetchB = 24,
   kCtrRehash = 28,
   kCtrItems0 = 32,
-  kCtrItemsB0 = 40,
   kNumCounters = 48
 };
 constexpr int kItemClasses = 8;
+constexpr int kBatchWork = 0;
+constexpr int kBatchCls = 8;
+constexpr int kBatchCtrInts = 32;
 
 enum Total64 {
   kTotVoxelsUpdated = 0,
diff --git a/khronos_b200/csrc/kb_kernels.cu b/khronos_b200/csrc/kb_kernels.cu
--- a/khronos_b200/csrc/kb_kernels.cu
+++ b/khronos_b200/csrc/kb_kernels.cu
@@ -1,6 +1,7 @@
 #include <limits.h>
 
 #include <algorithm>
+#include <type_traits>
 
 #include "../../include/khronos_b200.h"
 #include "kb_kernels.cuh"
@@ -55,7 +56,7 @@
 };
 
 template <bool COMPACT>
-__device__ __forceinline__ Taps nearestTaps(const BatchParams& p, const FrameView& f, float u, float v) {
+__device__ __forceinline__ Taps nearestTaps(const BatchCommon& p, const FrameView& f, float u, float v) {
   Taps t;
   t.bilinear = false;
   t.u = static_cast<int>(roundf(u));
@@ -66,7 +67,7 @@
 }
 
 template <bool COMPACT>
-__device__ __forceinline__ Taps computeTaps(const BatchParams& p, const FrameView& f, float u, float v, float& range) {
+__device__ __forceinline__ Taps computeTaps(const BatchCommon& p, const FrameView& f, float u, float v, float& range) {
   Taps t;
   t.valid = false;
   if (p.interp == KB_INTERP_NEAREST) {
@@ -113,7 +114,7 @@
   return t;
 }
 
-__device__ __forceinline__ int tapIndex(const BatchParams& p, const Taps& t) {
+__device__ __forceinline__ int tapIndex(const BatchCommon& p, const Taps& t) {
   int du = 0, dv = 0;
   if (t.bilinear) {
     int best = 0;
@@ -127,7 +128,7 @@
   return (t.v + dv) * p.W + t.u + du;
 }
 
-__device__ __forceinline__ float measurementWeight(const BatchParams& p, float depth, float sdf) {
+__device__ __forceinline__ float measurementWeight(const BatchCommon& p, float depth, float sdf) {
   float w = (p.fx * p.fy) * (p.voxel_size * p.voxel_size) / (depth * depth);
   if (!p.constant_weight) w = w / (depth * depth);
   if (p.use_dropoff && sdf < -p.dropoff_eps) {
@@ -137,7 +138,7 @@
   return w;
 }
 
-__device__ __forceinline__ uchar3 measuredColor(const BatchParams& p, const FrameView& f, const Taps& t) {
+__device__ __forceinline__ uchar3 measuredColor(const BatchCommon& p, const FrameView& f, const Taps& t) {
   const uint8_t* __restrict__ p0 = f.color + (static_cast<size_t>(t.v) * p.W + t.u) * 3;
   if (!t.bilinear) return make_uchar3(__ldg(p0), __ldg(p0 + 1), __ldg(p0 + 2));
   const uint8_t* __restrict__ p1 = p0 + static_cast<size_t>(p.W) * 3;
@@ -383,7 +384,7 @@
     }
     atomicAdd(&m.counters[kCtrPairs], __popc(mask));
     atomicAdd(&totals64(m.counters)[kTotPairs], static_cast<unsigned long long>(__popc(mask)));
-    i = atomicAdd(&m.counters[kCtrWork0 + p.parity], 1);
+    i = atomicAdd(p.work_ctr, 1);
     if (i < p.max_work) {
       p.work_slots[i] = slot;
       p.work_masks[i] = mask;
@@ -404,7 +405,7 @@
   const int warp = (blockIdx.x * blockDim.x + threadIdx.x) >> 5;
   const int n_warps = (gridDim.x * blockDim.x) >> 5;
   const int chunks = (p.n_frames + kCullChunk - 1) / kCullChunk;
-  const int n = min(m.counters[kCtrWork0 + p.parity], p.max_work) * chunks;
+  const int n = min(*p.work_ctr, p.max_work) * chunks;
   for (int w = warp; w < n; w += n_warps) {
     const int wi = w / chunks, ch = w % chunks;
     const uint32_t bmask = p.work_masks[wi] & (((kCullChunk >= 32 ? 0u : (1u << kCullChunk)) - 1u) << (ch * kCullChunk));
@@ -427,12 +428,17 @@
   }
 }
 
-template <int VPS, bool PB>
+template <int VPS, bool SCATTER>
 __global__ void __launch_bounds__(256) itemCompactKernel(const DeviceMap m, const __grid_constant__ BatchParams p) {
-  constexpr int kItems = PB ? kCtrItemsB0 : kCtrItems0;
   constexpr int BOXES = (VPS / 4) * (VPS / 8) * (VPS / 4);
-  const int n = min(m.counters[kCtrWork0 + p.parity], p.max_work) * BOXES;
+  const int n = min(*p.work_ctr, p.max_work) * BOXES;
   const int lane = threadIdx.x & 31;
+  int base_of[kItemClasses];
+  if constexpr (SCATTER) {
+    int b = 0;
+#pragma unroll
+    for (int c = 0; c < kItemClasses; ++c) { base_of[c] = b; b += p.cls_ctr[c]; }
+  }
   for (int base = (blockIdx.x * blockDim.x + threadIdx.x) - lane; base < n; base += gridDim.x * blockDim.x) {
     const int i = base + lane;
     const uint32_t fm = i < n ? p.item_fmask[i] : 0u;
@@ -441,22 +447,75 @@
     if (cls < 0) continue;
     const int leader = __ffs(peers) - 1;
     int start = 0;
-    if (lane == leader) start = atomicAdd(&m.counters[kItems + cls], __popc(peers));
-    start = __shfl_sync(peers, start, leader);
-    const int idx = start + __popc(peers & ((1u << lane) - 1u));
-    if (idx < p.item_list_cap) p.item_list[static_cast<size_t>(cls) * p.item_list_cap + idx] = i;
-  }
-}
-
-template <bool PB>
-__device__ __forceinline__ int listedBox(const BatchParams& p, const int (&n_cls)[kItemClasses], int j) {
-  int k = 0;
+    if (lane == leader) start = atomicAdd(&p.cls_ctr[(SCATTER ? kItemClasses : 0) + cls], __popc(peers));
+    if constexpr (SCATTER) {
+      start = __shfl_sync(peers, start, leader);
+      int b = 0;
 #pragma unroll
-  for (int c = 0; c < kItemClasses - 1; ++c) {
-    if (k == c && j >= n_cls[c]) { j -= n_cls[c]; k = c + 1; }
-  }
-  return p.item_list[static_cast<size_t>(k) * p.item_list_cap + j];
-}
+      for (int c = 0; c < kItemClasses; ++c) b = c == cls ? base_of[c] : b;
+      const int idx = b + start + __popc(peers & ((1u << lane) - 1u));
+      if (idx < p.item_list_cap) {
+        p.item_list[idx] = i;
+        if (p.item_prev) p.item_prev[idx] = static_cast<int>(atomicExch(&p.last_listed[static_cast<size_t>(p.work_slots[i / BOXES]) * BOXES + i % BOXES], p.seq));
+      }
+    }
+  }
+}
+
+__device__ __forceinline__ int listedItems(const int* cls_ctr, int cap) {
+  int n = 0;
+#pragma unroll
+  for (int c = 0; c < kItemClasses; ++c) n += cls_ctr[c];
+  return min(n, cap);
+}
+template <bool WIN, class P>
+__device__ __forceinline__ WindowBatch batchAt(const P& p, int g) {
+  if constexpr (WIN) return p.b[g];
+  else return WindowBatch{p.work_slots, p.work_upd, p.item_fmask, p.cls_ctr, p.item_list, p.item_prev, p.seq};
+}
+template <bool WIN, class P>
+__device__ __forceinline__ const FrameView& frameAt(const P& p, int g, int b) {
+  if constexpr (WIN) return p.f[g][b];
+  else return p.f[b];
+}
+__device__ __forceinline__ uint32_t ldAcquireGpu(const uint32_t* a) {
+  uint32_t v;
+  asm volatile("ld.acquire.gpu.global.u32 %0, [%1];" : "=r"(v) : "l"(a) : "memory");
+  return v;
+}
+__device__ __forceinline__ void stReleaseGpu(uint32_t* a, uint32_t v) {
+  asm volatile("st.release.gpu.global.u32 [%0], %1;" ::"l"(a), "r"(v) : "memory");
+}
+
+#ifdef KB_FUSE_TRACE
+struct FuseTraceRec {
+  unsigned long long t0, t1;
+  unsigned long long wait_ns;
+  uint32_t launch, smid, items, pad;
+};
+constexpr unsigned kFuseTraceCap = 1u << 21;
+__device__ FuseTraceRec g_fuse_trace[kFuseTraceCap];
+__device__ unsigned g_fuse_trace_n, g_fuse_trace_launch, g_fuse_trace_exited;
+__device__ __forceinline__ unsigned long long globalTimer() {
+  unsigned long long t;
+  asm volatile("mov.u64 %0, %%globaltimer;" : "=l"(t));
+  return t;
+}
+__device__ __forceinline__ void fuseTraceExit(unsigned long long t0, uint32_t launch, int items, unsigned long long wait_ns) {
+  if ((threadIdx.x & 31) != 0) return;
+  const unsigned long long t1 = globalTimer();
+  uint32_t smid;
+  asm volatile("mov.u32 %0, %%smid;" : "=r"(smid));
+  const unsigned i = atomicAdd(&g_fuse_trace_n, 1u);
+  if (i < kFuseTraceCap) g_fuse_trace[i] = FuseTraceRec{t0, t1, wait_ns, launch, smid, static_cast<uint32_t>(items), 0u};
+  __threadfence();
+  const unsigned warps = gridDim.x * (blockDim.x >> 5);
+  if (atomicAdd(&g_fuse_trace_exited, 1u) == warps - 1) {
+    g_fuse_trace_exited = 0;
+    atomicAdd(&g_fuse_trace_launch, 1u);
+  }
+}
+#endif
 
 __device__ __noinline__ uint32_t trackingFold(const DeviceMap m, const TrackEval t, uint32_t born, size_t gi) {
   const uint8_t fl = m.vflags[gi];
@@ -468,47 +527,92 @@
   return (fl & kVoxEverFree) | (act ? kVoxActive : 0) | (rem ? kVoxToRemove : 0);
 }
 
-template <int VPS, int LPI, bool COMPACT, bool COLOR, bool LIST = false, bool PB = false>
-__global__ void __launch_bounds__(kFuseThreads, COLOR ? KB_FUSE_COLOR_MIN_BLOCKS : KB_FUSE_MIN_BLOCKS) fuseKernel(const DeviceMap m, const __grid_constant__ BatchParams p) {
-  constexpr int kFetch = PB ? kCtrFetchB : kCtrFetch;
-  [[maybe_unused]] constexpr int kItems = PB ? kCtrItemsB0 : kCtrItems0;
+template <int VPS, int LPI, bool COMPACT, bool COLOR, bool LIST = false, bool WIN = false>
+__global__ void __launch_bounds__(kFuseThreads, COLOR ? KB_FUSE_COLOR_MIN_BLOCKS : KB_FUSE_MIN_BLOCKS)
+fuseKernel(const DeviceMap m, const __grid_constant__ std::conditional_t<WIN, WindowParams, BatchParams> p) {
+  static_assert(!WIN || (LIST && LPI == 1), "windows run listed one-layer items");
   constexpr int V = VPS * VPS * VPS;
   constexpr int NK = 4;
   constexpr int BOXES = (VPS / 4) * (VPS / 8) * (VPS / NK);
   extern __shared__ float s_rows[];
+  __shared__ int s_start[kMaxWindow + 1];
   const int lane = threadIdx.x & 31;
   constexpr int lpi = LPI, ipb = NK / LPI;
-  int n_cls[kItemClasses] = {0};
   int n_items;
-  if constexpr (LIST) {
-    n_items = 0;
-#pragma unroll
-    for (int c = 0; c < kItemClasses; ++c) {
-      n_cls[c] = min(m.counters[kItems + c], p.item_list_cap);
-      n_items += n_cls[c];
-    }
-    n_items *= ipb;
+  if constexpr (WIN) {
+    if (threadIdx.x == 0) {
+      int n = 0;
+      for (int g = 0; g < p.n_batches; ++g) {
+        s_start[g] = n;
+        n += listedItems(p.b[g].cls_ctr, p.item_list_cap) * ipb;
+      }
+      s_start[p.n_batches] = n;
+    }
+    __syncthreads();
+    n_items = s_start[p.n_batches];
+  } else if constexpr (LIST) {
+    n_items = listedItems(p.cls_ctr, p.item_list_cap) * ipb;
   } else {
-    n_items = min(m.counters[kCtrWork0 + p.parity], p.max_work) * BOXES * ipb;
+    n_items = min(*p.work_ctr, p.max_work) * BOXES * ipb;
   }
   const bool binary = p.sem_mode == KB_SEMANTICS_BINARY;
   const int L = p.L;
   int n_valid = 0, n_band = 0, n_sem = 0;
 
   int pending = 0;
-  if (lane == 0) pending = atomicAdd(&m.counters[kFetch], 1);
+#ifdef KB_FUSE_TRACE
+  const uint32_t tr_launch = *reinterpret_cast<volatile unsigned*>(&g_fuse_trace_launch);
+  const unsigned long long tr_t0 = globalTimer();
+  unsigned long long tr_wait = 0;
+  int tr_items = 0;
+#endif
+  if (lane == 0) pending = atomicAdd(p.fetch, 1);
   for (;;) {
     const int w = __shfl_sync(0xffffffffu, pending, 0);
     if (w >= n_items) break;
-    if (lane == 0) pending = atomicAdd(&m.counters[kFetch], 1);
-    int box = w / ipb;
+    if (lane == 0) pending = atomicAdd(p.fetch, 1);
+#ifdef KB_FUSE_TRACE
+    ++tr_items;
+#endif
+    int g = 0, wl = w;
+    if constexpr (WIN) {
+      while (g + 1 < p.n_batches && w >= s_start[g + 1]) ++g;
+      wl = w - s_start[g];
+    }
+    const WindowBatch bt = batchAt<WIN>(p, g);
+    int box = wl / ipb;
+    uint32_t prev = 0;
     if constexpr (LIST) {
-      box = listedBox<PB>(p, n_cls, box);
-    }
-    const uint32_t fmask = p.item_fmask[box];
-    if (!fmask) continue;
+      if constexpr (WIN) prev = static_cast<uint32_t>(bt.item_prev[box]);
+      box = bt.item_list[box];
+    }
+    const uint32_t fmask = bt.item_fmask[box];
     const int wi = box / BOXES, it = box % BOXES;
-    const int slot = p.work_slots[wi];
+    uint32_t tix = 0;
+    if constexpr (WIN) {
+      tix = (static_cast<uint32_t>(bt.work_slots[wi]) * BOXES + it) * NK + wl % ipb;
+      if (lane == 0 && prev >= p.seq0) {
+#ifdef KB_FUSE_TRACE
+        const unsigned long long tw = globalTimer();
+#endif
+        unsigned ns = 32;
+        while (ldAcquireGpu(p.done + tix) < prev) {
+          __nanosleep(ns);
+          ns = min(ns * 2u, 1024u);
+        }
+#ifdef KB_FUSE_TRACE
+        tr_wait += globalTimer() - tw;
+#endif
+      }
+      __syncwarp();
+    }
+    if (!fmask) {
+      if constexpr (WIN) {
+        if (lane == 0) stReleaseGpu(p.done + tix, p.b[g].seq);
+      }
+      continue;
+    }
+    const int slot = bt.work_slots[wi];
     const int3 bi = m.block_index[slot];
     const int sem = L > 0 ? m.block_sem[slot] : -1;
     int x0, y0, z0;
@@ -534,7 +638,7 @@
     while (rem) {
       const int b = __ffs(rem) - 1;
       rem &= rem - 1;
-      const FrameView& f = p.f[b];
+      const FrameView& f = frameAt<WIN>(p, g, b);
       const bool has_label_img = L > 0 && (binary ? f.object_image != nullptr : (COMPACT ? f.label8 != nullptr : f.label != nullptr));
       float x, y, z;
       xform(f.R, f.t, wx, wy, wz, x, y, z);
@@ -658,6 +762,10 @@
     upd_all |= upd_frames;
     any_have |= have;
     }
+    if constexpr (WIN) {
+      __syncwarp();
+      if (lane == 0) stReleaseGpu(p.done + tix, p.b[g].seq);
+    }
     if (__any_sync(0xffffffffu, any_have)) {
       uint32_t upd_frames = upd_all;
 #pragma unroll
@@ -665,8 +773,8 @@
       if (lane == 0) {
         const uint32_t all = KB_FLAG_UPDATED | KB_FLAG_MESH_UPDATED | KB_FLAG_ESDF_UPDATED | KB_FLAG_TRACKING_UPDATED;
         if ((m.block_flags[slot] & all) != all) atomicOr(&m.block_flags[slot], all);
-        if ((p.work_upd[wi] & upd_frames) != upd_frames) {
-          const uint32_t prev = atomicOr(&p.work_upd[wi], upd_frames);
+        if ((batchAt<WIN>(p, g).work_upd[wi] & upd_frames) != upd_frames) {
+          const uint32_t prev = atomicOr(&batchAt<WIN>(p, g).work_upd[wi], upd_frames);
           const int fresh = __popc(upd_frames & ~prev);
           if (fresh) {
             atomicAdd(&m.counters[kCtrBlocksUpdated], fresh);
@@ -694,537 +802,9 @@
       }
     }
   }
-}
-
-template <int VPS, bool COMPACT, bool PB>
-__global__ void __launch_bounds__(kFuseThreads, KB_FUSE_MIN_BLOCKS) fuseKernelCoop(const DeviceMap m, const __grid_constant__ BatchParams p) {
-  constexpr int kFetch = PB ? kCtrFetchB : kCtrFetch;
-  constexpr int kItems = PB ? kCtrItemsB0 : kCtrItems0;
-  constexpr int V = VPS * VPS * VPS;
-  constexpr int NK = 4;
-  constexpr int BOXES = (VPS / 4) * (VPS / 8) * (VPS / NK);
-  constexpr uint8_t kInvalid = 0xFE, kNoSem = 0xFF;
-  extern __shared__ float s_dyn[];
-  const int rows_floats = max(m.Lp, 2) * 32;
-  float* __restrict__ s_rows = s_dyn;
-  float* __restrict__ s_w = s_dyn + rows_floats;
-  float* __restrict__ s_s = s_w + 32 * 32;
-  uint8_t* __restrict__ s_l = reinterpret_cast<uint8_t*>(s_s + 32 * 32);
-  __shared__ int s_item;
-  const int warp = threadIdx.x >> 5, lane = threadIdx.x & 31;
-  int n_cls[kItemClasses];
-  int n_items = 0;
-#pragma unroll
-  for (int c = 0; c < kItemClasses; ++c) {
-    n_cls[c] = min(m.counters[kItems + c], p.item_list_cap);
-    n_items += n_cls[c];
-  }
-  n_items *= NK;
-  const bool binary = p.sem_mode == KB_SEMANTICS_BINARY;
-  const int L = p.L;
-  int n_valid = 0, n_band = 0, n_sem = 0;
-  int pending = 0;
-  if (threadIdx.x == 0) pending = atomicAdd(&m.counters[kFetch], 1);
-  for (;;) {
-    if (threadIdx.x == 0) s_item = pending;
-    __syncthreads();
-    const int w = s_item;
-    if (w >= n_items) break;
-    if (threadIdx.x == 0) pending = atomicAdd(&m.counters[kFetch], 1);
-    const int box = listedBox<PB>(p, n_cls, w / NK);
-    const uint32_t fmask = p.item_fmask[box];
-    const int wi = box / BOXES, it = box % BOXES;
-    const int slot = p.work_slots[wi];
-    const int3 bi = m.block_index[slot];
-    const int sem = L > 0 ? m.block_sem[slot] : -1;
-    int x0, y0, z0;
-    itemOrigin<VPS>(it, x0, y0, z0);
-    const int vx = x0 + (lane & 3), vy = y0 + (lane >> 2), vz = z0 + (w % NK);
-    const int lin = vx + VPS * (vy + VPS * vz);
-    const size_t gi = static_cast<size_t>(slot) * V + lin;
-    const float wx = static_cast<float>(bi.x) * p.block_size + (static_cast<float>(vx) + 0.5f) * p.voxel_size;
-    const float wy = static_cast<float>(bi.y) * p.block_size + (static_cast<float>(vy) + 0.5f) * p.voxel_size;
-    const float wz = static_cast<float>(bi.z) * p.block_size + (static_cast<float>(vz) + 0.5f) * p.voxel_size;
-    const int nf = __popc(fmask);
-    for (int r = warp; r < nf; r += 4) {
-      const int b = __fns(fmask, 0, r + 1);
-      const FrameView& f = p.f[b];
-      const bool has_label_img = L > 0 && (binary ? f.object_image != nullptr : (COMPACT ? f.label8 != nullptr : f.label != nullptr));
-      uint8_t tag = kInvalid;
-      float sdf = 0.f, wm = 0.f;
-      float x, y, z;
-      xform(f.R, f.t, wx, wy, wz, x, y, z);
-      if (z > 0.f) {
-        const float u = p.fx * x / z + p.cx;
-        const float v = p.fy * y / z + p.cy;
-        if (!(u < 0.f || u > static_cast<float>(p.W - 1) || v < 0.f || v > static_cast<float>(p.H - 1))) {
-          float range = 0.f;
-          const Taps taps = computeTaps<COMPACT>(p, f, u, v, range);
-          if (taps.valid) {
-            sdf = range - z;
-            if (!(sdf < -p.trunc)) {
-              bool ok = true;
-              uint32_t label = 0;
-              const bool in_band = fabsf(sdf) < p.trunc;
-              if (in_band) {
-                const int ti = tapIndex(p, taps);
-                if (f.mask != nullptr && __ldg(&f.mask[ti]) != 0) ok = false;
-                if (ok && has_label_img) {
-                  if (binary) {
-                    label = __ldg(&f.object_image[ti]) == f.target_id ? 1u : 0u;
-                  } else {
-                    label = static_cast<uint32_t>(labelAt<COMPACT>(f, ti));
-                    if (label < static_cast<uint32_t>(KB_MAX_LABELS) && ((p.blocked_mask >> label) & 1ull)) ok = false;
-                  }
-                }
-              }
-              if (ok) {
-                wm = measurementWeight(p, z, sdf);
-                tag = (in_band && sem >= 0 && has_label_img && label < static_cast<uint32_t>(L)) ? static_cast<uint8_t>(label) : kNoSem;
-              }
-            }
-          }
-        }
-      }
-      s_w[r * 32 + lane] = wm;
-      s_s[r * 32 + lane] = sdf;
-      s_l[r * 32 + lane] = tag;
-    }
-    __syncthreads();
-    if (warp == 0) {
-      float2 st = make_float2(0.f, 0.f);
-      uint32_t lobs = 0, vfl = 0, upd_frames = 0;
-      bool have = false, row_resident = false;
-      int best_label = 0;
-      uint32_t rem = fmask;
-      int r = 0;
-      while (rem) {
-        const int b = __ffs(rem) - 1;
-        rem &= rem - 1;
-        const uint8_t tag = s_l[r * 32 + lane];
-        const float wm = s_w[r * 32 + lane], sdf = s_s[r * 32 + lane];
-        ++r;
-        if (tag == kInvalid) continue;
-        if (!have) {
-          st = m.tsdf[gi];
-          have = true;
-          if (p.with_tracking) vfl = trackingFold(m, p.trk, m.born_frame[slot], gi);
-        }
-        const float sdf_c = fminf(fmaxf(sdf, -p.trunc), p.trunc);
-        const float2 old = st;
-        st.x = (old.x * old.y + sdf_c * wm) / (old.y + wm);
-        st.y = fminf(old.y + wm, p.max_weight);
-        lobs = p.f[b].frame_idx;
-        upd_frames |= 1u << b;
-        ++n_valid;
-        if (!(fabsf(sdf) < p.trunc)) continue;
-        ++n_band;
-        if (tag == kNoSem) continue;
-        const uint32_t label = tag;
-        const size_t si = static_cast<size_t>(sem) * V + lin;
-        if (!row_resident) {
-          row_resident = true;
-          const bool empty = m.sem_label[si] == kSemEmpty;
-          if (binary) {
-            const float2 c = empty ? make_float2(0.f, 0.f) : *reinterpret_cast<const float2*>(m.sem_lik + si * 2);
-            s_rows[lane] = c.x;
-            s_rows[32 + lane] = c.y;
-          } else {
-            const float4* __restrict__ lk = reinterpret_cast<const float4*>(m.sem_lik + si * m.Lp);
-            for (int k4 = 0; k4 < m.Lp; k4 += 4) {
-              const float4 c = empty ? make_float4(p.mle_init, p.mle_init, p.mle_init, p.mle_init) : lk[k4 >> 2];
-              s_rows[(k4 + 0) * 32 + lane] = c.x;
-              s_rows[(k4 + 1) * 32 + lane] = c.y;
-              s_rows[(k4 + 2) * 32 + lane] = c.z;
-              s_rows[(k4 + 3) * 32 + lane] = c.w;
-            }
-          }
-        }
-        if (binary) {
-          s_rows[label * 32 + lane] = s_rows[label * 32 + lane] + 1.f;
-          best_label = s_rows[32 + lane] > s_rows[lane] ? 1 : 0;
-        } else {
-          for (int k2 = 0; k2 < m.Lp; k2 += 2) {
-            float c0 = s_rows[(k2 + 0) * 32 + lane], c1 = s_rows[(k2 + 1) * 32 + lane];
-            c0 += static_cast<uint32_t>(k2 + 0) == label ? p.mle_diag : p.mle_off;
-            c1 += static_cast<uint32_t>(k2 + 1) == label ? p.mle_diag : p.mle_off;
-            s_rows[(k2 + 0) * 32 + lane] = c0;
-            s_rows[(k2 + 1) * 32 + lane] = c1;
-          }
-        }
-        ++n_sem;
-      }
-      if (have) {
-        m.tsdf[gi] = st;
-        if (p.with_tracking) {
-          m.last_obs[gi] = lobs;
-          m.vflags[gi] = static_cast<uint8_t>(vfl | (st.x < p.occ_thr ? 0 : kVoxNotOccupied));
-        }
-        if (row_resident) {
-          const size_t si = static_cast<size_t>(sem) * V + lin;
-          if (binary) {
-            *reinterpret_cast<float2*>(m.sem_lik + si * 2) = make_float2(s_rows[lane], s_rows[32 + lane]);
-          } else {
-            float4* __restrict__ lk = reinterpret_cast<float4*>(m.sem_lik + si * m.Lp);
-            for (int k4 = 0; k4 < m.Lp; k4 += 4)
-              lk[k4 >> 2] = make_float4(s_rows[(k4 + 0) * 32 + lane], s_rows[(k4 + 1) * 32 + lane], s_rows[(k4 + 2) * 32 + lane],
-                                        s_rows[(k4 + 3) * 32 + lane]);
-            float bestv = s_rows[lane];
-            best_label = 0;
-            for (int kk = 1; kk < L; ++kk) {
-              const float c = s_rows[kk * 32 + lane];
-              if (c > bestv) { bestv = c; best_label = kk; }
-            }
-          }
-          m.sem_label[si] = static_cast<uint16_t>(best_label);
-        }
-      }
-      if (__any_sync(0xffffffffu, have)) {
-#pragma unroll
-        for (int o = 16; o > 0; o >>= 1) upd_frames |= __shfl_xor_sync(0xffffffffu, upd_frames, o);
-        if (lane == 0) {
-          const uint32_t all = KB_FLAG_UPDATED | KB_FLAG_MESH_UPDATED | KB_FLAG_ESDF_UPDATED | KB_FLAG_TRACKING_UPDATED;
-          if ((m.block_flags[slot] & all) != all) atomicOr(&m.block_flags[slot], all);
-          if ((p.work_upd[wi] & upd_frames) != upd_frames) {
-            const uint32_t prev = atomicOr(&p.work_upd[wi], upd_frames);
-            const int fresh = __popc(upd_frames & ~prev);
-            if (fresh) {
-              atomicAdd(&m.counters[kCtrBlocksUpdated], fresh);
-              atomicAdd(&totals64(m.counters)[kTotBlocksUpdated], static_cast<unsigned long long>(fresh));
-            }
-          }
-        }
-      }
-    }
-  }
-  if (warp == 0) {
-    n_valid = warpSum(n_valid);
-    if (n_valid) {
-      n_band = warpSum(n_band);
-      n_sem = warpSum(n_sem);
-      if (lane == 0) {
-        unsigned long long* t64 = totals64(m.counters);
-        atomicAdd(&m.counters[kCtrVoxelsUpdated], n_valid);
-        atomicAdd(&t64[kTotVoxelsUpdated], static_cast<unsigned long long>(n_valid));
-        if (n_band) {
-          atomicAdd(&m.counters[kCtrVoxelsBand], n_band);
-          atomicAdd(&t64[kTotVoxelsBand], static_cast<unsigned long long>(n_band));
-        }
-        if (n_sem) {
-          atomicAdd(&m.counters[kCtrVoxelsSemantic], n_sem);
-          atomicAdd(&t64[kTotVoxelsSemantic], static_cast<unsigned long long>(n_sem));
-        }
-      }
-    }
-  }
-}
-
-#ifndef KB_FUSE_MLP_MIN_BLOCKS
-#define KB_FUSE_MLP_MIN_BLOCKS 5
+#ifdef KB_FUSE_TRACE
+  fuseTraceExit(tr_t0, tr_launch, tr_items, tr_wait);
 #endif
-template <int VPS, int LPI, bool COMPACT, int G, bool LIST, bool PB = false>
-__global__ void __launch_bounds__(kFuseThreads, KB_FUSE_MLP_MIN_BLOCKS) fuseKernelMlp(const DeviceMap m, const __grid_constant__ BatchParams p) {
-  constexpr int kFetch = PB ? kCtrFetchB : kCtrFetch;
-  [[maybe_unused]] constexpr int kItems = PB ? kCtrItemsB0 : kCtrItems0;
-  constexpr int V = VPS * VPS * VPS;
-  constexpr int NK = 4;
-  constexpr int BOXES = (VPS / 4) * (VPS / 8) * (VPS / NK);
-  extern __shared__ float s_rows[];
-  const int lane = threadIdx.x & 31;
-  constexpr int lpi = LPI, ipb = NK / LPI;
-  int n_cls[kItemClasses] = {0};
-  int n_items;
-  if constexpr (LIST) {
-    n_items = 0;
-#pragma unroll
-    for (int c = 0; c < kItemClasses; ++c) {
-      n_cls[c] = min(m.counters[kItems + c], p.item_list_cap);
-      n_items += n_cls[c];
-    }
-    n_items *= ipb;
-  } else {
-    n_items = min(m.counters[kCtrWork0 + p.parity], p.max_work) * BOXES * ipb;
-  }
-  const bool binary = p.sem_mode == KB_SEMANTICS_BINARY;
-  const int L = p.L;
-  const int W = p.W, H = p.H;
-  int n_valid = 0, n_band = 0, n_sem = 0;
-
-  int pending = 0;
-  if (lane == 0) pending = atomicAdd(&m.counters[kFetch], 1);
-  for (;;) {
-    const int w = __shfl_sync(0xffffffffu, pending, 0);
-    if (w >= n_items) break;
-    if (lane == 0) pending = atomicAdd(&m.counters[kFetch], 1);
-    int box = w / ipb;
-    if constexpr (LIST) {
-      box = listedBox<PB>(p, n_cls, box);
-    }
-    const uint32_t fmask = p.item_fmask[box];
-    if (!fmask) continue;
-    const int wi = box / BOXES, it = box % BOXES;
-    const int slot = p.work_slots[wi];
-    const int3 bi = m.block_index[slot];
-    const int sem = L > 0 ? m.block_sem[slot] : -1;
-    int x0, y0, z0;
-    itemOrigin<VPS>(it, x0, y0, z0);
-    uint32_t upd_all = 0;
-    bool any_have = false;
-#pragma unroll 1
-    for (int k = (w % ipb) * lpi; k < (w % ipb) * lpi + lpi; ++k) {
-      const int vx = x0 + (lane & 3), vy = y0 + (lane >> 2), vz = z0 + k;
-      const int lin = vx + VPS * (vy + VPS * vz);
-      const size_t gi = static_cast<size_t>(slot) * V + lin;
-      const float wx = static_cast<float>(bi.x) * p.block_size + (static_cast<float>(vx) + 0.5f) * p.voxel_size;
-      const float wy = static_cast<float>(bi.y) * p.block_size + (static_cast<float>(vy) + 0.5f) * p.voxel_size;
-      const float wz = static_cast<float>(bi.z) * p.block_size + (static_cast<float>(vz) + 0.5f) * p.voxel_size;
-      float2 st = make_float2(0.f, 0.f);
-      uint32_t lobs = 0, vfl = 0, upd_frames = 0;
-      bool have = false, row_resident = false;
-      int best_label = 0;
-
-      uint32_t rem = fmask;
-#pragma unroll 1
-      while (rem) {
-        int fb[G];
-        bool ok[G], inside[G];
-        int u0[G], v0[G];
-        float fz[G], du[G], dv[G], r0[G], r1[G], r2[G], r3[G];
-#pragma unroll
-        for (int g = 0; g < G; ++g) {
-          ok[g] = false;
-          fb[g] = 0;
-          if (rem) {
-            const int b = __ffs(rem) - 1;
-            rem &= rem - 1;
-            fb[g] = b;
-            const FrameView& f = p.f[b];
-            float x, y, z;
-            xform(f.R, f.t, wx, wy, wz, x, y, z);
-            const float zs = z > 0.f ? z : 1.f;
-            const float u = p.fx * x / zs + p.cx;
-            const float v = p.fy * y / zs + p.cy;
-            const bool o = z > 0.f && !(u < 0.f || u > static_cast<float>(W - 1) || v < 0.f || v > static_cast<float>(H - 1));
-            const int iu = o ? static_cast<int>(floorf(u)) : 0, iv = o ? static_cast<int>(floorf(v)) : 0;
-            ok[g] = o;
-            fz[g] = z;
-            u0[g] = iu;
-            v0[g] = iv;
-            du[g] = u - static_cast<float>(iu);
-            dv[g] = v - static_cast<float>(iv);
-            inside[g] = iu + 1 < W && iv + 1 < H;
-            const int iu1 = min(iu + 1, W - 1), iv1 = min(iv + 1, H - 1);
-            r0[g] = depthAt<COMPACT>(f, iv * W + iu);
-            r2[g] = depthAt<COMPACT>(f, iv * W + iu1);
-            r1[g] = depthAt<COMPACT>(f, iv1 * W + iu);
-            r3[g] = depthAt<COMPACT>(f, iv1 * W + iu1);
-          }
-        }
-        bool valid[G], band[G];
-        float sdfc[G], wm[G];
-        uint32_t lab[G];
-        int maskv[G];
-#pragma unroll
-        for (int g = 0; g < G; ++g) {
-          valid[g] = false;
-          band[g] = false;
-          sdfc[g] = 0.f;
-          wm[g] = 0.f;
-          lab[g] = 0;
-          maskv[g] = 0;
-          if (!ok[g]) continue;
-          const FrameView& f = p.f[fb[g]];
-          const bool ru = du[g] >= 0.5f, rv = dv[g] >= 0.5f;
-          const float rn = ru ? (rv ? r3[g] : r2[g]) : (rv ? r1[g] : r0[g]);
-          bool tv = false, bil = false;
-          float range = 0.f, w0 = 0.f, w1 = 0.f, w2 = 0.f, w3 = 0.f;
-          if (p.interp == KB_INTERP_NEAREST) {
-            tv = rn > 0.f;
-            range = rn;
-          } else {
-            bool use_nearest = !inside[g], reject = false;
-            if (inside[g]) {
-              const bool all_valid = r0[g] > 0.f && r1[g] > 0.f && r2[g] > 0.f && r3[g] > 0.f;
-              if (p.interp == KB_INTERP_ADAPTIVE) {
-                const float mx = fmaxf(fmaxf(r0[g], r1[g]), fmaxf(r2[g], r3[g]));
-                const float mn = fminf(fminf(r0[g], r1[g]), fminf(r2[g], r3[g]));
-                use_nearest = !all_valid || !(mx - mn < p.adaptive_thr);
-              } else if (!all_valid) {
-                reject = true;
-              }
-            } else if (p.interp != KB_INTERP_ADAPTIVE) {
-              reject = true;
-            }
-            if (!reject) {
-              if (use_nearest) {
-                tv = rn > 0.f;
-                range = rn;
-              } else {
-                tv = true;
-                bil = true;
-                w0 = (1.f - du[g]) * (1.f - dv[g]);
-                w1 = (1.f - du[g]) * dv[g];
-                w2 = du[g] * (1.f - dv[g]);
-                w3 = du[g] * dv[g];
-                range = ((w0 * r0[g] + w1 * r1[g]) + w2 * r2[g]) + w3 * r3[g];
-              }
-            }
-          }
-          if (!tv) continue;
-          const float sdf = range - fz[g];
-          if (sdf < -p.trunc) continue;
-          valid[g] = true;
-          band[g] = fabsf(sdf) < p.trunc;
-          sdfc[g] = fminf(fmaxf(sdf, -p.trunc), p.trunc);
-          wm[g] = measurementWeight(p, fz[g], sdf);
-          if (band[g]) {
-            int tu = u0[g] + (ru ? 1 : 0), tvv = v0[g] + (rv ? 1 : 0);
-            if (bil) {
-              int best = 0;
-              float bw = w0;
-              if (w1 > bw) { best = 1; bw = w1; }
-              if (w2 > bw) { best = 2; bw = w2; }
-              if (w3 > bw) { best = 3; }
-              tu = u0[g] + (best >> 1);
-              tvv = v0[g] + (best & 1);
-            }
-            const int ti = tvv * W + tu;
-            if (f.mask != nullptr) maskv[g] = __ldg(&f.mask[ti]);
-            const bool has_label_img = L > 0 && (binary ? f.object_image != nullptr : (COMPACT ? f.label8 != nullptr : f.label != nullptr));
-            if (has_label_img) {
-              if (binary) lab[g] = __ldg(&f.object_image[ti]) == f.target_id ? 1u : 0u;
-              else lab[g] = static_cast<uint32_t>(labelAt<COMPACT>(f, ti));
-            }
-          }
-        }
-#pragma unroll
-        for (int g = 0; g < G; ++g) {
-          if (!valid[g]) continue;
-          const int b = fb[g];
-          const FrameView& f = p.f[b];
-          const bool has_label_img = L > 0 && (binary ? f.object_image != nullptr : (COMPACT ? f.label8 != nullptr : f.label != nullptr));
-          const uint32_t label = lab[g];
-          if (band[g]) {
-            if (maskv[g] != 0) continue;
-            if (has_label_img && !binary && label < static_cast<uint32_t>(KB_MAX_LABELS) && ((p.blocked_mask >> label) & 1ull)) continue;
-          }
-          if (!have) {
-            st = m.tsdf[gi];
-            have = true;
-            if (p.with_tracking) vfl = trackingFold(m, p.trk, m.born_frame[slot], gi);
-          }
-          const float2 old = st;
-          st.x = (old.x * old.y + sdfc[g] * wm[g]) / (old.y + wm[g]);
-          st.y = fminf(old.y + wm[g], p.max_weight);
-          lobs = f.frame_idx;
-          upd_frames |= 1u << b;
-          ++n_valid;
-          if (!band[g]) continue;
-          ++n_band;
-          if (sem >= 0 && has_label_img && label < static_cast<uint32_t>(L)) {
-            const size_t si = static_cast<size_t>(sem) * V + lin;
-            if (!row_resident) {
-              row_resident = true;
-              const bool empty = m.sem_label[si] == kSemEmpty;
-              if (binary) {
-                const float2 c = empty ? make_float2(0.f, 0.f) : *reinterpret_cast<const float2*>(m.sem_lik + si * 2);
-                s_rows[threadIdx.x] = c.x;
-                s_rows[kFuseThreads + threadIdx.x] = c.y;
-              } else {
-                const float4* __restrict__ lk = reinterpret_cast<const float4*>(m.sem_lik + si * m.Lp);
-                for (int k4 = 0; k4 < m.Lp; k4 += 4) {
-                  const float4 c = empty ? make_float4(p.mle_init, p.mle_init, p.mle_init, p.mle_init) : lk[k4 >> 2];
-                  s_rows[(k4 + 0) * kFuseThreads + threadIdx.x] = c.x;
-                  s_rows[(k4 + 1) * kFuseThreads + threadIdx.x] = c.y;
-                  s_rows[(k4 + 2) * kFuseThreads + threadIdx.x] = c.z;
-                  s_rows[(k4 + 3) * kFuseThreads + threadIdx.x] = c.w;
-                }
-              }
-            }
-            if (binary) {
-              const float c = s_rows[label * kFuseThreads + threadIdx.x] + 1.f;
-              s_rows[label * kFuseThreads + threadIdx.x] = c;
-              best_label = s_rows[kFuseThreads + threadIdx.x] > s_rows[threadIdx.x] ? 1 : 0;
-            } else {
-              for (int k2 = 0; k2 < m.Lp; k2 += 2) {
-                float c0 = s_rows[(k2 + 0) * kFuseThreads + threadIdx.x], c1 = s_rows[(k2 + 1) * kFuseThreads + threadIdx.x];
-                c0 += static_cast<uint32_t>(k2 + 0) == label ? p.mle_diag : p.mle_off;
-                c1 += static_cast<uint32_t>(k2 + 1) == label ? p.mle_diag : p.mle_off;
-                s_rows[(k2 + 0) * kFuseThreads + threadIdx.x] = c0;
-                s_rows[(k2 + 1) * kFuseThreads + threadIdx.x] = c1;
-              }
-            }
-            ++n_sem;
-          }
-        }
-      }
-
-      if (have) {
-        m.tsdf[gi] = st;
-        if (p.with_tracking) {
-          m.last_obs[gi] = lobs;
-          m.vflags[gi] = static_cast<uint8_t>(vfl | (st.x < p.occ_thr ? 0 : kVoxNotOccupied));
-        }
-        if (row_resident) {
-          const size_t si = static_cast<size_t>(sem) * V + lin;
-          if (binary) {
-            *reinterpret_cast<float2*>(m.sem_lik + si * 2) = make_float2(s_rows[threadIdx.x], s_rows[kFuseThreads + threadIdx.x]);
-          } else {
-            float4* __restrict__ lk = reinterpret_cast<float4*>(m.sem_lik + si * m.Lp);
-            for (int k4 = 0; k4 < m.Lp; k4 += 4)
-              lk[k4 >> 2] = make_float4(s_rows[(k4 + 0) * kFuseThreads + threadIdx.x], s_rows[(k4 + 1) * kFuseThreads + threadIdx.x],
-                                        s_rows[(k4 + 2) * kFuseThreads + threadIdx.x], s_rows[(k4 + 3) * kFuseThreads + threadIdx.x]);
-          }
-          if (!binary) {
-            float bestv = s_rows[threadIdx.x];
-            best_label = 0;
-            for (int kk = 1; kk < L; ++kk) {
-              const float c = s_rows[kk * kFuseThreads + threadIdx.x];
-              if (c > bestv) { bestv = c; best_label = kk; }
-            }
-          }
-          m.sem_label[si] = static_cast<uint16_t>(best_label);
-        }
-      }
-      upd_all |= upd_frames;
-      any_have |= have;
-    }
-    if (__any_sync(0xffffffffu, any_have)) {
-      uint32_t upd_frames = upd_all;
-#pragma unroll
-      for (int o = 16; o > 0; o >>= 1) upd_frames |= __shfl_xor_sync(0xffffffffu, upd_frames, o);
-      if (lane == 0) {
-        const uint32_t all = KB_FLAG_UPDATED | KB_FLAG_MESH_UPDATED | KB_FLAG_ESDF_UPDATED | KB_FLAG_TRACKING_UPDATED;
-        if ((m.block_flags[slot] & all) != all) atomicOr(&m.block_flags[slot], all);
-        if ((p.work_upd[wi] & upd_frames) != upd_frames) {
-          const uint32_t prev = atomicOr(&p.work_upd[wi], upd_frames);
-          const int fresh = __popc(upd_frames & ~prev);
-          if (fresh) {
-            atomicAdd(&m.counters[kCtrBlocksUpdated], fresh);
-            atomicAdd(&totals64(m.counters)[kTotBlocksUpdated], static_cast<unsigned long long>(fresh));
-          }
-        }
-      }
-    }
-  }
-  n_valid = warpSum(n_valid);
-  if (n_valid) {
-    n_band = warpSum(n_band);
-    n_sem = warpSum(n_sem);
-    if (lane == 0) {
-      unsigned long long* t64 = totals64(m.counters);
-      atomicAdd(&m.counters[kCtrVoxelsUpdated], n_valid);
-      atomicAdd(&t64[kTotVoxelsUpdated], static_cast<unsigned long long>(n_valid));
-      if (n_band) {
-        atomicAdd(&m.counters[kCtrVoxelsBand], n_band);
-        atomicAdd(&t64[kTotVoxelsBand], static_cast<unsigned long long>(n_band));
-      }
-      if (n_sem) {
-        atomicAdd(&m.counters[kCtrVoxelsSemantic], n_sem);
-        atomicAdd(&t64[kTotVoxelsSemantic], static_cast<unsigned long long>(n_sem));
-      }
-    }
-  }
 }
 
 __global__ void trackingPassKernel(const DeviceMap m, const TrackingParams p) {
@@ -1826,10 +1406,14 @@
     else itemCullKernel<8><<<cull_grid, 128, 0, s>>>(m, p);
   }
   if (p.item_list) {
-    const bool pb = p.fetch_ctr == kCtrFetchB;
-    cudaMemsetAsync(m.counters + (pb ? kCtrItemsB0 : kCtrItems0), 0, kItemClasses * sizeof(int), s);
-    if (m.vps == 16) { if (pb) itemCompactKernel<16, true><<<cull_grid, 256, 0, s>>>(m, p); else itemCompactKernel<16, false><<<cull_grid, 256, 0, s>>>(m, p); }
-    else { if (pb) itemCompactKernel<8, true><<<cull_grid, 256, 0, s>>>(m, p); else itemCompactKernel<8, false><<<cull_grid, 256, 0, s>>>(m, p); }
+    cudaMemsetAsync(p.cls_ctr, 0, 2 * kItemClasses * sizeof(int), s);
+    if (m.vps == 16) {
+      itemCompactKernel<16, false><<<cull_grid, 256, 0, s>>>(m, p);
+      itemCompactKernel<16, true><<<cull_grid, 256, 0, s>>>(m, p);
+    } else {
+      itemCompactKernel<8, false><<<cull_grid, 256, 0, s>>>(m, p);
+      itemCompactKernel<8, true><<<cull_grid, 256, 0, s>>>(m, p);
+    }
   }
 }
 static size_t fuseSmemBytes(int Lp) { return static_cast<size_t>(std::max(Lp, 2)) * kFuseThreads * sizeof(float); }
@@ -1843,56 +1427,12 @@
   if (grid <= 0) return;
   const size_t smem = fuseSmemBytes(m.Lp);
   const bool one = p.layers_per_item == 1, c = p.compact_taps != 0, col = p.has_color != 0 && m.color != nullptr;
-  const bool pb = p.fetch_ctr == kCtrFetchB;
 #define KB_FUSE(V, LP, C)                                                                        \
   do {                                                                                           \
-    if (pb) {                                                                                    \
-      if (col) fuseKernel<V, LP, C, true, false, true><<<grid, kFuseThreads, smem, s>>>(m, p);   \
-      else if (p.item_list) fuseKernel<V, LP, C, false, true, true><<<grid, kFuseThreads, smem, s>>>(m, p); \
-      else fuseKernel<V, LP, C, false, false, true><<<grid, kFuseThreads, smem, s>>>(m, p);      \
-    } else {                                                                                     \
-      if (col) fuseKernel<V, LP, C, true><<<grid, kFuseThreads, smem, s>>>(m, p);                \
-      else if (p.item_list) fuseKernel<V, LP, C, false, true><<<grid, kFuseThreads, smem, s>>>(m, p); \
-      else fuseKernel<V, LP, C, false><<<grid, kFuseThreads, smem, s>>>(m, p);                   \
-    }                                                                                            \
+    if (col) fuseKernel<V, LP, C, true><<<grid, kFuseThreads, smem, s>>>(m, p);                  \
+    else if (p.item_list) fuseKernel<V, LP, C, false, true><<<grid, kFuseThreads, smem, s>>>(m, p); \
+    else fuseKernel<V, LP, C, false><<<grid, kFuseThreads, smem, s>>>(m, p);                     \
   } while (0)
-#define KB_FUSE_MLP_G(V, LP, C, GG)                                                                                  \
-  do {                                                                                                               \
-    if (pb) {                                                                                                        \
-      if (p.item_list) fuseKernelMlp<V, LP, C, GG, true, true><<<grid, kFuseThreads, smem, s>>>(m, p);               \
-      else fuseKernelMlp<V, LP, C, GG, false, true><<<grid, kFuseThreads, smem, s>>>(m, p);                          \
-    } else {                                                                                                         \
-      if (p.item_list) fuseKernelMlp<V, LP, C, GG, true><<<grid, kFuseThreads, smem, s>>>(m, p);                     \
-      else fuseKernelMlp<V, LP, C, GG, false><<<grid, kFuseThreads, smem, s>>>(m, p);                                \
-    }                                                                                                                \
-  } while (0)
-#define KB_FUSE_MLP(V, LP, C)                                                                                        \
-  do {                                                                                                               \
-    if (p.mlp_group == 2) KB_FUSE_MLP_G(V, LP, C, 2);                                                                \
-    else KB_FUSE_MLP_G(V, LP, C, 4);                                                                                 \
-  } while (0)
-  if (p.coop && p.item_list && one && !col && p.mlp_group == 0) {
-    const size_t csmem = static_cast<size_t>(std::max(m.Lp, 2)) * 32 * sizeof(float) + 2 * 32 * 32 * sizeof(float) + 32 * 32;
-#define KB_COOP(V, C)                                                                   \
-  do {                                                                                  \
-    if (pb) fuseKernelCoop<V, C, true><<<grid, kFuseThreads, csmem, s>>>(m, p);         \
-    else fuseKernelCoop<V, C, false><<<grid, kFuseThreads, csmem, s>>>(m, p);           \
-  } while (0)
-    if (m.vps == 16) { if (c) KB_COOP(16, true); else KB_COOP(16, false); }
-    else { if (c) KB_COOP(8, true); else KB_COOP(8, false); }
-#undef KB_COOP
-    return;
-  }
-  if (p.mlp_group != 0 && !col) {
-    if (m.vps == 16) {
-      if (one) { if (c) KB_FUSE_MLP(16, 1, true); else KB_FUSE_MLP(16, 1, false); }
-      else { if (c) KB_FUSE_MLP(16, 4, true); else KB_FUSE_MLP(16, 4, false); }
-    } else {
-      if (one) { if (c) KB_FUSE_MLP(8, 1, true); else KB_FUSE_MLP(8, 1, false); }
-      else { if (c) KB_FUSE_MLP(8, 4, true); else KB_FUSE_MLP(8, 4, false); }
-    }
-    return;
-  }
   if (m.vps == 16) {
     if (one) { if (c) KB_FUSE(16, 1, true); else KB_FUSE(16, 1, false); }
     else { if (c) KB_FUSE(16, 4, true); else KB_FUSE(16, 4, false); }
@@ -1901,8 +1441,12 @@
     else { if (c) KB_FUSE(8, 4, true); else KB_FUSE(8, 4, false); }
   }
 #undef KB_FUSE
-#undef KB_FUSE_MLP
-#undef KB_FUSE_MLP_G
+}
+void launchFuseWindow(const DeviceMap& m, const WindowParams& p, int grid, cudaStream_t s) {
+  if (grid <= 0) return;
+  const size_t smem = fuseSmemBytes(m.Lp);
+  if (m.vps == 16) fuseKernel<16, 1, false, false, true, true><<<grid, kFuseThreads, smem, s>>>(m, p);
+  else fuseKernel<8, 1, false, false, true, true><<<grid, kFuseThreads, smem, s>>>(m, p);
 }
 void launchTrackingPass(const DeviceMap& m, const TrackingParams& p, int everfree_grid, cudaStream_t s) {
   trackingPassKernel<<<(std::max(p.n_slots, 1) + 255) / 256, 256, 0, s>>>(m, p);
@@ -2045,3 +1589,19 @@
 
 
 }
+
+#ifdef KB_FUSE_TRACE
+extern "C" int kb_fuse_trace_reset() {
+  const unsigned z = 0;
+  if (cudaMemcpyToSymbol(kb::g_fuse_trace_n, &z, sizeof(z)) != cudaSuccess) return -1;
+  if (cudaMemcpyToSymbol(kb::g_fuse_trace_launch, &z, sizeof(z)) != cudaSuccess) return -1;
+  return cudaMemcpyToSymbol(kb::g_fuse_trace_exited, &z, sizeof(z)) == cudaSuccess ? 0 : -1;
+}
+extern "C" long long kb_fuse_trace_read(void* out, long long cap) {
+  unsigned n = 0;
+  if (cudaDeviceSynchronize() != cudaSuccess || cudaMemcpyFromSymbol(&n, kb::g_fuse_trace_n, sizeof(n)) != cudaSuccess) return -1;
+  const size_t k = std::min<size_t>({static_cast<size_t>(n), static_cast<size_t>(cap), static_cast<size_t>(kb::kFuseTraceCap)});
+  if (k && cudaMemcpyFromSymbol(out, kb::g_fuse_trace, k * sizeof(kb::FuseTraceRec)) != cudaSuccess) return -1;
+  return n;
+}
+#endif
diff --git a/khronos_b200/csrc/kb_kernels.cuh b/khronos_b200/csrc/kb_kernels.cuh
--- a/khronos_b200/csrc/kb_kernels.cuh
+++ b/khronos_b200/csrc/kb_kernels.cuh
@@ -22,7 +22,7 @@
   int target_id;
 };
 
-struct BatchParams {
+struct BatchCommon {
   int W, H;
   float fx, fy, cx, cy, min_range, max_range;
   float pl[4][2];
@@ -43,6 +43,12 @@
   int with_tracking;
   TrackEval trk;
   float occ_thr;
+  int item_list_cap;
+  int items_per_block;
+  int max_work;
+};
+
+struct BatchParams : BatchCommon {
   int n_frames;
   int parity;
   int compact_taps;
@@ -54,17 +60,36 @@
   uint32_t* work_upd;
   uint32_t* item_fmask;
   int pipelined;
-  int fetch_ctr;
-  int items_ctr;
-  int coop;
-  int mlp_group;
+  int* work_ctr;
+  int* fetch;
+  int* cls_ctr;
   int* item_list;
-  int item_list_cap;
-  int items_per_block;
+  int* item_prev;
+  uint32_t* last_listed;
+  uint32_t seq;
   int layers_per_item;
-  int max_work;
   FrameView f[kMaxBatch];
 };
+
+constexpr int kMaxWindow = 6;
+struct WindowBatch {
+  const int* work_slots;
+  uint32_t* work_upd;
+  const uint32_t* item_fmask;
+  const int* cls_ctr;
+  const int* item_list;
+  const int* item_prev;
+  uint32_t seq;
+};
+struct WindowParams : BatchCommon {
+  int n_batches;
+  uint32_t seq0;
+  int* fetch;
+  uint32_t* done;
+  WindowBatch b[kMaxWindow];
+  FrameView f[kMaxWindow][kMaxBatch];
+};
+static_assert(sizeof(WindowParams) <= 32764, "kernel parameter limit");
 
 struct TrackingParams {
   TrackEval ev;
@@ -118,6 +143,7 @@
 void launchExpandDepth(const uint16_t* src, float scale, float* dst, int n, cudaStream_t s);
 void launchSelectBlocks(const DeviceMap& m, const BatchParams& p, int cull_grid, cudaStream_t s);
 void launchFuse(const DeviceMap& m, const BatchParams& p, int grid, cudaStream_t s);
+void launchFuseWindow(const DeviceMap& m, const WindowParams& p, int grid, cudaStream_t s);
 int fuseBlocksPerSm(int vps, int Lp);
 void launchTrackingPass(const DeviceMap& m, const TrackingParams& p, int everfree_grid, cudaStream_t s);
 void launchResetInactive(const DeviceMap& m, const TrackEval& ev, int n_slots, int3* removed, int max_removed, cudaStream_t s);
```

After: 186,800, median of 6. 1.04x the previous value.
